# esq4/nind-denoise

Measured on AMD Instinct MI355X. Metric: megapixels/sec denoised, UtNet cs=256 on 24 MP frames, 1/2/4/8 MI355X, higher is better.
Workload: dtype f32; 1 GPU; configs[1]: one 6000x4000 (24.0 MP) fp32 frame per step, f32 storage in the conv stack (fp32 accumulate), UtNet(funit=64,PReLU) random-init (seed 123), cs=264 (nearest valid to the named size; the reference rejects 256 / 512) ucs=200 ol=64 -> 1276 tiles/frame, tiles per conv-stack launch 256, crop->infer->stitch device resident (frame and canvas in HBM); every tile's input is the whole cs x cs cro; tiles_per_frame=1276, parallelism=single GPU

## Files before the change

### include/nind_hip.h

```cpp
#ifndef NIND_HIP_H
#define NIND_HIP_H

#include <stddef.h>
#include <stdint.h>

#ifdef __cplusplus
extern "C" {
#endif

typedef enum nd_status {
    ND_OK = 0,
    ND_EINVAL = -1,
    ND_ENOMEM = -2,
    ND_EHIP = -3
} nd_status;

typedef enum nd_act {
    ND_ACT_NONE = 0,
    ND_ACT_PRELU = 1,
    ND_ACT_ELU = 2,
    ND_ACT_HARDSWISH = 3
} nd_act;

typedef enum nd_layer_kind {
    ND_CONV3 = 0,
    ND_CONVT3 = 1,
    ND_CONVT2S2 = 2,
    ND_CONV1 = 3,
    ND_CONV2S2 = 4
} nd_layer_kind;

typedef enum nd_dtype {
    ND_F32 = 0,
    ND_BF16 = 1,
    ND_F16 = 2
} nd_dtype;

typedef enum nd_flags {
    ND_FLAG_NO_SPLITK = 1,
    ND_FLAG_DIRECT_CONV = 2,
    ND_FLAG_W1D_REGS = 4,
    ND_FLAG_UNFUSED_POOL = 16,
    ND_FLAG_TILE_ENCODER = 32,
    ND_FLAG_TILE_LEVEL2 = 64,
    ND_FLAG_FIND_NOISE = 128,
    ND_FLAG_FULL_TILES = 8
} nd_flags;

int nd_version(void);
const char *nd_last_error(void);

int nd_tile_grid(int width, int height, int cs, int ucs, int ol, int *cols, int *rows, int *pad);
int nd_tile_geom(int i, int width, int height, int cs, int ucs, int ol,
                 int *x0, int *y0, int usefuldim[4], int usefulstart[2]);

int nd_tile_gather(const float *img_chw, int width, int height, int cs, int ucs, int ol,
                   int tile_begin, int tile_count, float *tiles_nchw, void *stream);
int nd_stitch_add(float *canvas_chw, int width, int height, int cs, int ucs, int ol,
                  const float *tiles_nchw, int tile_begin, int tile_count, void *stream);

int nd_utnet_num_tensors(void);
const char *nd_utnet_tensor_name(int idx);
size_t nd_utnet_packed_bytes(int funit, int dtype);
int nd_utnet_pack_weights(int funit, int dtype, const float *const *tensors, int n_tensors,
                          void *packed_host, size_t packed_bytes);

int nd_utnet_pack_weights_device(int funit, int dtype, const float *const *dev_tensors, int n_tensors, void *packed_dev,
                                 size_t packed_bytes, void *stream);

size_t nd_utnet_workspace_bytes_hw(int funit, int h, int w, int batch, int dtype);
int nd_utnet_workspace_init_hw(void *workspace, size_t workspace_bytes, int funit, int h, int w, int batch, int dtype,
                               void *stream);
int nd_utnet_forward_hw(int funit, int act, int dtype, int flags, const void *packed_dev,
                        const float *x_nchw, float *y_nchw, int batch, int h, int w,
                        void *workspace, size_t workspace_bytes, void *stream);

int nd_utnet_denoise_tiles(int funit, int act, int dtype, int flags, const void *packed_dev,
                           const float *img_chw, float *canvas_chw, int width, int height,
                           int cs, int ucs, int ol, int tile_begin, int tile_count, int batch,
                           void *workspace, size_t workspace_bytes, void *stream);

typedef void (*nd_progress_fn)(void *ctx, int n, int tile_begin, int tile_count);
size_t nd_utnet_frame_workspace_bytes(int funit, int dtype, int flags, int width, int height, int cs, int ucs, int ol, int batch);
int nd_utnet_denoise_frame(int funit, int act, int dtype, int flags, const void *packed_dev,
                           const float *img_chw, float *canvas_chw, int width, int height,
                           int cs, int ucs, int ol, int tile_begin, int tile_count, int batch,
                           void *workspace, size_t workspace_bytes, void *frame_ws, size_t frame_ws_bytes, void *stream,
                           nd_progress_fn progress, void *progress_ctx);
int nd_utnet_frame_plan(int funit, int dtype, int flags, int width, int height, int cs, int ucs, int ol, int *out);
int nd_utnet_frame_levels(int funit, int dtype, int flags, int width, int height, int cs, int ucs, int ol, int *levels);

typedef struct nd_step_profile {
    float ms;
    float ms_xform_in;
    float ms_gemm;
    float ms_xform_out;
    int form;
    int kind;
    double flops;
    double mfma_flops;
    double bytes;
    double xform_bytes_in;
    double xform_bytes_out;
} nd_step_profile;
int nd_utnet_profile_stack(int funit, int act, int dtype, int flags, const void *packed_dev, int batch, int cs, int crop,
                           void *workspace, size_t workspace_bytes, void *stream, nd_step_profile *steps, int max_steps);
const char *nd_utnet_step_name(int i);
int nd_utnet_useful_region(int funit, int cs, int crop, int step, int *rect);

int nd_unet_num_tensors(void);
const char *nd_unet_tensor_name(int idx);
size_t nd_unet_packed_bytes(int dtype);
int nd_unet_pack_weights(int dtype, const float *const *tensors, int n_tensors, void *packed_host, size_t packed_bytes);
size_t nd_unet_workspace_bytes(int h, int w, int batch, int dtype);
int nd_unet_workspace_init(void *workspace, size_t workspace_bytes, int h, int w, int batch, int dtype, void *stream);
int nd_unet_forward(int dtype, const void *packed_dev, const float *x_nchw, float *y_nchw, int batch, int h, int w,
                    void *workspace, size_t workspace_bytes, void *stream);

int nd_unet_pack_weights_device(int dtype, const float *const *dev_tensors, int n_tensors, void *packed_dev, size_t packed_bytes,
                                void *stream);

int nd_unet_num_steps(void);
const char *nd_unet_step_name(int i);
int nd_unet_useful_region(int cs, int crop, int step, int *rect);

int nd_unet_denoise_frame(int dtype, int flags, const void *packed_dev, const float *img_chw, float *canvas_chw, int width,
                          int height, int cs, int ucs, int ol, int tile_begin, int tile_count, int batch, void *workspace,
                          size_t workspace_bytes, void *stream, nd_progress_fn progress, void *progress_ctx);

double nd_utnet_flops(int funit, int cs);

size_t nd_layer_packed_bytes(int kind, int cin, int cout, int dtype);
int nd_layer_pack(int kind, int cin, int cout, int dtype, const float *weight, const float *bias,
                  void *packed_host, size_t packed_bytes);
size_t nd_layer_workspace_bytes(int kind, int batch, int cin, int cout, int h, int w, int dtype);
int nd_layer_forward(int kind, int act, float slope, int dtype, const void *packed_dev,
                     const float *x_nchw, int batch, int cin, int h, int w, int cout, float *y_nchw,
                     void *workspace, size_t workspace_bytes, int variant, int flags, void *stream);
int nd_maxpool2_forward(const float *x_nchw, int batch, int c, int h, int w, float *y_nchw,
                        void *workspace, size_t workspace_bytes, void *stream);

size_t nd_layer_wgrad_workspace_bytes(int kind, int batch, int cin, int cout, int h, int w);
int nd_layer_wgrad(int kind, const float *x_nchw, const float *dy_nchw, int batch, int cin, int h, int w, int cout,
// ... 53 lines not shown
```

### nind_denoise_amd/_lib.py

```python
import ctypes
import os
from ctypes import POINTER, c_char_p, c_double, c_float, c_int, c_size_t, c_void_p

_HERE = os.path.dirname(os.path.abspath(__file__))
LIB_PATH = os.path.join(_HERE, "libnind_hip.so")

ND_F32, ND_BF16, ND_F16 = 0, 1, 2
DTYPE = {"f32": 0, "fp32": 0, "float32": 0, "bf16": 1, "bfloat16": 1, "f16": 2, "fp16": 2, "float16": 2}
ACT = {"none": 0, "PReLU": 1, "ELU": 2, "Hardswish": 3}
KIND = {"conv3": 0, "convT3": 1, "convT2s2": 2, "conv1": 3, "conv2s2": 4}
FLAG_NO_SPLITK, FLAG_DIRECT_CONV, FLAG_W1D_REGS, FLAG_FULL_TILES, FLAG_UNFUSED_POOL, FLAG_TILE_ENCODER, FLAG_TILE_LEVEL2 = 1, 2, 4, 8, 16, 32, 64
FLAG_FIND_NOISE = 128
PROGRESS_FN = ctypes.CFUNCTYPE(None, c_void_p, c_int, c_int, c_int)


class StepProfile(ctypes.Structure):
    _fields_ = [("ms", c_float), ("ms_xform_in", c_float), ("ms_gemm", c_float), ("ms_xform_out", c_float),
                ("form", c_int), ("kind", c_int), ("flops", c_double), ("mfma_flops", c_double), ("bytes", c_double),
                ("xform_bytes_in", c_double), ("xform_bytes_out", c_double)]


FORM_NAMES = {-1: "pool", 0: "direct", 1: "w1d_f43", 2: "w1d_f23", 3: "wino3p_f6x6"}


class NindHipError(RuntimeError):
    pass


class NindHipMissing(ImportError):
    pass


_lib = None

_SIGNATURES = {
    "nd_version": (c_int, []),
    "nd_last_error": (c_char_p, []),
    "nd_tile_grid": (c_int, [c_int] * 5 + [POINTER(c_int)] * 3),
    "nd_tile_geom": (c_int, [c_int] * 6 + [POINTER(c_int)] * 4),
    "nd_tile_gather": (c_int, [c_void_p] + [c_int] * 7 + [c_void_p, c_void_p]),
    "nd_stitch_add": (c_int, [c_void_p] + [c_int] * 5 + [c_void_p, c_int, c_int, c_void_p]),
    "nd_utnet_num_tensors": (c_int, []),
    "nd_utnet_tensor_name": (c_char_p, [c_int]),
    "nd_utnet_packed_bytes": (c_size_t, [c_int, c_int]),
    "nd_utnet_pack_weights": (c_int, [c_int, c_int, POINTER(c_void_p), c_int, c_void_p, c_size_t]),
    "nd_utnet_pack_weights_device": (c_int, [c_int, c_int, POINTER(c_void_p), c_int, c_void_p, c_size_t, c_void_p]),
    "nd_utnet_workspace_bytes_hw": (c_size_t, [c_int] * 5),
    "nd_utnet_workspace_init_hw": (c_int, [c_void_p, c_size_t] + [c_int] * 5 + [c_void_p]),
    "nd_utnet_forward_hw": (c_int, [c_int] * 4 + [c_void_p] * 3 + [c_int, c_int, c_int, c_void_p, c_size_t, c_void_p]),
    "nd_utnet_denoise_tiles": (c_int, [c_int] * 4 + [c_void_p] * 3 + [c_int] * 8 + [c_void_p, c_size_t, c_void_p]),
    "nd_unet_num_tensors": (c_int, []),
    "nd_unet_tensor_name": (c_char_p, [c_int]),
    "nd_unet_packed_bytes": (c_size_t, [c_int]),
    "nd_unet_pack_weights": (c_int, [c_int, POINTER(c_void_p), c_int, c_void_p, c_size_t]),
    "nd_unet_workspace_bytes": (c_size_t, [c_int] * 4),
    "nd_unet_workspace_init": (c_int, [c_void_p, c_size_t] + [c_int] * 4 + [c_void_p]),
    "nd_unet_forward": (c_int, [c_int, c_void_p, c_void_p, c_void_p, c_int, c_int, c_int, c_void_p, c_size_t, c_void_p]),
    "nd_unet_pack_weights_device": (c_int, [c_int, POINTER(c_void_p), c_int, c_void_p, c_size_t, c_void_p]),
    "nd_unet_num_steps": (c_int, []),
    "nd_unet_step_name": (c_char_p, [c_int]),
    "nd_unet_useful_region": (c_int, [c_int, c_int, c_int, POINTER(c_int)]),
    "nd_unet_denoise_frame": (c_int, [c_int, c_int] + [c_void_p] * 3 + [c_int] * 8 + [c_void_p, c_size_t, c_void_p, PROGRESS_FN, c_void_p]),
    "nd_utnet_flops": (c_double, [c_int, c_int]),
    "nd_utnet_profile_stack": (c_int, [c_int] * 4 + [c_void_p, c_int, c_int, c_int, c_void_p, c_size_t, c_void_p, c_void_p, c_int]),
    "nd_utnet_step_name": (c_char_p, [c_int]),
    "nd_utnet_useful_region": (c_int, [c_int, c_int, c_int, c_int, POINTER(c_int)]),
    "nd_utnet_frame_workspace_bytes": (c_size_t, [c_int] * 9),
    "nd_utnet_frame_plan": (c_int, [c_int] * 8 + [POINTER(c_int)]),
    "nd_utnet_frame_levels": (c_int, [c_int] * 8 + [POINTER(c_int)]),
    "nd_utnet_denoise_frame": (c_int, [c_int] * 4 + [c_void_p] * 3 + [c_int] * 8 + [c_void_p, c_size_t, c_void_p, c_size_t, c_void_p,
                                                                                    PROGRESS_FN, c_void_p]),
    "nd_layer_packed_bytes": (c_size_t, [c_int] * 4),
    "nd_layer_pack": (c_int, [c_int] * 4 + [c_void_p, c_void_p, c_void_p, c_size_t]),
    "nd_layer_workspace_bytes": (c_size_t, [c_int] * 7),
    "nd_layer_forward": (c_int, [c_int, c_int, c_float, c_int, c_void_p, c_void_p] + [c_int] * 5
                         + [c_void_p, c_void_p, c_size_t, c_int, c_int, c_void_p]),
    "nd_winograd_packed_bytes": (c_size_t, [c_int] * 3),
    "nd_winograd_pack": (c_int, [c_int] * 4 + [c_void_p, c_void_p, c_void_p, c_size_t]),
    "nd_layer_winograd_workspace_bytes": (c_size_t, [c_int] * 7),
    "nd_layer_forward_winograd": (c_int, [c_int, c_int, c_int, c_float, c_void_p, c_void_p] + [c_int] * 5
                                  + [c_void_p, c_void_p, c_size_t, c_int, c_void_p]),
    "nd_maxpool2_forward": (c_int, [c_void_p] + [c_int] * 4 + [c_void_p, c_void_p, c_size_t, c_void_p]),
    "nd_layer_wgrad_workspace_bytes": (c_size_t, [c_int] * 6),
    "nd_layer_wgrad": (c_int, [c_int, c_void_p, c_void_p] + [c_int] * 5 + [c_void_p, c_void_p, c_void_p, c_size_t, c_void_p]),
    "nd_utnet_param_count": (c_size_t, [c_int]),
    "nd_utnet_param_range": (c_int, [c_int, c_int, POINTER(c_size_t), POINTER(c_size_t)]),
    "nd_utnet_train_blob_bytes": (c_size_t, [c_int]),
    "nd_utnet_grad_buckets": (c_int, [c_int, POINTER(c_size_t), POINTER(c_size_t), c_int]),
    "nd_utnet_train_workspace_bytes_hw": (c_size_t, [c_int] * 4),
    "nd_utnet_train_workspace_init_hw": (c_int, [c_void_p, c_size_t, c_int, c_int, c_int, c_int, c_void_p]),
    "nd_utnet_train_forward_hw": (c_int, [c_int, c_int, c_int, c_void_p, c_void_p, c_void_p, c_void_p, c_int, c_int, c_int, c_void_p,
                                          c_size_t, c_void_p]),
    "nd_utnet_train_backward_hw": (c_int, [c_int, c_int, c_int, c_void_p, c_void_p, c_void_p, c_void_p, c_void_p, c_int, c_int, c_int,
                                           c_void_p, c_size_t, c_void_p, POINTER(c_void_p), c_int]),
    "nd_utnet_train_step_hw": (c_int, [c_int, c_int, c_void_p, c_void_p, c_void_p, c_void_p, c_void_p, c_void_p, c_float, c_float,
                                       c_float, c_float, c_void_p, c_int, c_int, c_int, c_int, c_void_p, c_size_t, c_void_p,
                                       POINTER(c_void_p), c_int]),
    "nd_adam_step": (c_int, [c_void_p] * 5 + [c_size_t, c_float, c_float, c_float, c_float, c_int, c_int, c_void_p]),
    "nd_ssim_workspace_bytes": (c_size_t, [c_int] * 4),
    "nd_ssim": (c_int, [c_void_p, c_void_p] + [c_int] * 4 + [c_void_p, c_void_p, c_size_t, c_void_p]),
    "nd_ms_ssim": (c_int, [c_void_p, c_void_p] + [c_int] * 4 + [c_void_p, c_void_p, c_size_t, c_void_p]),
    "nd_ssim_loss_workspace_bytes": (c_size_t, [c_int] * 4),
    "nd_ssim_loss_grad": (c_int, [c_void_p, c_void_p] + [c_int] * 5 + [c_float, c_void_p, c_void_p, c_int, c_void_p, c_size_t,
                                  c_void_p]),
    "nd_mse": (c_int, [c_void_p, c_void_p, c_size_t, c_void_p, c_void_p, c_size_t, c_void_p]),
    "nd_conv_bench": (c_int, [c_int] * 9 + [c_void_p, c_size_t, c_void_p, POINTER(c_float)]),
    "nd_winograd_bench": (c_int, [c_int] * 8 + [c_void_p, c_size_t, c_void_p, POINTER(c_float)]),
    "nd_num_conv_variants": (c_int, []),
    "nd_conv_variant_name": (c_char_p, [c_int]),
}

EXPORTS = tuple(_SIGNATURES)


def load():
    global _lib
    if _lib is not None:
        return _lib
    if not os.path.isfile(LIB_PATH):
        raise NindHipMissing(
            f"{LIB_PATH} not found: build it with `make -C nind_denoise_amd/csrc` (or __graft_entry__.build()). "
            "nind_denoise_amd has no CPU fallback for the denoise hot path.")
# ... 46 lines not shown
```

### nind_denoise_amd/csrc/conv_f32.hip

```cpp
#include "conv_qp.inc"

extern const Variant g_variants_bf16[kGroup];
extern const Variant g_variants_f16[kGroup];
static const Variant g_f32_group[kGroup] = {ND_VARIANT_GROUP(ND_F32, "f32")};
static const Variant g_f32_extra[] = {
    ND_VARIANT(ND_F32, "f32", 2, 2, 2, 4, 9, 1, false, 3),
    ND_VARIANT(ND_F32, "f32", 2, 2, 1, 4, 9, 1, false, 3),
    ND_VARIANT(ND_F32, "f32", 2, 4, 4, 2, 1, 2, false, 3),
    ND_VARIANT(ND_F32, "f32", 2, 2, 2, 4, 1, 2, false, 3),
    ND_VARIANT(ND_F32, "f32", 2, 4, 4, 2, 1, 4, false, 2),
    ND_VARIANT(ND_F32, "f32", 2, 4, 2, 4, 1, 4, false, 2),
    ND_VARIANT(ND_F32, "f32", 2, 4, 4, 2, 1, 4, true, 2),
};
constexpr int kExtra = (int)(sizeof(g_f32_extra) / sizeof(g_f32_extra[0]));
static const int g_nvariants = 3 * kGroup + kExtra;
static const Variant &variant_at(int v) {
    if (v < kGroup) return g_f32_group[v];
    if (v < 2 * kGroup) return g_variants_bf16[v - kGroup];
    if (v < 3 * kGroup) return g_variants_f16[v - 2 * kGroup];
    return g_f32_extra[v - 3 * kGroup];
}


int nd_conv_variant_count() { return g_nvariants; }
// ... 157 lines not shown
        }
        const int order[] = {M <= 32 ? 3 : 0, 0, 1, 2};
        for (int v : order)
            if (variant_lds(variant_at(g0 + v), d.in, nullptr, nullptr, Hr, Wr, band2) <= kMaxLds) return g0 + v;
        return g0 + 2;
    }
    if (taps == 4) return g0 + (variant_lds(variant_at(g0 + 12), d.in, nullptr, nullptr, Hr, Wr) <= kMaxLds ? 12 : 13);
    if (KB % 2) return g0 + (up ? 7 : 5);
    if (up) {
        int cand[8], n = 0;
        if (dt == ND_F32 && M % 256 == 0 && KB % 4 == 0) cand[n++] = 3 * kGroup + 6;
        if (M >= 128) {
            if (KB % 4 == 0) cand[n++] = g0 + 10;
            if (KB % 2 == 0) cand[n++] = g0 + 8;
        }
        if (KB % 4 == 0) cand[n++] = g0 + 9;
        if (KB % 2 == 0) cand[n++] = g0 + 6;
        cand[n++] = g0 + 7;
        for (int i = 0; i < n; ++i)
            if (variant_lds(variant_at(cand[i]), d.in, nullptr, nullptr, Hr, Wr) <= kMaxLds) return cand[i];
        return cand[n - 1];
    }
    return g0 + 4;
}

bool nd_conv_pool_fits(const ConvDesc &d) {
    if (!d.pool || d.in.dt == ND_F32 || nd_taps(d.kind) != 9 || d.roi_rows > 0 || d.pre || d.nbatch > 1) return false;
    if (((d.in.Hb - 2) | (d.in.Wb - 2)) & 1) return false;
    if ((long)(d.in.Hb - 2) * (d.in.Wb - 2) < 100L * 100) return false;
    int dev, cus;
    if (nd_device(&dev, &cus) != ND_OK) return false;
    const int v = pick_variant(d, d.cout, cus);
    if (v < 0 || v >= g_nvariants) return false;
    return variant_lds(variant_at(v), d.in, nullptr, nullptr, 0, 0, true) <= kMaxLds;
}

bool nd_conv_roi_fits(const ConvDesc &d) {
    const bool up = d.kind == ND_CONVT2S2;
    int dev, cus;
    if (nd_device(&dev, &cus) != ND_OK) return false;
    const int v = pick_variant(d, up ? 4 * d.cout : d.cout, cus);
    if (v < 0 || v >= g_nvariants) return false;
    return variant_lds(variant_at(v), d.in, nullptr, nullptr, d.roi_rows > 0 ? d.roi_rows : 0, d.roi_rows > 0 ? d.roi_cols : 0) <= kMaxLds;
}

int nd_launch_conv(const ConvDesc &d, hipStream_t stream) {
    const int taps = nd_taps(d.kind);
    const bool up = d.kind == ND_CONVT2S2;
    const int dt = d.in.dt;
    if (dt < ND_F32 || dt > ND_F16 || d.out.dt != dt) ND_FAIL(ND_EINVAL, "conv: input / output storage types %d / %d", d.in.dt, d.out.dt);
    const int KB = nd_kblocks(d.cin, dt);
    const int M = up ? 4 * d.cout : d.cout;
    if (d.cout % nd_cpp(dt)) ND_FAIL(ND_EINVAL, "conv: cout=%d must be a multiple of %d", d.cout, nd_cpp(dt));
    ND_TRY(nd_check_in_planes("conv", d, KB));
    ND_TRY(nd_check_int32("conv", d.in));

    int dev = 0, ncus = 0;
    ND_TRY(nd_device(&dev, &ncus));
    int v = d.variant >= 0 ? d.variant : pick_variant(d, M, ncus);
    if (v < 0 || v >= g_nvariants) ND_FAIL(ND_EINVAL, "conv: unknown variant %d", v);
    const Variant &V = variant_at(v);
    if (V.taps != taps || V.up != up || V.dt != dt) ND_FAIL(ND_EINVAL, "conv: variant %s does not match layer kind %d / dtype %d", V.name, d.kind, dt);
    if (KB % V.kbc) ND_FAIL(ND_EINVAL, "conv: Cin/8=%d not a multiple of the variant's K chunk %d", KB, V.kbc);

    ConvParams p = nd_conv_params(d, KB, M);
    valid_grid(taps, d.in, &p.Hv, &p.Wv, &p.stride);
    const bool roi = d.roi_rows > 0;
    ND_TRY(nd_check_roi("conv", d, p.Hv, p.Wv, taps == 4 || d.nbatch > 1 || d.pre, "a stride-2, batched or training launch"));
    if (roi) {
        p.out += (long)((up ? 2 : 1) * d.roi_r0) * d.out.Wb + (up ? 2 : 1) * d.roi_c0;
        p.Hv = d.roi_rows;
        p.Wv = d.roi_cols;
    }
    p.PV = p.Hv * p.Wv;
    if (taps == 4 && ((d.in.Hb | d.in.Wb) & 1)) ND_FAIL(ND_EINVAL, "conv: the stride-2 layer reads even-sized buffers only");
    p.ioff = (taps == 9 ? 0 : d.in.pad * d.in.Wb + d.in.pad) + (roi ? d.roi_r0 * d.in.Wb + d.roi_c0 : 0);
    if (d.pre && (dt != ND_F32 || up)) ND_FAIL(ND_EINVAL, "conv: the pre-activation copy exists for fp32 non-upsampling layers only");
    ND_TRY(nd_check_out("conv", d, up ? 2 * p.Hv : p.Hv, up ? 2 * p.Wv : p.Wv, up || roi));

    if (d.pool) {
        if (dt == ND_F32 || taps != 9 || up || roi || d.pre || d.nbatch > 1 || (p.Hv & 1) || (p.Wv & 1))
            ND_FAIL(ND_EINVAL, "conv: a fused pool needs a whole 16-bit 3x3 layer with even output sizes (got %d x %d, dtype %d)", p.Hv, p.Wv, dt);
        ND_TRY(nd_conv_pool("conv", d, p.Hv, p.Wv, p));
        p.band2 = 1;
    }
    bool cross = true;
    const size_t lds = variant_lds(V, d.in, &cross, &p.G, roi ? p.Hv : 0, roi ? p.Wv : 0, p.band2 != 0);
    if (lds > kMaxLds) ND_FAIL(ND_EINVAL, "conv: %zu B of LDS needed (row width %d too large for variant %s)", lds, p.Wb, V.name);
    ND_TRY(nd_raise_lds(dev, (const void *)V.fn, lds));

    nd_conv_tiles(p, cross, V.nblk, V.mblk);
    p.linear = taps == 1 && !up && dt == ND_F32 && d.in.pad == 0 && d.out.pad == 0 && d.out.Hb == d.in.Hb && d.out.Wb == d.in.Wb && cross &&
               d.act == ND_ACT_NONE && d.nbatch > 1 && !d.pre && !roi;
    p.in_bs = d.in_bs;
    p.out_bs = d.out_bs;
    p.w_bs = (long)d.w_bs;
    if (d.nbatch > 1 && d.pre) ND_FAIL(ND_EINVAL, "conv: a batched launch keeps no pre-activation copy");
    nd_conv_fastdivs(p);
    if (dt != ND_F32) p.fd_upq = nd_fastdiv(p.cout / 8 > 0 ? p.cout / 8 : 1);
    const long ntiles = (long)p.tiles_per_problem * (d.nbatch > 1 ? d.nbatch : 1);
    const int per_cu = lds * 2 <= kMaxLds && V.threads <= 256 ? 2 : 1;
    const long slots = (long)ncus * per_cu;
    const long cap = d.part && !d.nosplit && !p.band2 ? (long)(d.part_bytes / ((size_t)V.mblk * V.nblk * 4)) : 0;
    const long grid = nd_conv_schedule(p, ntiles, KB / V.kbc, slots, cap);
    p.part = (f32x4 *)d.part;
#ifdef ND_QP_ABLATE
    static const int abl_env = getenv("ND_QP_ABL") ? atoi(getenv("ND_QP_ABL")) : 0;
    p.dbg = abl_env;
#endif
#ifdef ND_QP_STAMPS
    static const int dbg_env = getenv("ND_QP_DBG") ? atoi(getenv("ND_QP_DBG")) : 0;
    if (dbg_env & 128) {
        static int printed = 0;
        static const char *const names[5] = {"barrier", "issue DMA", "MFMA loop", "wait vmcnt", "epilogue+next"};
        char header[160];
        snprintf(header, sizeof header, "[qp stamps] %s cin %d M %d tiles %ld chunks %d G %d", V.name, d.cin, M, ntiles, KB / V.kbc, p.G);
        p.dbg = dbg_env;
        return nd_stamped_launch(V.fn, V.threads, lds, p, ntiles, KB / V.kbc, slots, stream, printed++ < 40, header, "   wave", names, 5,
// ... 9 lines not shown
```

### nind_denoise_amd/csrc/conv_qp.inc

```
#pragma once
#include <stdlib.h>

#include <initializer_list>
#include <type_traits>

#include "nd_common.h"

typedef float f32x4 __attribute__((ext_vector_type(4)));
typedef float f32x8 __attribute__((ext_vector_type(8)));
typedef float f32x16 __attribute__((ext_vector_type(16)));
typedef __bf16 bf16x8 __attribute__((ext_vector_type(8)));
typedef __bf16 bf16x4 __attribute__((ext_vector_type(4)));
typedef _Float16 f16x8 __attribute__((ext_vector_type(8)));
typedef _Float16 f16x4 __attribute__((ext_vector_type(4)));

template <int DT> struct FragOf { typedef f32x4 type; };
template <> struct FragOf<ND_BF16> { typedef bf16x8 type; };
template <> struct FragOf<ND_F16> { typedef f16x8 type; };

struct FastDiv {
    unsigned m;
    int sh;
};
static inline FastDiv nd_fastdiv(int d) {
    FastDiv f;
    int s = 0;
    while ((1L << s) < (long)d) ++s;
    f.m = (unsigned)((((unsigned long long)1 << (31 + s)) + (unsigned long long)d - 1) / (unsigned long long)d);
    f.sh = 31 + s;
    return f;
}
__device__ __forceinline__ unsigned fdiv(unsigned n, const FastDiv &f) { return (unsigned)(((unsigned long long)n * f.m) >> f.sh); }

struct ConvParams {
    const f32x4 *in;
    const float *wpk;
    const float *bias;
    f32x4 *out;
    long in_plane;
    long out_plane;
    int nimg;
    int P, Wb;
    int Hv, Wv, PV;
    int tpi;
    int G;
    int stride;
    int ioff;
    f32x4 *pre;
    long pre_plane;
    int KB;
    int M;
    int cout;
    int Po, Wo, opad;
    int out_plane0;
    int act;
    float slope;
    const float *slope_dev;
    int n_tiles_n;
    int n_tiles_m;
    int split_first, S, cps, nitems;
    f32x4 *part;
    int wpx;
    int tiles_per_problem;
    long in_bs, out_bs;
    long w_bs;
    int dbg;
    int linear;
    FastDiv fd_PV, fd_Wv, fd_ntm, fd_tpp, fd_upq, fd_tpi;
    f32x4 *pool;
    long pool_plane;
    int pool_P, pool_W, pool_pad;
    int band2;
    FastDiv fd_2Wv;
    const f32x4 *in2;
    long in2_plane;
    const int *origin2;
    int kb2, Wb2;
};

static inline void nd_conv_fastdivs(ConvParams &p) {
    p.fd_PV = nd_fastdiv(p.PV > 0 ? p.PV : 1);
    p.fd_Wv = nd_fastdiv(p.Wv > 0 ? p.Wv : 1);
    p.fd_2Wv = nd_fastdiv(p.Wv > 0 ? 2 * p.Wv : 1);
    p.fd_ntm = nd_fastdiv(p.n_tiles_m > 0 ? p.n_tiles_m : 1);
    p.fd_tpp = nd_fastdiv(p.tiles_per_problem > 0 ? p.tiles_per_problem : 1);
    p.fd_upq = nd_fastdiv(p.cout / 4 > 0 ? p.cout / 4 : 1);
    p.fd_tpi = nd_fastdiv(p.tpi > 0 ? p.tpi : 1);
}

ConvParams nd_conv_params(const ConvDesc &d, int KB, int M);
int nd_conv_pool(const char *who, const ConvDesc &d, int Hv, int Wv, ConvParams &p);
void nd_conv_tiles(ConvParams &p, bool cross, int nblk, int mblk);
long nd_conv_schedule(ConvParams &p, long ntiles, int nchunks, long slots, long cap);
double nd_conv_schedule_time(long ntiles, int nchunks, long slots, long cap);
int nd_launch_split_finish(const ConvParams &p, int n_split_tiles, int mblk, int nblk, int up, int dt, hipStream_t s);
#ifdef ND_QP_STAMPS
int nd_stamped_launch(void (*fn)(ConvParams), int threads, size_t lds, ConvParams p, long ntiles, int nchunks, long slots, hipStream_t s,
                      bool print, const char *header, const char *wave_prefix, const char *const *names, int nphases, std::initializer_list<int> waves);
#endif

__device__ __forceinline__ void glds16(const void *g, void *l) {
    __builtin_amdgcn_global_load_lds((const __attribute__((address_space(1))) void *)g,
                                     (__attribute__((address_space(3))) void *)l, 16, 0, 0);
}

__device__ __forceinline__ f32x8 sload8(const float *p) {
    const unsigned long long a = (unsigned long long)p;
    const unsigned lo = __builtin_amdgcn_readfirstlane((unsigned)a);
    const unsigned hi = __builtin_amdgcn_readfirstlane((unsigned)(a >> 32));
    const float *sp = (const float *)(((unsigned long long)hi << 32) | lo);
    f32x8 v;
    asm volatile("s_load_dwordx8 %0, %1, 0x0\n\ts_waitcnt lgkmcnt(0)" : "=s"(v) : "s"(sp) : "memory");
    return v;
}
__device__ __forceinline__ f32x4 sload_bias4(const float *p, int h) {
    const unsigned long long a = (unsigned long long)p;
    const unsigned lo = __builtin_amdgcn_readfirstlane((unsigned)a);
    const unsigned hi = __builtin_amdgcn_readfirstlane((unsigned)(a >> 32));
    const float *sp = (const float *)(((unsigned long long)hi << 32) | lo);
    f32x4 b0, b1;
    asm volatile("s_load_dwordx4 %0, %2, 0x0\n\ts_load_dwordx4 %1, %2, 0x10\n\ts_waitcnt lgkmcnt(0)" : "=&s"(b0), "=&s"(b1) : "s"(sp) : "memory");
    f32x4 r;
#pragma unroll
    for (int e = 0; e < 4; ++e) r[e] = h ? b1[e] : b0[e];
    return r;
}

#ifdef ND_QP_STAMPS
__device__ __forceinline__ unsigned long long qp_stamp() {
    unsigned long long t;
// ... 77 lines not shown
            const Item it = decode(vb + i * nwg);
            nsteps += it.c1 - it.c0;
        }
    if (nsteps == 0) return;

    auto pixel_of = [&](int nb, int l, int &img, int &r) -> bool {
        bool ok;
        if (p.tpi) {
            img = (int)fdiv((unsigned)nb, p.fd_tpi);
            r = (nb - img * p.tpi) * NBLK + l;
            ok = r < p.PV;
            r = ok ? r : p.PV - 1;
        } else {
            const unsigned g = (unsigned)nb * (unsigned)NBLK + (unsigned)l;
            const unsigned tot = (unsigned)p.nimg * (unsigned)p.PV;
            ok = g < tot;
            const unsigned gc = ok ? g : tot - 1;
            img = (int)fdiv(gc, p.fd_PV);
            r = (int)(gc - (unsigned)img * (unsigned)p.PV);
        }
        return ok;
    };
    auto yx_of = [&](int r, int &y, int &x) {
        if (p.band2) {
            const int band = (int)fdiv((unsigned)r, p.fd_2Wv), rem = r - band * 2 * p.Wv;
            y = 2 * band + (rem & 1);
            x = rem >> 1;
        } else {
            y = (int)fdiv((unsigned)r, p.fd_Wv);
            x = r - y * p.Wv;
        }
    };
    auto q_of = [&](int img, int r) -> long {
        int y, x;
        yx_of(r, y, x);
        return (long)img * p.P + (long)(y * p.stride) * p.Wb + x * p.stride + p.ioff;
    };
    auto tile_q0 = [&](int nb) -> long {
        if (TAPS == 1 && !UP && p.linear) return (long)nb * NBLK;
        int img, r;
        pixel_of(nb, 0, img, r);
        return q_of(img, r);
    };

    int f_id = vb, f_c = 0, f_end = 0, f_stage = 0, issued = 0;
    const float *f_w;
    const f32x4 *f_a;
    auto set_fill_tile = [&](int w) {
        const Item it = decode(w);
        f_c = it.c0;
        f_end = it.c1;
        const int z = (int)fdiv((unsigned)it.tile, p.fd_tpp), id = it.tile - z * p.tiles_per_problem;
        const int nb = (int)fdiv((unsigned)id, p.fd_ntm), mb = id - nb * p.n_tiles_m;
        f_w = p.wpk + z * p.w_bs + (size_t)mb * MTB * p.KB * TAPS * 256 + lane * 4;
        f_a = p.in + z * p.in_bs + tile_q0(nb) + lane;
    };
    set_fill_tile(f_id);
    constexpr bool SPREAD = DT != ND_F32 && TAPS == 9;
    constexpr int NFILL = SPREAD ? NW : (NW > 4 ? 4 : NW);
    constexpr int RW = KBC * TAPS;
    constexpr int NGROUPS = STEPS * (DT == ND_F32 ? 4 : 1);
#ifndef ND_QP_NUSE_NUM
#define ND_QP_NUSE_NUM 5
#endif
    constexpr int NUSE = NGROUPS * ND_QP_NUSE_NUM / 8 > 1 ? NGROUPS * ND_QP_NUSE_NUM / 8 : 1;
    constexpr int PSUB_ = (NUSE - MTB) / (2 * KBC);
    constexpr int PSUB = PSUB_ < 1 ? 1 : (PSUB_ > 4 ? 4 : PSUB_);
    constexpr int NSLICE = MTB + 2 * KBC * PSUB;
    constexpr int SPG = (NSLICE + NUSE - 1) / NUSE;
    char *fill_sb = smem;
    bool fill_on = false;
    auto fill_begin = [&]() {
        fill_on = issued < nsteps;
        fill_sb = smem + f_stage * stageB;
    };
    auto fill_slice = [&](int i) {
        if (!fill_on || wave >= NFILL) return;
#ifdef ND_QP_ABLATE
        if (p.dbg & (i < MTB ? 2 : 1)) return;
#endif
        if (i < MTB) {
            const float *src = f_w + ((size_t)i * p.KB + (size_t)f_c * KBC) * TAPS * 256;
            char *dst = fill_sb + i * RW * 1024;
            for (int q = wave; q < RW; q += NFILL) glds16(src + q * 256, dst + q * 1024);
        } else {
            const int pl = (i - MTB) / PSUB, part = (i - MTB) % PSUB;
            const f32x4 *src = f_a + (size_t)(f_c * 2 * KBC + pl) * p.in_plane;
            char *dst = fill_sb + WBYTES + pl * planeB;
            for (int g = wave + part * NFILL; g < G; g += NFILL * PSUB) glds16(src + g * 64, dst + g * 1024);
        }
    };
    auto fill_end = [&]() {
        if (!fill_on) return;
        ++issued;
        f_stage = (f_stage + 1 == NSTAGE) ? 0 : f_stage + 1;
        if (++f_c == f_end) {
            f_id += nwg;
            if (f_id < nitems) set_fill_tile(f_id);
        }
    };
    auto fill_group = [&](int gi) {
        if (!SPREAD || gi * SPG >= NSLICE) return;
        __builtin_amdgcn_sched_barrier(0);
#pragma unroll
        for (int k = 0; k < SPG; ++k)
            if (gi * SPG + k < NSLICE) {
                fill_slice(gi * SPG + k);
                if (gi * SPG + k == NSLICE - 1) fill_end();
            }
        __builtin_amdgcn_sched_barrier(0);
    };
    auto fill_next = [&]() {
        fill_begin();
#pragma unroll
        for (int i = 0; i < NSLICE; ++i) fill_slice(i);
        fill_end();
    };

    const int aOff = (wm * MR) * KBC * TAPS * 1024 + lane * 16;
    struct BOff { int v[NR]; };
    auto lane_offsets = [&](int w) -> BOff {
        BOff o;
        if (TAPS == 1 && !UP && p.linear) {
#pragma unroll
            for (int nr = 0; nr < NR; ++nr) o.v[nr] = WBYTES + h * planeB + ((wn * NR + nr) * 32 + j) * 16;
            return o;
        }
        const int tl_ = decode(w).tile;
        const int nb = (int)fdiv((unsigned)(tl_ - (int)fdiv((unsigned)tl_, p.fd_tpp) * p.tiles_per_problem), p.fd_ntm);
        const long q0 = tile_q0(nb);
#pragma unroll
        for (int nr = 0; nr < NR; ++nr) {
            int img, r;
            pixel_of(nb, (wn * NR + nr) * 32 + j, img, r);
            o.v[nr] = WBYTES + h * planeB + (int)(q_of(img, r) - q0) * 16;
// ... 349 lines not shown
```

### nind_denoise_amd/csrc/conv_w2d.hip

```cpp
#include "conv_qp.inc"

namespace {

typedef float f32x2 __attribute__((ext_vector_type(2)));

constexpr int kR = 8;
constexpr int kS = 16;
constexpr int kRI = kR + 2;
constexpr int kVPlane = kRI * kS * 16;
constexpr int kVPos = 2 * kVPlane;
constexpr int kVBytes = 6 * kVPos;
constexpr int kTaps = 18;
constexpr int kMTB = 2;
constexpr int kWBytes = kMTB * kTaps * 1024;
constexpr int kStage = kWBytes + kVBytes;
constexpr int kStages = 2;
constexpr int kScratch = 2048;
constexpr int kLds = kStages * kStage + 8 * kScratch;
constexpr int kDmaAt = 4;
constexpr int kXfAt = 12;
constexpr int kSlots = 4 * 32 * 4;

template <int OFF> __device__ __forceinline__ void glds16o(const void *g, void *l) {
    __builtin_amdgcn_global_load_lds((const __attribute__((address_space(1))) void *)g, (__attribute__((address_space(3))) void *)l, 16, OFF, 0);
}

__device__ __forceinline__ int vslot(int r, int s) { return r * kS + (s ^ ((r & 3) << 2)); }

__device__ __forceinline__ void w4_in(const f32x4 *d, f32x4 *v) {
    const f32x4 s34 = d[3] + d[4], d43 = d[4] - d[3], s12 = d[1] + d[2], d12 = d[1] - d[2], d42 = d[4] - d[2], d31 = d[3] - d[1];
    v[0] = 4.f * d[0] - 5.f * d[2] + d[4];
    v[1] = s34 - 4.f * s12;
    v[2] = d43 + 4.f * d12;
    v[3] = d42 + 2.f * d31;
    v[4] = d42 - 2.f * d31;
    v[5] = 4.f * d[1] - 5.f * d[3] + d[5];
}
__device__ __forceinline__ void w4_out(const float *m, float *y) {
    const float a = m[1] + m[2], b = m[1] - m[2], c = m[3] + m[4], e = m[3] - m[4];
    y[0] = m[0] + a + c;
    y[1] = b + 2.f * e;
    y[2] = a + 4.f * c;
    y[3] = b + 8.f * e + m[5];
}

__device__ __forceinline__ unsigned long long stamp() {
    unsigned long long t;
    __builtin_amdgcn_sched_barrier(0);
    asm volatile("s_memtime %0\n\ts_waitcnt lgkmcnt(0)" : "=s"(t)::"memory");
    __builtin_amdgcn_sched_barrier(0);
    return t;
}

struct Strip { int img, y0, x0; bool ok; };

template <int DBG, bool SRC2 = false>
__global__ __launch_bounds__(512) void conv_w2d(ConvParams p) {
    extern __shared__ __attribute__((aligned(16))) char smem[];
    const int lane = threadIdx.x & 63;
    const int wave = __builtin_amdgcn_readfirstlane(threadIdx.x >> 6);
    const int wm = wave >> 2, wn = wave & 3;
    const int j = lane & 31, h = lane >> 5;
    const int nwg = gridDim.x;
    const int bid = blockIdx.x;
    const int vb = (nwg % 8 == 0) ? (bid % 8) * (nwg / 8) + bid / 8 : bid;

    const int nchunks = p.KB;
    const int nitems = p.nitems;
    const int my_items = vb < nitems ? (nitems - vb + nwg - 1) / nwg : 0;
    struct Item { int tile, c0, c1, slice; };
    auto decode = [&](int w) -> Item {
        Item it;
        if (w < p.split_first) {
            it.tile = w; it.c0 = 0; it.c1 = nchunks; it.slice = -1;
        } else {
            const int u = w - p.split_first;
            const int t = u / p.S, ks = u - t * p.S;
            it.tile = p.split_first + t;
            it.c0 = ks * p.cps;
            it.c1 = it.c0 + p.cps < nchunks ? it.c0 + p.cps : nchunks;
            it.slice = u;
        }
        return it;
    };
    int nsteps = 0;
    if (p.split_first >= nitems)
        nsteps = my_items * nchunks;
    else
        for (int i = 0; i < my_items; ++i) {
            const Item it = decode(vb + i * nwg);
            nsteps += it.c1 - it.c0;
        }
    if (nsteps == 0) return;

    const unsigned tot = (unsigned)p.nimg * (unsigned)p.PV;
    auto strip_of = [&](int nb, int s) -> Strip {
        Strip r;
        const unsigned u = (unsigned)nb * kS + s;
        r.ok = u < tot;
        const unsigned uc = r.ok ? u : tot - 1;
        r.img = (int)fdiv(uc, p.fd_PV);
        const int rem = (int)(uc - (unsigned)r.img * p.PV);
        const int band = (int)fdiv((unsigned)rem, p.fd_Wv);
        r.y0 = band * kR;
        r.x0 = 4 * (rem - band * p.Wv);
        return r;
    };

    int f_id = vb, f_c = 0, f_end = 0, f_stage = 0, issued = 0;
    int f_nb = 0;
    const float *f_w;
    const unsigned lane16 = (unsigned)lane * 16u;
    const int kXfHalf = 1;
    const bool xfA = (wave >> 2) == kXfHalf, xfB = wave == 4 * (1 - kXfHalf);
    const int dw = wave - 4 * (1 - kXfHalf);
    int vwOff[2];
    int x_h[2], x_i[2], x_s[2];
#pragma unroll
    for (int ps = 0; ps < 2; ++ps) {
        const int xt = ps == 0 ? (wave & 3) * 64 + lane : 256 + lane;
        x_h[ps] = xt / (kS * kRI);
        x_i[ps] = (xt / kS) % kRI;
        x_s[ps] = xt % kS;
        vwOff[ps] = kWBytes + x_h[ps] * kVPlane + vslot(x_i[ps], x_s[ps]) * 16;
    }
    unsigned x_off[2] = {0, 0};
    int x_keep[2] = {6, 6};
    auto set_fill_tile = [&](int w) {
        const Item it = decode(w);
        f_c = it.c0;
        f_end = it.c1;
        const int nb = (int)fdiv((unsigned)it.tile, p.fd_ntm), mb = it.tile - nb * p.n_tiles_m;
        f_w = p.wpk + (size_t)mb * kMTB * p.KB * kTaps * 256;
        if constexpr (SRC2) f_nb = nb;
#pragma unroll
        for (int ps = 0; ps < 2; ++ps)
            if (ps == 0 ? xfA : xfB) {
                const Strip st = strip_of(nb, x_s[ps]);
                x_off[ps] = 16u * ((unsigned)x_h[ps] * (unsigned)p.in_plane + (unsigned)st.img * (unsigned)p.P + (unsigned)(st.y0 + x_i[ps]) * p.Wb + st.x0);
                const int left = p.wpx - st.x0;
                x_keep[ps] = left + 2 < 6 ? left + 2 : 6;
            }
    };
    auto set_fill_src2 = [&]() {
        const int nb = f_nb;
#pragma unroll
        for (int ps = 0; ps < 2; ++ps)
            if (ps == 0 ? xfA : xfB) {
                const Strip st = strip_of(nb, x_s[ps]);
                x_off[ps] = 16u * ((unsigned)x_h[ps] * (unsigned)p.in2_plane + (unsigned)p.origin2[st.img] + (unsigned)(st.y0 + x_i[ps]) * p.Wb2 + st.x0);
            }
    };
    set_fill_tile(f_id);
    if constexpr (SRC2) if (f_c >= p.kb2) set_fill_src2();
    f32x4 dn[2][6];
#pragma unroll
    for (int ps = 0; ps < 2; ++ps)
#pragma unroll
        for (int k = 0; k < 6; ++k) dn[ps][k] = f32x4{0.f, 0.f, 0.f, 0.f};
    auto fill_loads = [&]() {
        if (issued >= nsteps || (DBG & 8)) return;
        const bool s2 = SRC2 && f_c >= p.kb2;
        const char *kbase = s2 ? (const char *)(p.in2 + (size_t)(2 * (f_c - p.kb2)) * p.in2_plane)
                               : (const char *)(p.in + (size_t)(2 * f_c) * p.in_plane);
        if (xfA) {
#pragma unroll
            for (int k = 0; k < 6; ++k) dn[0][k] = *(const f32x4 *)(kbase + x_off[0] + 16 * k);
        }
        if (xfB) {
#pragma unroll
            for (int k = 0; k < 6; ++k) dn[1][k] = *(const f32x4 *)(kbase + x_off[1] + 16 * k);
        }
    };
    auto fill_xform = [&]() {
        if (issued >= nsteps || (DBG & 16)) return;
#pragma unroll
        for (int ps = 0; ps < 2; ++ps)
            if (ps == 0 ? xfA : xfB) {
                if (__builtin_amdgcn_ballot_w64(x_keep[ps] < 6)) {
                    const f32x4 zero = {0.f, 0.f, 0.f, 0.f};
#pragma unroll
                    for (int k = 3; k < 6; ++k)
                        if (k >= x_keep[ps]) dn[ps][k] = zero;
                }
                f32x4 v[6];
                w4_in(dn[ps], v);
                char *dst = smem + f_stage * kStage + vwOff[ps];
#pragma unroll
                for (int x = 0; x < 6; ++x) *(f32x4 *)(dst + x * kVPos) = v[x];
            }
    };
    auto fill_dma = [&]() {
        if (issued >= nsteps || (DBG & 4)) return;
        if (dw >= 0 && dw < 4) {
            const int mt = dw >> 1, pl0 = (dw & 1) * 9;
            const char *src = (const char *)(f_w + (((size_t)mt * p.KB + (size_t)f_c) * kTaps + pl0) * 256) + lane16;
            char *dst = smem + f_stage * kStage + (mt * kTaps + pl0) * 1024;
            glds16o<-4096>(src + 4096, dst + 4096);
            glds16o<-3072>(src + 4096, dst + 4096);
            glds16o<-2048>(src + 4096, dst + 4096);
            glds16o<-1024>(src + 4096, dst + 4096);
            glds16o<0>(src + 4096, dst + 4096);
            glds16o<1024>(src + 4096, dst + 4096);
            glds16o<2048>(src + 4096, dst + 4096);
            glds16o<3072>(src + 4096, dst + 4096);
            glds16o<0>(src + 8192, dst + 8192);
        }
    };
    auto fill_advance = [&]() {
        if (issued >= nsteps) return;
        ++issued;
        f_stage ^= 1;
        if (++f_c == f_end) {
            f_id += nwg;
            if (f_id < nitems) {
                set_fill_tile(f_id);
                if constexpr (SRC2) if (f_c >= p.kb2) set_fill_src2();
            }
        } else if constexpr (SRC2) {
            if (f_c == p.kb2) set_fill_src2();
        }
    };

    const int sl = 4 * wn + (j >> 3), rr = j & 7;
    const int aOff = (wm * kTaps) * 1024 + lane * 16;
    int bOffK[3];
#pragma unroll
    for (int ky = 0; ky < 3; ++ky) bOffK[ky] = kWBytes + h * kVPlane + vslot(rr + ky, sl) * 16;

    f32x16 acc[6];
#pragma unroll
    for (int x = 0; x < 6; ++x)
#pragma unroll
        for (int r = 0; r < 16; ++r) acc[x][r] = 0.f;

    const float slope = p.act == ND_ACT_NONE ? 1.f : (p.slope_dev ? *p.slope_dev : p.slope);
    const bool slope01 = p.act <= ND_ACT_PRELU && slope >= 0.f && slope <= 1.f;

    auto combine = [&](int g, f32x4 *y) {
#pragma unroll
        for (int e = 0; e < 4; ++e) {
            float m[6], o[4];
#pragma unroll
            for (int x = 0; x < 6; ++x) {
                m[x] = acc[x][4 * g + e];
                acc[x][4 * g + e] = 0.f;
            }
            w4_out(m, o);
#pragma unroll
            for (int i = 0; i < 4; ++i) y[i][e] = o[i];
        }
    };

    char *const scratch = smem + kStages * kStage + wave * kScratch;
    const int e_row = lane >> 4, e_px = lane & 15;
    f32x4 biasq[4];
    auto load_bias = [&](int id) {
        const int mb = id - (int)fdiv((unsigned)id, p.fd_ntm) * p.n_tiles_m;
#pragma unroll
        for (int g = 0; g < 4; ++g) biasq[g] = *(const f32x4 *)(p.bias + (mb * kMTB + wm) * 32 + 8 * g + 4 * h);
    };
    load_bias(decode(vb).tile);
    auto epilogue = [&](int id, auto fast) {
        const int nb = (int)fdiv((unsigned)id, p.fd_ntm), mb = id - nb * p.n_tiles_m;
        const Strip st = strip_of(nb, 4 * wn + (e_px >> 2));
        const int ex = st.x0 + (e_px & 3);
        const unsigned offA = (unsigned)((st.img * p.Po + (st.y0 + e_row + p.opad) * p.Wo + ex + p.opad) * 16);
        const unsigned offB = offA + (unsigned)(4 * p.Wo * 16);
        const bool okx = st.ok && ex < p.wpx;
        const bool okA = okx && st.y0 + e_row < p.Hv, okB = okx && st.y0 + e_row + 4 < p.Hv;
        const int q0 = (mb * kMTB + wm) * 8;
        const f32x2 slope2 = {slope, slope};
        const int pp_i = (e_px & ~3) + 2 * (e_px & 1);
        const int pxp = (st.x0 >> 1) + (e_px & 1), pyp = (st.y0 >> 1) + e_row;
        const bool okP = !SRC2 && p.pool && !(lane & 2) && st.ok && 2 * pxp + 1 < p.wpx && 2 * pyp + 1 < p.Hv;
        const unsigned offP = (unsigned)((st.img * p.pool_P + (pyp + p.pool_pad) * p.pool_W + pxp + p.pool_pad) * 16);
#pragma unroll
        for (int g = 0; g < 4; ++g) {
            f32x4 yy[4], ypre[4];
#pragma unroll
            for (int pr = 0; pr < 2; ++pr) {
                f32x2 m[6];
#pragma unroll
                for (int x = 0; x < 6; ++x) {
                    m[x] = f32x2{acc[x][4 * g + 2 * pr], acc[x][4 * g + 2 * pr + 1]};
                    acc[x][4 * g + 2 * pr] = 0.f;
                    acc[x][4 * g + 2 * pr + 1] = 0.f;
                }
                const f32x2 bq = {biasq[g][2 * pr], biasq[g][2 * pr + 1]};
                const f32x2 a = m[1] + m[2] + bq, b = m[1] - m[2] + bq, c = m[3] + m[4], e = m[3] - m[4];
                f32x2 y[4];
                y[0] = m[0] + a + c;
                y[1] = b + 2.f * e;
                y[2] = a + 4.f * c;
                y[3] = b + 8.f * e + m[5];
#pragma unroll
                for (int i = 0; i < 4; ++i) {
                    ypre[i][2 * pr] = y[i][0];
                    ypre[i][2 * pr + 1] = y[i][1];
                    if constexpr (decltype(fast)::value) {
                        const f32x2 t = y[i] * slope2;
                        y[i] = f32x2{fmaxf(y[i][0], t[0]), fmaxf(y[i][1], t[1])};
                    } else {
                        y[i] = f32x2{apply_act(y[i][0], p.act, slope), apply_act(y[i][1], p.act, slope)};
                    }
                    yy[i][2 * pr] = y[i][0];
                    yy[i][2 * pr + 1] = y[i][1];
                }
            }
            if (!SRC2 && p.pre) {
                const Strip so = strip_of(nb, sl);
                const int yo = so.y0 + rr, m4 = (q0 + 2 * g + h) * 4, left = p.wpx - so.x0;
                if (so.ok && yo < p.Hv && m4 < p.M) {
                    f32x4 *dst = p.pre + (long)(m4 >> 2) * p.pre_plane + ((long)so.img * p.Hv + yo) * p.wpx + so.x0;
#pragma unroll
                    for (int i = 0; i < 4; ++i)
                        if (i < left) dst[i] = ypre[i];
                }
            }
            if (DBG & 256) {
                const Strip so = strip_of(nb, sl);
                const int yo = so.y0 + rr, m4 = (q0 + 2 * g + h) * 4, left = p.wpx - so.x0;
                if (so.ok && yo < p.Hv && m4 < p.M) {
                    f32x4 *dst = p.out + (long)(p.out_plane0 + (m4 >> 2)) * p.out_plane + (long)so.img * p.Po + (long)(yo + p.opad) * p.Wo + so.x0 + p.opad;
#pragma unroll
                    for (int i = 0; i < 4; ++i)
                        if (i < left) dst[i] = yy[i];
                }
                continue;
            }
#pragma unroll
            for (int hq = 0; hq < 2; ++hq) {
                if (h == hq) {
                    f32x4 *w = (f32x4 *)scratch + rr * 16 + (j >> 3) * 4;
#pragma unroll
                    for (int i = 0; i < 4; ++i) w[i] = yy[i];
                }
                __builtin_amdgcn_fence(__ATOMIC_RELEASE, "wavefront");
                __builtin_amdgcn_wave_barrier();
                __builtin_amdgcn_fence(__ATOMIC_ACQUIRE, "wavefront");
                const f32x4 va = *((const f32x4 *)scratch + e_row * 16 + e_px);
                const f32x4 vb2 = *((const f32x4 *)scratch + (e_row + 4) * 16 + e_px);
                f32x4 vp = va;
                if (!SRC2 && p.pool) {
                    const f32x4 *blk = (const f32x4 *)scratch + (2 * e_row) * 16 + pp_i;
                    const f32x4 p00 = blk[0], p01 = blk[1], p10 = blk[16], p11 = blk[17];
#pragma unroll
                    for (int e = 0; e < 4; ++e) vp[e] = fmaxf(fmaxf(p00[e], p01[e]), fmaxf(p10[e], p11[e]));
                }
                __builtin_amdgcn_fence(__ATOMIC_RELEASE, "wavefront");
                __builtin_amdgcn_wave_barrier();
                __builtin_amdgcn_fence(__ATOMIC_ACQUIRE, "wavefront");
                const int quad = q0 + 2 * g + hq;
                if (quad * 4 < p.M && !(DBG & 1)) {
                    char *pb = (char *)(p.out + (size_t)(p.out_plane0 + quad) * p.out_plane);
                    if (okA) *(f32x4 *)(pb + offA) = va;
                    if (okB) *(f32x4 *)(pb + offB) = vb2;
                    if (okP) *(f32x4 *)((char *)(p.pool + (size_t)quad * p.pool_plane) + offP) = vp;
                }
            }
        }
    };
    auto epilogue_partial = [&](int slice) {
        f32x4 *dst = p.part + (size_t)slice * (kMTB * 8) * kSlots;
#pragma unroll
        for (int g = 0; g < 4; ++g) {
            f32x4 yy[4];
            combine(g, yy);
            f32x4 *d2 = dst + (size_t)(wm * 8 + 2 * g + h) * kSlots + 4 * (wn * 32 + j);
#pragma unroll
            for (int i = 0; i < 4; ++i) d2[i] = yy[i];
        }
    };

    fill_loads();
    fill_xform();
    fill_dma();
    fill_advance();
    asm volatile("s_waitcnt vmcnt(0) lgkmcnt(0)" ::: "memory");
    __builtin_amdgcn_s_barrier();

    int c_id = vb, c_stage = 0;
    Item c_it = decode(vb);
    int c_c = c_it.c0;
    unsigned long long tph[6] = {0, 0, 0, 0, 0, 0}, t0 = 0, t1 = 0;
    for (int s = 0; s < nsteps; ++s) {
        if (DBG & 128) t0 = stamp();
        fill_loads();
        __builtin_amdgcn_sched_barrier(0);
        if (DBG & 128) { t1 = stamp(); tph[0] += t1 - t0; t0 = t1; }
        const char *wa = smem + c_stage * kStage + aOff;
        const char *vq = smem + c_stage * kStage;
        f32x4 a[2], b[2];
        a[0] = *(const f32x4 *)wa;
        b[0] = *(const f32x4 *)(vq + bOffK[0]);
#pragma unroll
        for (int st = 0; st < kTaps; ++st) {
// ... 13 lines not shown
            }
            if (st + 1 == kDmaAt) {
                __builtin_amdgcn_sched_barrier(0);
                fill_dma();
                __builtin_amdgcn_sched_barrier(0);
            }
            if (st + 1 == kXfAt) {
                __builtin_amdgcn_sched_barrier(0);
                if (DBG & 128) { t1 = stamp(); tph[1] += t1 - t0; t0 = t1; }
                fill_xform();
                fill_advance();
                if (DBG & 128) { t1 = stamp(); tph[3] += t1 - t0; t0 = t1; }
                __builtin_amdgcn_sched_barrier(0);
            }
        }
        __builtin_amdgcn_sched_barrier(0);
        if (DBG & 128) { t1 = stamp(); tph[1] += t1 - t0; t0 = t1; }
        asm volatile("s_waitcnt vmcnt(0) lgkmcnt(0)" ::: "memory");
        if (DBG & 128) { t1 = stamp(); tph[2] += t1 - t0; t0 = t1; }
        c_stage ^= 1;
        if (++c_c == c_it.c1) {
            if (DBG & 2) {
            } else if (c_it.slice >= 0)
                epilogue_partial(c_it.slice);
            else if (slope01)
                epilogue(c_it.tile, std::true_type{});
            else
                epilogue(c_it.tile, std::false_type{});
            c_id += nwg;
            if (c_id < nitems) {
                c_it = decode(c_id);
                if (p.n_tiles_m > 1) load_bias(c_it.tile);
            }
            c_c = c_it.c0;
        }
        if (DBG & 128) { t1 = stamp(); tph[4] += t1 - t0; t0 = t1; }
        if (!(DBG & 64)) __builtin_amdgcn_s_barrier();
        if (DBG & 128) { t1 = stamp(); tph[5] += t1 - t0; }
    }
    if ((DBG & 128) && lane == 0 && p.part) {
        unsigned long long *o = (unsigned long long *)p.part + ((size_t)blockIdx.x * 8 + wave) * 8;
        for (int k = 0; k < 6; ++k) o[k] = tph[k];
        o[6] = (unsigned long long)nsteps;
    }
}

__global__ __launch_bounds__(256) void k_w2d_split_finish(ConvParams p) {
    const int t = blockIdx.x, quad = blockIdx.y;
    const int gid = p.split_first + t;
    const int nb = gid / p.n_tiles_m, mb = gid - nb * p.n_tiles_m;
    const int m4 = mb * (kMTB * 32) + quad * 4;
    if (m4 >= p.M) return;
    const float slope = p.act == ND_ACT_NONE ? 1.f : (p.slope_dev ? *p.slope_dev : p.slope);
    const f32x4 bv = *(const f32x4 *)(p.bias + m4);
    const unsigned tot = (unsigned)p.nimg * (unsigned)p.PV;
    for (int l = threadIdx.x; l < kSlots; l += 256) {
        const int i = l & 3, jj = l >> 2, wn = jj >> 5, j = jj & 31;
        const int s = 4 * wn + (j >> 3), rr = j & 7;
        const unsigned u = (unsigned)nb * kS + s;
        if (u >= tot) continue;
        const int img = (int)(u / (unsigned)p.PV);
        const int rem = (int)(u - (unsigned)img * p.PV);
        const int band = rem / p.Wv;
        const int y = band * kR + rr, x = 4 * (rem - band * p.Wv) + i;
        if (y >= p.Hv || x >= p.wpx) continue;
        f32x4 acc = {0.f, 0.f, 0.f, 0.f};
        for (int ks = 0; ks < p.S; ++ks) acc += p.part[((size_t)(t * p.S + ks) * (kMTB * 8) + quad) * kSlots + l];
        acc += bv;
        f32x4 v;
#pragma unroll
        for (int e = 0; e < 4; ++e) v[e] = p.act <= ND_ACT_PRELU ? (acc[e] > 0.f ? acc[e] : acc[e] * slope) : apply_act(acc[e], p.act, slope);
        p.out[(long)(p.out_plane0 + (m4 >> 2)) * p.out_plane + (long)img * p.Po + (long)(y + p.opad) * p.Wo + x + p.opad] = v;
    }
}

}

bool nd_w2d_ok(const QpBuf &in) { return in.dt == ND_F32 && in.Hb >= 3 && in.Wb >= 3; }
long nd_w2d_tiles(const QpBuf &in, int cout) {
    const long strips = (long)in.B * ((in.Hb - 2 + kR - 1) / kR) * ((in.Wb - 2 + 3) / 4);
    return ((strips + kS - 1) / kS) * ((cout + kMTB * 32 - 1) / (kMTB * 32));
}

int nd_launch_conv_w2d(const ConvDesc &d, hipStream_t stream) {
    if ((d.kind != ND_CONV3 && d.kind != ND_CONVT3) || d.in.dt != ND_F32 || d.out.dt != ND_F32) ND_FAIL(ND_EINVAL, "w2d: fp32 3x3 layers only");
    const int KB = nd_kblocks(d.cin);
    const int Hfull = d.in.Hb - 2, Wfull = d.in.Wb - 2;
    if (Hfull < 1 || Wfull < 1) ND_FAIL(ND_EINVAL, "w2d: input smaller than the kernel");
    ND_TRY(nd_check_roi("w2d", d, Hfull, Wfull, d.pool != nullptr, "a pooled layer"));
    const bool roi = d.roi_rows > 0;
    const int Hv = roi ? d.roi_rows : Hfull, Wpx = roi ? d.roi_cols : Wfull, Wg = (Wpx + 3) / 4, NB = (Hv + kR - 1) / kR;
    if (d.pre && (roi || d.pool)) ND_FAIL(ND_EINVAL, "w2d: a pre-activation copy goes with whole, unpooled layers only");
    if (d.cout % 4) ND_FAIL(ND_EINVAL, "w2d: cout must be a multiple of 4");
    ND_TRY(nd_check_in_planes("w2d", d, KB, true));
    const bool src2 = d.in2.base != nullptr;
    if (src2 && (d.pool || d.pre)) ND_FAIL(ND_EINVAL, "w2d: a layer with a second input source is neither pooled nor keeps a pre-activation copy");
    if (src2) ND_TRY(nd_check_in2("w2d", d, KB, (long)(d.roi_r0 + (NB - 1) * kR + kRI - 1) * d.in2.Wb + d.roi_c0 + 4 * (Wg - 1) + 6));
    ND_TRY(nd_check_out("w2d", d, Hfull, Wfull, false));
    ND_TRY(nd_check_int32("w2d", d.in));
    if (2 * d.in.np() * 16 + 65536 >= (1L << 32)) ND_FAIL(ND_EINVAL, "w2d: input too large for 32-bit byte offsets");

    int dev = 0, ncus = 0;
    ND_TRY(nd_device(&dev, &ncus));
    void (*fn)(ConvParams) = src2 ? conv_w2d<0, true> : conv_w2d<0>;
#ifdef ND_QP_STAMPS
    static const int dbg_all = getenv("ND_W2D_DBG") ? atoi(getenv("ND_W2D_DBG")) : 0;
    const int dbg_env = src2 ? 0 : dbg_all;
    switch (dbg_env) {
        case 1: fn = conv_w2d<1>; break;
        case 2: fn = conv_w2d<2>; break;
        case 4: fn = conv_w2d<4>; break;
        case 8: fn = conv_w2d<8>; break;
        case 16: fn = conv_w2d<16>; break;
        case 24: fn = conv_w2d<24>; break;
        case 28: fn = conv_w2d<28>; break;
        case 30: fn = conv_w2d<30>; break;
        case 32: fn = conv_w2d<32>; break;
        case 62: fn = conv_w2d<62>; break;
        case 128: fn = conv_w2d<128>; break;
        case 256: fn = conv_w2d<256>; break;
        default: break;
    }
#endif
    ND_TRY(nd_raise_lds(dev, (const void *)fn, kLds));

    ConvParams p = nd_conv_params(d, KB, d.cout);
    if (roi) {
        p.in += (long)d.roi_r0 * d.in.Wb + d.roi_c0;
        p.out += (long)d.roi_r0 * d.out.Wb + d.roi_c0;
    }
    if (src2) {
        p.in2 = (const f32x4 *)d.in2.base + (long)d.in2_plane0 * d.in2.np() + (roi ? (long)d.roi_r0 * d.in2.Wb + d.roi_c0 : 0);
        p.in2_plane = d.in2.np();
        p.origin2 = d.in2_origin;
        p.kb2 = d.in2_from / 2;
        p.Wb2 = d.in2.Wb;
    }
    p.Hv = Hv;
    p.Wv = Wg;
    p.PV = NB * Wg;
    p.wpx = Wpx;
    if (d.pool) {
        ND_TRY(nd_conv_pool("w2d", d, Hv, Wpx, p));
        if (d.pool->used() * 16 >= (1L << 32)) ND_FAIL(ND_EINVAL, "w2d: pooled destination too large for 32-bit byte offsets");
    }
    nd_conv_tiles(p, true, kS, kMTB * 32);
    nd_conv_fastdivs(p);
    const long ntiles = p.tiles_per_problem;
    const long cap = d.part && !d.nosplit && !d.pool && !d.pre ? (long)(d.part_bytes / ((size_t)kMTB * 32 * kSlots * 4)) : 0;
    const long grid = nd_conv_schedule(p, ntiles, KB, ncus, cap);
    p.part = (f32x4 *)d.part;
#ifdef ND_QP_STAMPS
    if (dbg_env == 128) {
        static int printed = 0;
        static const char *const names[6] = {"issue loads + DMA", "MFMA loop", "wait vmcnt", "transform+publish (inside the loop)", "epilogue", "barrier"};
        return nd_stamped_launch(fn, 512, kLds, p, ntiles, KB, ncus, stream, printed++ < 2, nullptr, "[w2d stamps] wave", names, 6, {0, 1, 4});
    }
#endif
    hipLaunchKernelGGL(fn, dim3((unsigned)grid), dim3(512), kLds, stream, p);
    if (p.split_first < ntiles) hipLaunchKernelGGL(k_w2d_split_finish, dim3((unsigned)(ntiles - p.split_first), kMTB * 8), dim3(256), 0, stream, p);
    ND_HIP(hipGetLastError());
    return ND_OK;
}

bool nd_f43_w2d(const QpBuf &in, int cout, bool pre, int flags) {
    return !(flags & ND_FLAG_W1D_REGS) && nd_w2d_ok(in) && (!pre || nd_w2d_tiles(in, cout) >= 512);
}
int nd_launch_conv_f43(const ConvDesc &d, int flags, hipStream_t stream) {
    return nd_f43_w2d(d.in, d.cout, d.pre != nullptr, flags) ? nd_launch_conv_w2d(d, stream) : nd_launch_conv_w1d(4, d, stream);
}
```

### nind_denoise_amd/csrc/launch.hip

```cpp
#include <atomic>
#include <mutex>
#include <unordered_map>
#include <vector>

#include "conv_qp.inc"

namespace {
constexpr int kMaxDevices = 16;
std::atomic<int> g_cus[kMaxDevices];
std::mutex g_mu;
std::unordered_map<const void *, int> g_state[kMaxDevices];
}

int nd_device(int *dev, int *ncus) {
    ND_HIP(hipGetDevice(dev));
    if (*dev < 0 || *dev >= kMaxDevices) ND_FAIL(ND_EINVAL, "device index %d outside [0, %d)", *dev, kMaxDevices);
    if (!ncus) return ND_OK;
    int n = g_cus[*dev].load(std::memory_order_relaxed);
    if (!n) {
        hipDeviceProp_t prop;
        ND_HIP(hipGetDeviceProperties(&prop, *dev));
        n = prop.multiProcessorCount > 0 ? prop.multiProcessorCount : 256;
        g_cus[*dev].store(n, std::memory_order_relaxed);
    }
    *ncus = n;
    return ND_OK;
}

int nd_raise_lds(int dev, const void *fn, size_t bytes) {
    std::lock_guard<std::mutex> lock(g_mu);
    int &limit = g_state[dev][fn];
    if ((int)bytes <= limit) return ND_OK;
    ND_HIP(hipFuncSetAttribute(fn, hipFuncAttributeMaxDynamicSharedMemorySize, (int)bytes));
    limit = (int)bytes;
    return ND_OK;
}

int nd_once_per_device(int dev, int (*init)()) {
    std::lock_guard<std::mutex> lock(g_mu);
    int &done = g_state[dev][(const void *)init];
    if (done) return ND_OK;
    ND_TRY(init());
    done = 1;
    return ND_OK;
}

int nd_check_in_planes(const char *who, const ConvDesc &d, int KB, bool takes_in2) {
    if (d.in.planes < d.in_plane0 + 2 * KB) ND_FAIL(ND_EINVAL, "%s: input buffer has %d planes, needs %d", who, d.in.planes, d.in_plane0 + 2 * KB);
    if (d.in2.base && !takes_in2) ND_FAIL(ND_EINVAL, "%s: this kernel form has no second input source", who);
    return ND_OK;
}

int nd_check_in2(const char *who, const ConvDesc &d, int KB, long reach) {
    const QpBuf &q = d.in2;
    const int n2 = 2 * KB - d.in2_from;
    if (q.dt != ND_F32 || d.in.dt != ND_F32 || !d.in2_origin || d.in2_from <= 0 || (d.in2_from & 1) || n2 <= 0 || d.in2_plane0 < 0 ||
        d.in2_plane0 + n2 > q.planes || d.in2_origin_max < 0 || reach <= 0)
        ND_FAIL(ND_EINVAL, "%s: second input source: planes [%d,+%d) of %d from input plane %d of %d", who, d.in2_plane0, n2, q.planes,
                d.in2_from, 2 * KB);
    const long last = d.in2_origin_max + reach, room = (long)(q.planes - d.in2_plane0 - n2 + 1) * q.np() + (long)nd_buf_slack(q.Wb);
    if (last > room) ND_FAIL(ND_EINVAL, "%s: second input source: a launch reaches element %ld of a plane, the buffer ends at %ld", who, last, room);
    if ((2 * q.np() + last) * 16 + 65536 >= (1L << 32)) ND_FAIL(ND_EINVAL, "%s: second input source too large for 32-bit byte offsets", who);
    return ND_OK;
}

int nd_check_out(const char *who, const ConvDesc &d, int oh, int ow, bool at_least) {
    const int Hb = oh + 2 * d.out.pad, Wb = ow + 2 * d.out.pad;
    const bool fits = at_least ? (d.out.Hb >= Hb && d.out.Wb >= Wb) : (d.out.Hb == Hb && d.out.Wb == Wb);
    if (!fits || d.out.B != d.in.B)
        ND_FAIL(ND_EINVAL, "%s: destination %dx%dx%d(pad %d) does not fit result %dx%dx%d", who, d.out.B, d.out.Hb, d.out.Wb, d.out.pad,
                d.in.B, oh, ow);
    if (d.out_plane0 + d.cout / nd_cpp(d.out.dt) > d.out.planes) ND_FAIL(ND_EINVAL, "%s: destination planes overflow", who);
    return ND_OK;
}

int nd_check_int32(const char *who, const QpBuf &in) {
    if (in.used() >= (1L << 31)) ND_FAIL(ND_EINVAL, "%s: %ld linear pixels exceed the int32 index range", who, in.used());
    return ND_OK;
}

int nd_check_roi(const char *who, const ConvDesc &d, int Hv, int Wv, bool refused, const char *why) {
    if (d.roi_rows <= 0) return ND_OK;
    if (refused || d.roi_r0 < 0 || d.roi_c0 < 0 || d.roi_cols < 1 || d.roi_r0 + d.roi_rows > Hv || d.roi_c0 + d.roi_cols > Wv)
        ND_FAIL(ND_EINVAL, "%s: region [%d,+%d) x [%d,+%d) outside the %d x %d grid (or %s)", who, d.roi_r0, d.roi_rows, d.roi_c0,
                d.roi_cols, Hv, Wv, why);
    return ND_OK;
}

ConvParams nd_conv_params(const ConvDesc &d, int KB, int M) {
    ConvParams p = {};
    p.in = (const f32x4 *)d.in.base + (long)d.in_plane0 * d.in.np();
    p.wpk = d.wpk;
    p.bias = d.bias;
    p.out = (f32x4 *)d.out.base;
    p.in_plane = d.in.np();
    p.out_plane = d.out.np();
    p.nimg = d.in.B;
    p.P = d.in.Hb * d.in.Wb;
    p.Wb = d.in.Wb;
    p.pre = (f32x4 *)d.pre;
    p.pre_plane = d.pre_plane;
    p.KB = KB;
    p.M = M;
    p.cout = d.cout;
    p.Po = d.out.Hb * d.out.Wb;
    p.Wo = d.out.Wb;
    p.opad = d.out.pad;
    p.out_plane0 = d.out_plane0;
    p.act = d.act;
    p.slope = d.slope;
    p.slope_dev = d.slope_dev;
    return p;
}

int nd_conv_pool(const char *who, const ConvDesc &d, int Hv, int Wv, ConvParams &p) {
    const QpBuf &q = *d.pool;
    if (q.dt != d.in.dt || q.B != d.in.B || q.Hb - 2 * q.pad != Hv / 2 || q.Wb - 2 * q.pad != Wv / 2 || q.planes < d.cout / nd_cpp(d.in.dt))
        ND_FAIL(ND_EINVAL, "%s: pooled destination does not fit %d x %d x %d", who, d.cout, Hv / 2, Wv / 2);
    p.pool = (f32x4 *)q.base;
    p.pool_plane = q.np();
    p.pool_P = q.Hb * q.Wb;
    p.pool_W = q.Wb;
    p.pool_pad = q.pad;
    return ND_OK;
}

void nd_conv_tiles(ConvParams &p, bool cross, int nblk, int mblk) {
    if (cross) {
        p.tpi = 0;
        p.n_tiles_n = (int)(((long)p.nimg * p.PV + nblk - 1) / nblk);
    } else {
        p.tpi = (p.PV + nblk - 1) / nblk;
        p.n_tiles_n = p.tpi * p.nimg;
    }
    p.n_tiles_m = (p.M + mblk - 1) / mblk;
    p.tiles_per_problem = p.n_tiles_n * p.n_tiles_m;
}

namespace {
constexpr double kSplitOver = 3.0;
struct SplitPlan { int first, S, cps; double time; };
SplitPlan plan_split(long ntiles, int nchunks, long slots, long max_items) {
    SplitPlan b;
    const long full = ntiles / slots * slots, R = ntiles - full;
    b.first = (int)ntiles;
    b.S = 1;
    b.cps = nchunks;
    b.time = (double)((ntiles + slots - 1) / slots) * (nchunks + kSplitOver);
    if (R == 0 || max_items <= 0) return b;
    const double base = (double)(full / slots) * (nchunks + kSplitOver);
    for (int S = 2; S <= nchunks && S <= 64; ++S) {
        const int cps = (nchunks + S - 1) / S, Se = (nchunks + cps - 1) / cps;
        if (R * Se > max_items) break;
        const double t = base + (double)((R * Se + slots - 1) / slots) * (cps + 1.5 * kSplitOver);
        if (t < 0.93 * b.time) {
// ... 62 lines not shown
```

### nind_denoise_amd/csrc/nd_common.h

```cpp
#pragma once
#include <hip/hip_runtime.h>

#include <stdarg.h>
#include <stdint.h>
#include <stdio.h>

#include "nind_hip.h"

void nd_set_error(const char *fmt, ...);
#define ND_FAIL(code, ...)        \
    do {                          \
        nd_set_error(__VA_ARGS__); \
        return (code);            \
    } while (0)
#define ND_HIP(call)                                                                         \
    do {                                                                                     \
        hipError_t e_ = (call);                                                              \
        if (e_ != hipSuccess) ND_FAIL(ND_EHIP, "%s failed: %s", #call, hipGetErrorString(e_)); \
    } while (0)
#define ND_TRY(call)        \
    do {                    \
        int r_ = (call);    \
        if (r_ != 0) return r_; \
    } while (0)

static inline int nd_cpp(int dt) { return dt == ND_F32 ? 4 : 8; }
struct QpBuf {
    float *base;
    int planes;
    int B, Hb, Wb;
    int pad;
    long pstride;
    int dt = ND_F32;
    long np() const { return pstride; }
    long used() const { return (long)B * Hb * Wb; }
};

struct ConvDesc {
    int kind = ND_CONV3;
    int act = ND_ACT_NONE;
    float slope = 1.f;
    const float *slope_dev = nullptr;
    const float *wpk = nullptr;
    const float *bias = nullptr;
    int cin = 0, cout = 0;
    QpBuf in = {};
    QpBuf out = {};
    int out_plane0 = 0;
    int variant = -1;
    int in_plane0 = 0;
    float *pre = nullptr;
    long pre_plane = 0;
    float *part = nullptr;
    size_t part_bytes = 0;
    bool nosplit = false;
    int nbatch = 1;
    long in_bs = 0, out_bs = 0;
    size_t w_bs = 0;
    const QpBuf *pool = nullptr;
    int roi_r0 = 0, roi_c0 = 0, roi_rows = 0, roi_cols = 0;
    QpBuf in2 = {};
    int in2_plane0 = 0, in2_from = 0;
    const int *in2_origin = nullptr;
    long in2_origin_max = 0;
};
int nd_check_in2(const char *who, const ConvDesc &d, int KB, long reach);
static const size_t kSplitScratchBytes = (size_t)512 * 64 * 1024 * 4;
int nd_launch_conv(const ConvDesc &d, hipStream_t stream);
bool nd_conv_pool_fits(const ConvDesc &d);
bool nd_conv_roi_fits(const ConvDesc &d);
int nd_conv_variant_count();
int nd_conv_variant_gemm(int cin, int cout);
size_t nd_wino_packed_floats(int T, int cin, int cout);
int nd_wino_pack(int T, int kind, int cin, int cout, const float *w, const float *bias, float *packed);
size_t nd_wino_scratch_bytes(int T, const QpBuf &in, int cin, int cout);
int nd_launch_conv_wino(int T, const ConvDesc &d, void *scratch, size_t scratch_bytes, hipStream_t s, hipEvent_t *ev2 = nullptr);
void nd_wino_xform_bytes(int T, const QpBuf &in, int cin, int cout, double *bytes_in, double *bytes_out);
size_t nd_w1d_packed_floats(int T, int cin, int cout);
int nd_w1d_pack(int T, int kind, int cin, int cout, const float *w, const float *bias, float *packed);
bool nd_w1d_fits(int T, const QpBuf &in);
int nd_launch_conv_w1d(int T, const ConvDesc &d, hipStream_t stream);
bool nd_w2d_ok(const QpBuf &in);
long nd_w2d_tiles(const QpBuf &in, int cout);
int nd_launch_conv_w2d(const ConvDesc &d, hipStream_t stream);
bool nd_f43_w2d(const QpBuf &in, int cout, bool pre, int flags);
int nd_launch_conv_f43(const ConvDesc &d, int flags, hipStream_t stream);
static inline size_t nd_buf_slack(int Wb) { return (size_t)10 * Wb + 8 + 2048; }
int nd_device(int *dev, int *ncus = nullptr);
int nd_raise_lds(int dev, const void *fn, size_t bytes);
int nd_once_per_device(int dev, int (*init)());
int nd_check_in_planes(const char *who, const ConvDesc &d, int KB, bool takes_in2 = false);
int nd_check_out(const char *who, const ConvDesc &d, int oh, int ow, bool at_least);
int nd_check_int32(const char *who, const QpBuf &in);
int nd_check_roi(const char *who, const ConvDesc &d, int Hv, int Wv, bool refused, const char *why);
static inline int nd_check_flags(int flags, bool frame_loop = false, bool unet_frame = false) {
    const int known = ND_FLAG_NO_SPLITK | ND_FLAG_DIRECT_CONV | ND_FLAG_W1D_REGS | ND_FLAG_FULL_TILES | ND_FLAG_UNFUSED_POOL |
                      ND_FLAG_TILE_ENCODER | (frame_loop ? ND_FLAG_TILE_LEVEL2 : 0) | (unet_frame ? ND_FLAG_FIND_NOISE : 0);
    if (flags & ~known) ND_FAIL(ND_EINVAL, "unknown flag bits 0x%x", flags);
    return ND_OK;
}
const char *nd_conv_variant_label(int v);

static inline int nd_mtiles(int kind, int cout) {
    return kind == ND_CONVT2S2 ? (4 * cout + 255) / 256 * 8 : (cout + 127) / 128 * 4;
}
struct NdUpRow { int a, b, co; };
__host__ __device__ static inline NdUpRow nd_up_row(int m, int cout, int dt) {
    NdUpRow r;
    const int cpp = dt == ND_F32 ? 4 : 8, q = cout / cpp;
    const int G = m / (2 * cpp), e = m % cpp;
    r.b = (m / cpp) & 1;
    r.a = G / q;
    r.co = cpp * (G % q) + e;
    return r;
}
static inline int nd_taps(int kind) { return (kind == ND_CONV3 || kind == ND_CONVT3) ? 9 : (kind == ND_CONV2S2 ? 4 : 1); }
static inline int nd_kblocks(int cin, int dt = ND_F32) { return (cin + 2 * nd_cpp(dt) - 1) / (2 * nd_cpp(dt)); }
static inline size_t nd_bias_offset(int kind, int cin, int cout, int dt = ND_F32, int w1d_T = 0) {
    return (size_t)nd_mtiles(kind, cout) * nd_kblocks(cin, dt) * (w1d_T ? 3 * (w1d_T + 2) : nd_taps(kind)) * 256;
}
static inline size_t nd_packed_floats(int kind, int cin, int cout, int dt = ND_F32) {
    return nd_bias_offset(kind, cin, cout, dt) + (size_t)nd_mtiles(kind, cout) * 32;
}
void nd_pack_layer(int kind, int cin, int cout, int dt, const float *w, const float *bias, float *packed);

int nd_pack_layer_device(int kind, int cin, int cout, int dt, const float *w, const float *bias, float *packed, hipStream_t s,
                         const float *scale = nullptr);
int nd_launch_bn_fold(int cout, const float *b, const float *g, const float *be, const float *rm, const float *rv, float *scale,
                      float *fbias, hipStream_t s);
int nd_pack_w1d_device(int T, int kind, int cin, int cout, const float *w, const float *bias, float *packed, hipStream_t s);
int nd_pack_wino_device(int T, int kind, int cin, int cout, const float *w, const float *bias, float *packed, hipStream_t s);

int nd_launch_nchw_to_qp(const float *x, int C, const QpBuf &dst, int plane0, hipStream_t s);
int nd_launch_qp_to_nchw(const QpBuf &src, int plane0, float *y, int C, hipStream_t s);
int nd_launch_reflect_pack(const float *x_nchw, int B, int H, int W, const QpBuf &dst, hipStream_t s);
int nd_launch_maxpool2(const QpBuf &src, int src_plane0, int planes, const QpBuf &dst, hipStream_t s);
int nd_launch_final1x1(const QpBuf &src, int cin, const float *w, const float *bias, int crop, float *y_nchw, int H,
                       int W, hipStream_t s, int sigmoid = 0);
int nd_launch_final1x1_stitch(const QpBuf &src, int cin, const float *w, const float *bias, int crop, float *canvas,
                              int width, int height, int cs, int ucs, int ol, int tile_begin, int tile_count,
                              hipStream_t s, int sigmoid = 0, const float *noise_img = nullptr);
int nd_launch_gather_pack(const float *img, int width, int height, int cs, int ucs, int ol, int tile_begin,
                          int tile_count, const QpBuf &dst, hipStream_t s, int border = 2, bool reflect = true);
int nd_launch_gather_band(const float *img, int width, int height, int cs, int ucs, int ol, int band_row0, const QpBuf &dst,
                          hipStream_t s);
enum nd_edge_set { ND_EDGE_ROWS = 0, ND_EDGE_COLS = 1, ND_EDGE_CORNERS = 2 };
int nd_launch_gather_edges(const float *img, int width, int height, int cs, int ucs, int ol, int set, int first, int count,
                           const QpBuf &dst, hipStream_t s);
int nd_launch_skip_origins(const QpBuf &src, int dst_pad, int tile_begin, int tile_count, int cols, int band_rows, int step, long slot_elems,
                           int *table, long *origin_max, hipStream_t s);
// ... 7 lines not shown
```

### nind_denoise_amd/csrc/pack.hip

```cpp
#include <string.h>

#include "nd_common.h"

static thread_local char g_err[512] = "";

void nd_set_error(const char *fmt, ...) {
    va_list ap;
    va_start(ap, fmt);
    vsnprintf(g_err, sizeof(g_err), fmt, ap);
    va_end(ap);
}

extern "C" const char *nd_last_error(void) { return g_err; }
extern "C" int nd_version(void) { return 109; }

static inline uint16_t f32_to_bf16_rne(float f) {
    uint32_t u;
    memcpy(&u, &f, 4);
    if ((u & 0x7fffffffu) > 0x7f800000u) return (uint16_t)((u >> 16) | 0x40);
    return (uint16_t)((u + 0x7fffu + ((u >> 16) & 1u)) >> 16);
}
static inline uint16_t f32_to_f16_rne(float f) {
    const _Float16 h = (_Float16)f;
    uint16_t u;
    memcpy(&u, &h, 2);
    return u;
}

void nd_pack_layer(int kind, int cin, int cout, int dt, const float *w, const float *bias, float *packed) {
    const int taps = nd_taps(kind);
    const int KB = nd_kblocks(cin, dt);
    const int MT = nd_mtiles(kind, cout);
    const int M = kind == ND_CONVT2S2 ? 4 * cout : cout;
    const int cpp = nd_cpp(dt);
    float *bp = packed + nd_bias_offset(kind, cin, cout, dt);
    auto weff = [&](int m, int ci, int t) -> float {
        if (m >= M || ci >= cin) return 0.f;
        switch (kind) {
            case ND_CONV3: return w[((size_t)m * cin + ci) * 9 + t];
            case ND_CONVT3: return w[((size_t)ci * cout + m) * 9 + (8 - t)];
            case ND_CONVT2S2: {
                const NdUpRow r = nd_up_row(m, cout, dt);
                return w[((size_t)ci * cout + r.co) * 4 + 2 * r.a + r.b];
            }
            case ND_CONV2S2: return w[((size_t)m * cin + ci) * 4 + t];
            default: return w[(size_t)m * cin + ci];
        }
    };
    for (int mt = 0; mt < MT; ++mt)
        for (int kb = 0; kb < KB; ++kb)
            for (int t = 0; t < taps; ++t) {
                float *dst = packed + (((size_t)mt * KB + kb) * taps + t) * 256;
                uint16_t *dst16 = (uint16_t *)dst;
                for (int lane = 0; lane < 64; ++lane) {
                    const int i = lane & 31, h = lane >> 5;
                    const int m = 32 * mt + i;
                    for (int s = 0; s < cpp; ++s) {
                        const float v = weff(m, 2 * cpp * kb + cpp * h + s, t);
                        if (dt == ND_F32)
                            dst[lane * 4 + s] = v;
                        else
                            dst16[lane * 8 + s] = dt == ND_BF16 ? f32_to_bf16_rne(v) : f32_to_f16_rne(v);
                    }
                }
            }
    for (int m = 0; m < MT * 32; ++m) {
        float v = 0.f;
// ... 21 lines not shown
```

### nind_denoise_amd/csrc/utnet.hip

```cpp
#include <string.h>

#include <string>
#include <vector>

#include "nd_common.h"

#include "utnet_net.h"

extern "C" int nd_utnet_num_tensors(void) { return (int)tensor_names().size(); }
extern "C" const char *nd_utnet_tensor_name(int idx) {
    const auto &n = tensor_names();
    return (idx >= 0 && idx < (int)n.size()) ? n[idx].c_str() : nullptr;
}

extern "C" size_t nd_utnet_packed_bytes(int funit, int dtype) {
    if (check_funit(funit, dtype) != ND_OK) return 0;
    return blob_layout(funit, dtype).total * sizeof(float);
}

extern "C" int nd_utnet_pack_weights(int funit, int dtype, const float *const *tensors, int n_tensors, void *packed_host,
                                     size_t packed_bytes) {
    ND_TRY(check_funit(funit, dtype));
    if (n_tensors != nd_utnet_num_tensors()) ND_FAIL(ND_EINVAL, "nd_utnet_pack_weights: expected %d tensors, got %d", nd_utnet_num_tensors(), n_tensors);
    const BlobLayout bl = blob_layout(funit, dtype);
// ... 108 lines not shown
    ND_TRY(nd_launch_final1x1(pl.buf[T4B], funit, fw, fw + 3 * funit, 2, y, h, w, s));
    return ND_OK;
}

extern "C" int nd_utnet_denoise_tiles(int funit, int act, int dtype, int flags, const void *packed, const float *img,
                                      float *canvas, int width, int height, int cs, int ucs, int ol, int tile_begin,
                                      int tile_count, int batch, void *ws, size_t ws_bytes, void *stream) {
    ND_TRY(nd_check_flags(flags));
    Plan pl;
    ND_TRY(forward_common(funit, act, dtype, packed, batch, tile_count, cs, cs, ws, ws_bytes, &pl));
    if (!img || !canvas) ND_FAIL(ND_EINVAL, "UtNet: null image");
    hipStream_t s = (hipStream_t)stream;
    const float *blob = (const float *)packed;
    ND_TRY(nd_launch_gather_pack(img, width, height, cs, ucs, ol, tile_begin, tile_count, pl.buf[X0], s));
    const BlobLayout bl = blob_layout(funit, dtype);
    Roi rois[kNumSteps];
    StackOpts o;
    o.flags = flags;
    const int crop = (cs - ucs) / 2;
    if (!(flags & ND_FLAG_FULL_TILES) && plan_rois(pl, crop, crop, rois) && rois_supported(funit, dtype, flags, pl, bl, rois)) o.rois = rois;
    ND_TRY(run_stack(funit, act, dtype, blob, pl, s, o));
    const float *fw = blob + bl.off[kNumLayers - 1];
    ND_TRY(nd_launch_final1x1_stitch(pl.buf[T4B], funit, fw, fw + 3 * funit, 2, canvas, width, height, cs, ucs, ol,
                                     tile_begin, tile_count, s));
    return ND_OK;
}

extern "C" size_t nd_utnet_frame_workspace_bytes(int funit, int dtype, int flags, int width, int height, int cs, int ucs, int ol,
                                                 int batch) {
    FramePlan fp;
    if (nd_check_flags(flags, true) != ND_OK || frame_plan(funit, dtype, flags, width, height, cs, ucs, ol, batch, &fp) != ND_OK) return 0;
    return fp.bytes;
}

extern "C" int nd_utnet_frame_plan(int funit, int dtype, int flags, int width, int height, int cs, int ucs, int ol, int *out) {
    ND_TRY(nd_check_flags(flags, true));
    if (!out) ND_FAIL(ND_EINVAL, "nd_utnet_frame_plan: null output");
    FramePlan fp;
    ND_TRY(frame_plan(funit, dtype, flags, width, height, cs, ucs, ol, 1, &fp));
    const int v[8] = {fp.D, fp.aligned, fp.R, fp.nbands, fp.S, fp.cols, fp.rows, fp.hx};
    memcpy(out, v, sizeof(v));
    return ND_OK;
}

extern "C" int nd_utnet_frame_levels(int funit, int dtype, int flags, int width, int height, int cs, int ucs, int ol, int *levels) {
    ND_TRY(nd_check_flags(flags, true));
    if (!levels) ND_FAIL(ND_EINVAL, "nd_utnet_frame_levels: null output");
    FramePlan fp;
    ND_TRY(frame_plan(funit, dtype, flags, width, height, cs, ucs, ol, 1, &fp));
    *levels = fp.levels;
    return ND_OK;
}

extern "C" int nd_utnet_denoise_frame(int funit, int act, int dtype, int flags, const void *packed, const float *img, float *canvas,
                                      int width, int height, int cs, int ucs, int ol, int tile_begin, int tile_count, int batch,
                                      void *ws, size_t ws_bytes, void *fws, size_t fws_bytes, void *stream, nd_progress_fn progress,
                                      void *progress_ctx) {
    ND_TRY(nd_check_flags(flags, true));
    FramePlan fp;
    ND_TRY(frame_plan(funit, dtype, flags, width, height, cs, ucs, ol, batch, &fp));
    if (tile_begin < 0 || tile_count < 0 || tile_begin + tile_count > fp.cols * fp.rows)
        ND_FAIL(ND_EINVAL, "nd_utnet_denoise_frame: tiles [%d,+%d) outside the grid of %d", tile_begin, tile_count, fp.cols * fp.rows);
    const int end = tile_begin + tile_count;
    Plan pl;
    ND_TRY(forward_common(funit, act, dtype, packed, batch, batch, cs, cs, ws, ws_bytes, &pl));
    const BlobLayout bl = blob_layout(funit, dtype);
    Roi rois[kNumSteps];
    const int crop = (cs - ucs) / 2;
    if (fp.D && !(plan_rois(pl, crop, crop, rois) && rois_supported(funit, dtype, flags, pl, bl, rois))) fp.D = 0;
    if (fp.D == 0) {
        int n = 0;
        for (int t0 = tile_begin; t0 < end; t0 += batch, ++n) {
            const int cnt = end - t0 < batch ? end - t0 : batch;
            if (progress) progress(progress_ctx, n, t0, cnt);
            ND_TRY(nd_utnet_denoise_tiles(funit, act, dtype, flags & ~ND_FLAG_TILE_LEVEL2, packed, img, canvas, width, height, cs, ucs, ol, t0, cnt, batch, ws,
                                          ws_bytes, stream));
        }
        return ND_OK;
    }
    if (!img || !canvas) ND_FAIL(ND_EINVAL, "UtNet: null image");
    if (!fws || fws_bytes < fp.bytes || ((uintptr_t)fws & 255))
        ND_FAIL(ND_ENOMEM, "nd_utnet_denoise_frame: frame workspace %zu B given, %zu B needed (256-byte aligned)", fws_bytes, fp.bytes);
    hipStream_t s = (hipStream_t)stream;
    const float *blob = (const float *)packed;
    const float *fw = blob + bl.off[kNumLayers - 1];
    char *const band_base = (char *)fws, *const rows_base = band_base + fp.band_bytes, *const cols_base = rows_base + fp.row_edge_bytes;
    char *const corner_base = cols_base + fp.col_edge_bytes;
    int *const origins = (int *)(corner_base + fp.corner_bytes);
    const bool l2 = fp.levels == 3;
    char *const l2_band_base = (char *)origins + 3 * fp.origin_bytes, *const l2_rows_base = l2_band_base + fp.l2_band_bytes;
    char *const l2_cols_base = l2_rows_base + fp.l2_row_bytes, *const l2_corner_base = l2_cols_base + fp.l2_col_bytes;
    char *const l2_wino = l2_corner_base + fp.l2_corner_bytes;
    const int f4 = funit / 4, cols = fp.cols, S = fp.S;
    const int n2 = enc_extent(cs + 4, P2), n3 = l2_extent(n2, P3);
    StackOpts enc, enc2, dec;
    enc.flags = enc2.flags = dec.flags = flags;
    enc.step_end = enc2.step_begin = kSharedSteps;
    enc2.step_end = kLevel2End;
    dec.step_begin = l2 ? kLevel2End : kSharedSteps;
    dec.rois = rois;
    auto l2_scratch = [&](Plan p) {
        p.split = pl.split;
        p.wino = l2_wino;
        p.wino_bytes = fp.l2_wino_bytes;
        return p;
    };
    struct Skip { Buf cat; int planes, step, tstep; const int *win; int *table; bool in_place; } skips[3] = {
        {CAT4, f4, -1, S, fp.win4, origins, false}, {CAT3, 2 * f4, -1, S / 2, fp.win3, origins + fp.origin_bytes / sizeof(int), false},
        {CAT2, 4 * f4, -1, S / 4, fp.win2, origins + 2 * fp.origin_bytes / sizeof(int), false}};
    const int nskips = l2 ? 3 : 2;
    for (Skip &k : skips)
        for (int i = kSharedSteps; i < kNumSteps; ++i)
            if (kSteps[i].layer >= 0 && kSteps[i].src == k.cat) {
                k.step = i;
                k.in_place = form_takes_src2(kSteps[i], step_form(kSteps[i], funit, dtype, flags, pl, bl), funit, flags, pl);
            }
    StepSrc2 src2[3];
    dec.src2 = src2;
    const int per_band = fp.R * cols;
    const Plan bf = make_enc_plan(funit, fp.hx, fp.wx, 1, fp.hx, fp.wx, 1, band_base, dtype, fp.slots);
    const Plan bf2 = l2 ? l2_band_plan(fp, funit, dtype, fp.R, cs, l2_band_base) : Plan();
    int band_done = tile_begin / per_band - 1;
    for (int t0 = tile_begin, n = 0; t0 < end; ++n) {
        const int b0 = t0 / per_band;
        int cnt = end - t0 < batch ? end - t0 : batch;
        if (t0 + cnt > (b0 + 2) * per_band) cnt = (b0 + 2) * per_band - t0;
        for (int b = band_done + 1; b <= (t0 + cnt - 1) / per_band; ++b) {
            const int row0 = b * fp.R, nrows = fp.rows - row0 < fp.R ? fp.rows - row0 : fp.R;
            Plan bp = band_slot(make_enc_plan(funit, band_hx(fp, nrows, cs), fp.wx, 1, fp.hx, fp.wx, 1, band_base, dtype, fp.slots), b & 1, fp.slots);
            bp.split = pl.split;
            ND_TRY(nd_launch_gather_band(img, width, height, cs, ucs, ol, row0, bp.buf[X0], s));
            ND_TRY(run_stack(funit, act, dtype, blob, bp, s, enc));
            Plan re = band_slot(row_edge_plan(fp, funit, dtype, nrows, rows_base), b & 1, fp.slots, P2);
            Plan ce = band_slot(col_edge_plan(fp, funit, dtype, nrows, cs, cols_base), b & 1, fp.slots, P2);
            re.split = ce.split = pl.split;
            ND_TRY(nd_launch_gather_edges(img, width, height, cs, ucs, ol, ND_EDGE_ROWS, row0, nrows, re.buf[X0], s));
            ND_TRY(nd_launch_gather_edges(img, width, height, cs, ucs, ol, ND_EDGE_COLS, row0, nrows, ce.buf[X0], s));
            ND_TRY(run_stack(funit, act, dtype, blob, re, s, enc));
            ND_TRY(run_stack(funit, act, dtype, blob, ce, s, enc));
            if (l2) {
                Plan b2 = l2_scratch(l2_slot(l2_band_plan(fp, funit, dtype, nrows, cs, l2_band_base), b & 1, fp.slots));
                b2.buf[P2] = bp.buf[P2];
                ND_TRY(run_stack(funit, act, dtype, blob, b2, s, enc2));
                const Plan r2 = l2_scratch(l2_slot(l2_row_plan(fp, funit, dtype, nrows, l2_rows_base), b & 1, fp.slots, P3));
                const Plan c2 = l2_scratch(l2_slot(l2_col_plan(fp, funit, dtype, nrows, cs, l2_cols_base), b & 1, fp.slots, P3));
                const int h2 = bp.buf[P2].Hb, w2 = bp.buf[P2].Wb;
                for (int side = 0; side < 2; ++side) {
                    const int at = side * (kStrip2 - 1), in0 = 1 - side, in1 = kStrip2 - side;
                    SpliceMap br, lr, bc, lc;
                    br.step_y = bc.step_x = S / 4;
                    br.oy = bc.ox = side * (n2 - kStrip2);
                    lr.img_y = lc.img_x = 2;
                    lr.img_add = lc.img_add = side;
                    lr.oy = lc.ox = -at;
                    ND_TRY(nd_launch_splice(bp.buf[P2], 0, r2.buf[P2], 0, 2 * f4, 0, nrows, 1, 0, br, in0, in1, 0, w2, s, 0, 0, side * nrows));
                    ND_TRY(nd_launch_splice(re.buf[P2], 0, r2.buf[P2], 0, 2 * f4, 0, nrows, 1, 0, lr, at, at + 1, 0, w2, s, 0, 0, side * nrows));
                    ND_TRY(nd_launch_splice(bp.buf[P2], 0, c2.buf[P2], 0, 2 * f4, 0, cols, cols, 0, bc, 0, h2, in0, in1, s, 0, 0, side * cols));
                    ND_TRY(nd_launch_splice(ce.buf[P2], 0, c2.buf[P2], 0, 2 * f4, 0, cols, cols, 0, lc, 0, h2, at, at + 1, s, 0, 0, side * cols));
                }
                ND_TRY(run_stack(funit, act, dtype, blob, r2, s, enc2));
                ND_TRY(run_stack(funit, act, dtype, blob, c2, s, enc2));
            }
            band_done = b;
        }
        if (progress) progress(progress_ctx, n, t0, cnt);
        Plan cp = corner_plan(funit, dtype, cnt, batch, corner_base);
        cp.split = pl.split;
        ND_TRY(nd_launch_gather_edges(img, width, height, cs, ucs, ol, ND_EDGE_CORNERS, t0, cnt, cp.buf[X0], s));
        ND_TRY(run_stack(funit, act, dtype, blob, cp, s, enc));
        const Plan tp = make_plan(funit, cs, cs, batch, cnt, (char *)ws, dtype);
        dec.nsrc2 = 0;
        for (int ki = 0; ki < nskips; ++ki) {
            const Skip &k = skips[ki];
            const QpBuf &src = k.cat == CAT2 ? bf2.buf[k.cat] : bf.buf[k.cat];
            if (!k.in_place) {
                SpliceMap m;
                m.step_y = m.step_x = k.tstep;
                ND_TRY(nd_launch_splice(src, k.planes, tp.buf[k.cat], k.planes, k.planes, t0, cnt, cols, 0, m, k.win[0], k.win[1], k.win[0],
                                        k.win[1], s, fp.R, slot_elems(src, fp.slots)));
                continue;
            }
            StepSrc2 &q = src2[dec.nsrc2++];
            q.step = k.step;
            q.buf = src;
            q.plane0 = q.from = k.planes;
            q.origin = k.table;
            ND_TRY(nd_launch_skip_origins(src, tp.buf[k.cat].pad, t0, cnt, cols, fp.R, k.tstep, slot_elems(src, fp.slots), k.table,
                                          &q.origin_max, s));
        }
        SpliceMap whole;
        whole.step_y = whole.step_x = S / 4;
        ND_TRY(nd_launch_splice(bf.buf[P2], 0, tp.buf[P2], 0, 2 * f4, t0, cnt, cols, 0, whole, 0, n2, 0, n2, s, fp.R,
                                slot_elems(bf.buf[P2], fp.slots)));
        for (int b = b0; b <= (t0 + cnt - 1) / per_band; ++b) {
            const int lo = t0 > b * per_band ? t0 : b * per_band, hi = t0 + cnt < (b + 1) * per_band ? t0 + cnt : (b + 1) * per_band;
            const int row0 = b * fp.R, nrows = fp.rows - row0 < fp.R ? fp.rows - row0 : fp.R;
            const QpBuf rl = band_slot(row_edge_plan(fp, funit, dtype, nrows, rows_base), b & 1, fp.slots, P2).buf[P2];
            const QpBuf cl = band_slot(col_edge_plan(fp, funit, dtype, nrows, cs, cols_base), b & 1, fp.slots, P2).buf[P2];
            for (int side = 0; side < 2; ++side) {
                const int at = side * (n2 - 1);
                SpliceMap mr, mc;
                mr.step_x = mc.step_y = S / 4;
                mr.img_y = mc.img_x = 2;
                mr.img_add = mc.img_add = side;
                mr.oy = mc.ox = -at;
                ND_TRY(nd_launch_splice(rl, 0, tp.buf[P2], 0, 2 * f4, lo, hi - lo, cols, row0, mr, at, at + 1, 0, n2, s, 0, 0, lo - t0));
                ND_TRY(nd_launch_splice(cl, 0, tp.buf[P2], 0, 2 * f4, lo, hi - lo, cols, row0, mc, 0, n2, at, at + 1, s, 0, 0, lo - t0));
            }
        }
        for (int k = 0; k < 4; ++k) {
            const int r = (k >> 1) * (n2 - 1), c = (k & 1) * (n2 - 1);
            SpliceMap m;
            m.img_t = 4;
            m.img_add = k;
            m.oy = -r;
            m.ox = -c;
            ND_TRY(nd_launch_splice(cp.buf[P2], 0, tp.buf[P2], 0, 2 * f4, t0, cnt, cols, 0, m, r, r + 1, c, c + 1, s));
        }
        if (l2) {
            const Plan k2 = l2_scratch(l2_corner_plan(funit, dtype, cnt, batch, l2_corner_base));
            for (int k = 0; k < 4; ++k) {
                SpliceMap m;
                m.img_t = 1;
                m.oy = (k >> 1) * (n2 - kStrip2);
                m.ox = (k & 1) * (n2 - kStrip2);
                ND_TRY(nd_launch_splice(tp.buf[P2], 0, k2.buf[P2], 0, 2 * f4, 0, cnt, cnt, 0, m, 0, kStrip2, 0, kStrip2, s, 0, 0, k * cnt));
            }
            ND_TRY(run_stack(funit, act, dtype, blob, k2, s, enc2));
            SpliceMap whole3;
            whole3.step_y = whole3.step_x = S / 8;
            ND_TRY(nd_launch_splice(bf2.buf[P3], 0, tp.buf[P3], 0, 4 * f4, t0, cnt, cols, 0, whole3, 0, n3, 0, n3, s, fp.R,
                                    slot_elems(bf2.buf[P3], fp.slots)));
            for (int b = b0; b <= (t0 + cnt - 1) / per_band; ++b) {
                const int lo = t0 > b * per_band ? t0 : b * per_band, hi = t0 + cnt < (b + 1) * per_band ? t0 + cnt : (b + 1) * per_band;
                const int row0 = b * fp.R, nrows = fp.rows - row0 < fp.R ? fp.rows - row0 : fp.R;
                const QpBuf rl = l2_slot(l2_row_plan(fp, funit, dtype, nrows, l2_rows_base), b & 1, fp.slots, P3).buf[P3];
                const QpBuf cl = l2_slot(l2_col_plan(fp, funit, dtype, nrows, cs, l2_cols_base), b & 1, fp.slots, P3).buf[P3];
                for (int side = 0; side < 2; ++side) {
// ... 443 lines not shown
```

### nind_denoise_amd/csrc/utnet_net.h

```cpp
#pragma once
#include <string.h>

#include <string>
#include <vector>

#include "nd_common.h"

namespace {

struct LayerSpec {
    const char *key;
    int kind;
    int cin_mul, cout_mul;
    int prelu;
};

const LayerSpec kLayers[] = {
    {"convs1.0", ND_CONV3, 0, 1, 0},    {"convs1.2", ND_CONV3, 1, 1, 1},    {"convs2.0", ND_CONV3, 1, 2, 2},
    {"convs2.2", ND_CONV3, 2, 2, 3},    {"convs3.0", ND_CONV3, 2, 4, 4},    {"convs3.2", ND_CONV3, 4, 4, 5},
    {"convs4.0", ND_CONV3, 4, 8, 6},    {"convs4.2", ND_CONV3, 8, 8, 7},    {"bottom.0", ND_CONV3, 8, 16, 8},
    {"bottom.2", ND_CONVT3, 16, 16, 9}, {"up1", ND_CONVT2S2, 16, 8, -1},    {"tconvs1.0", ND_CONVT3, 16, 8, 10},
    {"tconvs1.2", ND_CONVT3, 8, 8, 11}, {"up2", ND_CONVT2S2, 8, 4, -1},     {"tconvs2.0", ND_CONVT3, 8, 4, 12},
    {"tconvs2.2", ND_CONVT3, 4, 4, 13}, {"up3", ND_CONVT2S2, 4, 2, -1},     {"tconvs3.0", ND_CONVT3, 4, 2, 14},
    {"tconvs3.2", ND_CONVT3, 2, 2, 15}, {"up4", ND_CONVT2S2, 2, 1, -1},     {"tconvs4.0", ND_CONVT3, 2, 1, 16},
// ... 259 lines not shown
        const Buf b = kind == ND_CONVT3 ? st.dst : st.src;
        const QpBuf &q = pl.buf[b];
        const int H = q.Hb - 2 * q.pad, W = q.Wb - 2 * q.pad;
        int r0 = 0, r1 = H, c0 = 0, c1 = W;
        if (kind == ND_CONVT3) {
            if (hi[0][b] >= 0) { r0 = lo[0][b]; r1 = hi[0][b]; }
            if (hi[1][b] >= 0) { c0 = lo[1][b]; c1 = hi[1][b]; }
        } else {
            if (hi[0][st.dst] >= 0) { r0 = lo[0][st.dst] >> 1; r1 = (hi[0][st.dst] + 1) >> 1; }
            if (hi[1][st.dst] >= 0) { c0 = lo[1][st.dst] >> 1; c1 = (hi[1][st.dst] + 1) >> 1; }
        }
        r0 = r0 < 0 ? 0 : r0; c0 = c0 < 0 ? 0 : c0;
        r1 = r1 > H ? H : r1; c1 = c1 > W ? W : c1;
        if (r0 == 0 && c0 == 0 && r1 == H && c1 == W) continue;
        if (r1 <= r0 || c1 <= c0) continue;
        roi[i] = Roi{r0, c0, r1 - r0, c1 - c0};
        any = true;
    }
    return any;
}

inline bool rois_supported(int f, int dt, int flags, const Plan &pl, const BlobLayout &bl, const Roi *rois) {
    for (int i = 0; i < kNumSteps; ++i) {
        if (rois[i].rows <= 0) continue;
        const Form form = step_form(kSteps[i], f, dt, flags, pl, bl);
        if (form == FORM_DIRECT) {
            const LayerSpec &l = kLayers[kSteps[i].layer];
            ConvDesc d;
            d.kind = l.kind;
            d.cin = lcin(l, f);
            d.cout = lcout(l, f);
            d.in = pl.buf[kSteps[i].src];
            d.out = pl.buf[kSteps[i].dst];
            d.roi_r0 = rois[i].r0;
            d.roi_c0 = rois[i].c0;
            d.roi_rows = rois[i].rows;
            d.roi_cols = rois[i].cols;
            if (!nd_conv_roi_fits(d)) return false;
            continue;
        }
        if (form == FORM_WINO3P) continue;
        if (form == FORM_W1D4 && !(flags & ND_FLAG_W1D_REGS)) continue;
        return false;
    }
    return true;
}

struct StepSrc2 {
    int step = -1;
    QpBuf buf = {};
    int plane0 = 0, from = 0;
    const int *origin = nullptr;
    long origin_max = 0;
};
inline bool form_takes_src2(const Step &st, Form form, int f, int flags, const Plan &pl) {
    if (form == FORM_WINO3P) return kWinoTile == 6;
    return form == FORM_W1D4 && nd_f43_w2d(pl.buf[st.src], lcout(kLayers[st.layer], f), false, flags);
}

struct StackOpts {
    int flags = 0;
    const Roi *rois = nullptr;
    int step_begin = 0, step_end = kNumSteps;
    const StepSrc2 *src2 = nullptr;
    int nsrc2 = 0;
    hipEvent_t *ev = nullptr;
    hipEvent_t *ev_x = nullptr;
    const QpBuf *pre = nullptr;
    const unsigned char *train_w1 = nullptr;
};
int run_stack(int f, int act, int dt, const float *blob, const Plan &pl, hipStream_t s, const StackOpts &o) {
    const QpBuf *const pre = o.pre;
    const int flags = o.flags, step_begin = o.step_begin, step_end = o.step_end;
    const BlobLayout bl = blob_layout(f, dt, pre != nullptr);
    const int cpp = nd_cpp(dt);
    int si = step_begin;
    bool pool_done = false;
    QpBuf pool_view;
    for (int k = step_begin; k < step_end; ++k) {
        const Step &st = kSteps[k];
        if (o.ev) ND_HIP(hipEventRecord(o.ev[si], s));
        const int this_step = si++;
        if (st.layer < 0) {
            if (pool_done) {
                pool_done = false;
                continue;
            }
            ND_TRY(nd_launch_maxpool2(pl.buf[st.src], st.dst_plane0_mul * f / cpp, st.dst_plane0_mul * f / cpp, pl.buf[st.dst], s));
            continue;
        }
        const LayerSpec &l = kLayers[st.layer];
        ConvDesc d;
        d.kind = l.kind;
        d.act = l.prelu >= 0 ? act : ND_ACT_NONE;
        d.slope = 0.25f;
        d.slope_dev = (l.prelu >= 0 && act == ND_ACT_PRELU) ? blob + l.prelu : nullptr;
        if (pre && l.prelu >= 0) {
            d.pre = pre[l.prelu].base;
            d.pre_plane = pre[l.prelu].np();
        }
        d.cin = lcin(l, f);
        d.cout = lcout(l, f);
        d.wpk = blob + bl.off[st.layer];
        d.bias = d.wpk + nd_bias_offset(l.kind, d.cin, d.cout, dt);
        d.in = pl.buf[st.src];
        d.out = pl.buf[st.dst];
        d.out_plane0 = st.dst_plane0_mul * f / cpp;
        d.part = pl.split;
        d.part_bytes = kSplitScratchBytes;
        d.nosplit = (flags & ND_FLAG_NO_SPLITK) != 0;
        const Form form = step_form(st, f, dt, flags, pl, bl, o.train_w1);
        if (o.rois && o.rois[this_step].rows > 0) {
            d.roi_r0 = o.rois[this_step].r0;
            d.roi_c0 = o.rois[this_step].c0;
            d.roi_rows = o.rois[this_step].rows;
            d.roi_cols = o.rois[this_step].cols;
        }
        for (int i = 0; i < o.nsrc2; ++i)
            if (o.src2[i].step == k) {
                d.in2 = o.src2[i].buf;
                d.in2_plane0 = o.src2[i].plane0;
                d.in2_from = o.src2[i].from;
                d.in2_origin = o.src2[i].origin;
                d.in2_origin_max = o.src2[i].origin_max;
            }
        const bool next_is_pool = this_step + 1 < step_end && kSteps[this_step + 1].layer < 0;
        const bool w2d = form == FORM_W1D4 && nd_f43_w2d(d.in, d.cout, pre != nullptr, flags);
        if (next_is_pool && !pre && !(flags & ND_FLAG_UNFUSED_POOL)) {
            pool_view = pl.buf[kSteps[this_step + 1].dst];
            d.pool = &pool_view;
            pool_done = w2d || form == FORM_WINO3P || (form == FORM_DIRECT && dt != ND_F32 && nd_conv_pool_fits(d));
            if (!pool_done) d.pool = nullptr;
        }
        if (form == FORM_W1D4 || form == FORM_W1D2) {
            const int T = form == FORM_W1D4 ? kW1dTile : 2;
            if (!pre) d.wpk = blob + (T == kW1dTile ? bl.w1off[st.layer] : bl.w1off2[st.layer]);
            d.bias = d.wpk + nd_bias_offset(d.kind, d.cin, d.cout, ND_F32, T);
            ND_TRY(form == FORM_W1D4 ? nd_launch_conv_f43(d, flags, s) : nd_launch_conv_w1d(T, d, s));
            continue;
        }
        if (form == FORM_WINO3P) {
            d.wpk = blob + bl.woff[st.layer];
            d.bias = nullptr;
            const int nimg = d.in.B;
            for (int b0 = 0; b0 < nimg; b0 += kWinoChunk) {
                ConvDesc c = d;
                c.in.B = c.out.B = nimg - b0 < kWinoChunk ? nimg - b0 : kWinoChunk;
                c.in.base = d.in.base + (size_t)b0 * d.in.Hb * d.in.Wb * 4;
                c.out.base = d.out.base + (size_t)b0 * d.out.Hb * d.out.Wb * 4;
                QpBuf pv;
                if (d.pool) {
                    pv = *d.pool;
                    pv.B = c.in.B;
                    pv.base = d.pool->base + (size_t)b0 * pv.Hb * pv.Wb * 4;
                    c.pool = &pv;
                }
                if (d.in2_origin) c.in2_origin = d.in2_origin + b0;
                ND_TRY(nd_launch_conv_wino(kWinoTile, c, pl.wino, pl.wino_bytes, s, (o.ev_x && nimg <= kWinoChunk) ? o.ev_x + 2 * this_step : nullptr));
            }
            continue;
        }
        ND_TRY(nd_launch_conv(d, s));
    }
    if (o.ev) ND_HIP(hipEventRecord(o.ev[si], s));
    return ND_OK;
}

constexpr int kSharedSteps = 6;
constexpr int kStrip = 16;
constexpr double kBandBytes = 8.0 * (1 << 30);

inline int enc_extent(int x, int b) {
    const int p1 = (x - 4) / 2;
    switch (b) {
        case X0: return x;
        case A1: return x - 2;
        case CAT4: return x - 4;
        case P1: return p1;
        case A2: return p1 - 2;
        case CAT3: return p1 - 4;
        default: return (p1 - 4) / 2;
    }
}
Plan make_enc_plan(int f, int hx, int wx, int B, int hcap, int wcap, int cap, char *base, int dt, int slots = 1, Buf slotted = CAT4) {
    Plan p = {};
    size_t off = 0;
    auto add = [&](Buf id, int ch, int pad) {
        QpBuf &q = p.buf[id];
        q.planes = id == X0 ? 2 : (ch + nd_cpp(dt) - 1) / nd_cpp(dt);
        q.dt = dt;
        q.B = B;
        q.Hb = enc_extent(hx, id) + 2 * pad;
        q.Wb = enc_extent(wx, id) + 2 * pad;
        q.pad = pad;
        q.pstride = (long)cap * (enc_extent(hcap, id) + 2 * pad) * (enc_extent(wcap, id) + 2 * pad);
        if ((id == CAT4 || id == CAT3 || id == P2) && id >= slotted) q.pstride *= slots;
        q.base = (float *)(base + off);
        off += ((size_t)q.planes * q.pstride + nd_buf_slack(enc_extent(wcap, id) + 2 * pad)) * 16;
        off = (off + 255) & ~(size_t)255;
    };
    add(X0, 8, 0);
    add(A1, f, 0);
    add(CAT4, 2 * f, 2);
    add(P1, f, 0);
    add(A2, 2 * f, 0);
    add(CAT3, 4 * f, 2);
    add(P2, 2 * f, 0);
    p.split = nullptr;
    p.wino = nullptr;
    p.bytes = off;
    return p;
}

inline long slot_elems(const QpBuf &q, int slots) { return q.pstride / slots; }
inline Plan band_slot(Plan p, int slot, int slots, Buf slotted = CAT4) {
    for (Buf id : {CAT4, CAT3, P2})
        if (id >= slotted) p.buf[id].base += (size_t)slot * slot_elems(p.buf[id], slots) * 4;
    return p;
}

struct FramePlan {
    int D = 0;
    int aligned = 0;
    int S = 0, cols = 0, rows = 0, pad = 0;
    int R = 0, nbands = 0;
    int slots = 1;
    int hx = 0, wx = 0;
    int win4[2] = {0, 0}, win3[2] = {0, 0};
    size_t band_bytes = 0, row_edge_bytes = 0, col_edge_bytes = 0, corner_bytes = 0, origin_bytes = 0, bytes = 0;
    int levels = 0;
    int h2 = 0, w2 = 0;
    int win2[2] = {0, 0};
    size_t l2_band_bytes = 0, l2_row_bytes = 0, l2_col_bytes = 0, l2_corner_bytes = 0, l2_wino_bytes = 0;
};
inline int band_hx(const FramePlan &fp, int nrows, int cs) { return (nrows - 1) * fp.S + cs + 4; }
inline Plan row_edge_plan(const FramePlan &fp, int f, int dt, int nrows, char *base) {
    return make_enc_plan(f, kStrip, fp.wx, 2 * nrows, kStrip, fp.wx, 2 * fp.R, base, dt, fp.slots, P2);
}
inline Plan col_edge_plan(const FramePlan &fp, int f, int dt, int nrows, int cs, char *base) {
    return make_enc_plan(f, band_hx(fp, nrows, cs), kStrip, 2 * fp.cols, fp.hx, kStrip, 2 * fp.cols, base, dt, fp.slots, P2);
}
inline Plan corner_plan(int f, int dt, int ntiles, int cap, char *base) {
    return make_enc_plan(f, kStrip, kStrip, 4 * ntiles, kStrip, kStrip, 4 * cap, base, dt);
}

constexpr int kLevel2End = 9;
constexpr int kStrip2 = 6;

inline int l2_extent(int x, int b) {
    switch (b) {
        case P2: return x;
        case A3: return x - 2;
        case CAT2: return x - 4;
        default: return (x - 4) / 2;
    }
}
Plan make_l2_plan(int f, int h2, int w2, int B, int hcap, int wcap, int cap, char *base, int dt, int slots = 1, Buf slotted = CAT2,
                  bool own_p2 = true) {
    Plan p = {};
    size_t off = 0;
    auto add = [&](Buf id, int ch, int pad) {
        QpBuf &q = p.buf[id];
        q.planes = (ch + nd_cpp(dt) - 1) / nd_cpp(dt);
        q.dt = dt;
        q.B = B;
        q.Hb = l2_extent(h2, id) + 2 * pad;
        q.Wb = l2_extent(w2, id) + 2 * pad;
        q.pad = pad;
        q.pstride = (long)cap * (l2_extent(hcap, id) + 2 * pad) * (l2_extent(wcap, id) + 2 * pad);
        if ((id == CAT2 || id == P3) && id >= slotted) q.pstride *= slots;
        q.base = (float *)(base + off);
        off += ((size_t)q.planes * q.pstride + nd_buf_slack(l2_extent(wcap, id) + 2 * pad)) * 16;
        off = (off + 255) & ~(size_t)255;
    };
    if (own_p2) add(P2, 2 * f, 0);
    add(A3, 4 * f, 0);
    add(CAT2, 8 * f, 2);
    add(P3, 4 * f, 0);
    p.split = nullptr;
    p.wino = nullptr;
    p.bytes = off;
    return p;
}
inline Plan l2_slot(Plan p, int slot, int slots, Buf slotted = CAT2) {
    for (Buf id : {CAT2, P3})
        if (id >= slotted) p.buf[id].base += (size_t)slot * slot_elems(p.buf[id], slots) * 4;
// ... 12 lines not shown
inline Plan l2_col_plan(const FramePlan &fp, int f, int dt, int nrows, int cs, char *base) {
    return make_l2_plan(f, band_h2(fp, nrows, cs), kStrip2, 2 * fp.cols, fp.h2, kStrip2, 2 * fp.cols, base, dt, fp.slots, P3);
}
inline Plan l2_corner_plan(int f, int dt, int ntiles, int cap, char *base) {
    return make_l2_plan(f, kStrip2, kStrip2, 4 * ntiles, kStrip2, kStrip2, 4 * cap, base, dt);
}

inline void frame_plan_level2(int f, int dt, int flags, int cs, int batch, const BlobLayout &bl, const Roi *rois, FramePlan *fp) {
    fp->levels = fp->D;
    if ((flags & ND_FLAG_TILE_LEVEL2) || fp->S % 8) return;
    const int n2 = enc_extent(cs + 4, P2), n = l2_extent(n2, CAT2);
    if (n2 < kStrip2 + 2 || l2_extent(n2, P3) < 3) return;
    bool reads_cat2 = false;
    for (int i = kLevel2End; i < kNumSteps; ++i) {
        const Step &st = kSteps[i];
        if (st.layer < 0 || st.src != CAT2 || kLayers[st.layer].kind != ND_CONVT3) continue;
        if (rois[i].rows <= 0 || rois[i].r0 != rois[i].c0 || rois[i].rows != rois[i].cols) return;
        fp->win2[0] = rois[i].r0 - 2 < 0 ? 0 : rois[i].r0 - 2;
        fp->win2[1] = rois[i].r0 + rois[i].rows > n ? n : rois[i].r0 + rois[i].rows;
        if (fp->win2[0] < 1 || fp->win2[1] > n - 1 || fp->win2[1] <= fp->win2[0]) return;
        reads_cat2 = true;
    }
    if (!reads_cat2) return;
    fp->h2 = enc_extent(fp->hx, P2);
    fp->w2 = enc_extent(fp->wx, P2);
    Plan plans[4] = {l2_band_plan(*fp, f, dt, fp->R, cs, nullptr), l2_row_plan(*fp, f, dt, fp->R, nullptr),
                     l2_col_plan(*fp, f, dt, fp->R, cs, nullptr), l2_corner_plan(f, dt, batch, batch, nullptr)};
    plans[0].buf[P2] = make_enc_plan(f, fp->hx, fp->wx, 1, fp->hx, fp->wx, 1, nullptr, dt).buf[P2];
    size_t wino = 0;
    for (const Plan &pp : plans)
        for (int i = kSharedSteps; i < kLevel2End; ++i) {
            const Step &st = kSteps[i];
            if (st.layer < 0) continue;
            const LayerSpec &l = kLayers[st.layer];
            const Form form = step_form(st, f, dt, flags, pp, bl);
            if (form == FORM_WINO3P) {
                QpBuf v = pp.buf[st.src];
                v.B = v.B < kWinoChunk ? v.B : kWinoChunk;
                const size_t need = nd_wino_scratch_bytes(kWinoTile, v, lcin(l, f), lcout(l, f));
                wino = need > wino ? need : wino;
            } else if (form != FORM_W1D4 || !nd_f43_w2d(pp.buf[st.src], lcout(l, f), false, flags)) {
                return;
            }
        }
    fp->l2_band_bytes = plans[0].bytes;
    fp->l2_row_bytes = plans[1].bytes;
    fp->l2_col_bytes = plans[2].bytes;
    fp->l2_corner_bytes = plans[3].bytes;
    fp->l2_wino_bytes = (wino + 255) & ~(size_t)255;
    fp->bytes += fp->origin_bytes + fp->l2_band_bytes + fp->l2_row_bytes + fp->l2_col_bytes + fp->l2_corner_bytes + fp->l2_wino_bytes;
    fp->levels = 3;
}

int frame_plan(int f, int dt, int flags, int W, int H, int cs, int ucs, int ol, int batch, FramePlan *fp) {
    *fp = FramePlan();
    ND_TRY(check_funit(f, dt));
    if (!valid_cs(cs)) ND_FAIL(ND_EINVAL, "frame plan: tile size %d", cs);
    ND_TRY(nd_tile_grid(W, H, cs, ucs, ol, &fp->cols, &fp->rows, &fp->pad));
    fp->S = ucs - ol;
    fp->aligned = 1;
    while (fp->aligned < 4 && fp->S % (1 << fp->aligned) == 0) ++fp->aligned;
    if (dt != ND_F32 || (flags & (ND_FLAG_FULL_TILES | ND_FLAG_TILE_ENCODER | ND_FLAG_DIRECT_CONV | ND_FLAG_W1D_REGS)) ||
        fp->S % 4 || W < cs || H < cs || batch <= 0)
        return ND_OK;
    const Plan tp = make_plan(f, cs, cs, 1, 1, nullptr, dt);
    const BlobLayout bl = blob_layout(f, dt);
    Roi rois[kNumSteps];
    const int crop = (cs - ucs) / 2;
    if (!plan_rois(tp, crop, crop, rois)) return ND_OK;
    for (int i = 0; i < kNumSteps; ++i) {
        const Step &st = kSteps[i];
        if (st.layer < 0 || (st.src != CAT4 && st.src != CAT3) || kLayers[st.layer].kind != ND_CONVT3) continue;
        const int n = enc_extent(cs + 4, st.src), edge = st.src == CAT4 ? 2 : 1;
        if (rois[i].rows <= 0 || rois[i].r0 != rois[i].c0 || rois[i].rows != rois[i].cols) return ND_OK;
        int *w = st.src == CAT4 ? fp->win4 : fp->win3;
        w[0] = rois[i].r0 - 2 < 0 ? 0 : rois[i].r0 - 2;
        w[1] = rois[i].r0 + rois[i].rows > n ? n : rois[i].r0 + rois[i].rows;
        if (w[0] < edge || w[1] > n - edge) return ND_OK;
    }
    if (fp->win4[1] <= fp->win4[0] || fp->win3[1] <= fp->win3[0]) return ND_OK;
    fp->wx = (fp->cols - 1) * fp->S + cs + 4;
    for (int R = fp->rows; R >= 1; --R) {
        const int hx = band_hx(*fp, R, cs);
        const size_t b = make_enc_plan(f, hx, fp->wx, 1, hx, fp->wx, 1, nullptr, dt).bytes;
        if (b <= kBandBytes || R == 1) {
            fp->R = R;
            fp->hx = hx;
            fp->band_bytes = b;
            break;
        }
    }
    fp->nbands = (fp->rows + fp->R - 1) / fp->R;
    fp->R = (fp->rows + fp->nbands - 1) / fp->nbands;
    fp->hx = band_hx(*fp, fp->R, cs);
    fp->slots = fp->nbands > 1 ? 2 : 1;
    fp->band_bytes = make_enc_plan(f, fp->hx, fp->wx, 1, fp->hx, fp->wx, 1, nullptr, dt, fp->slots).bytes;
    if ((long)fp->hx * fp->wx >= (1L << 26)) return ND_OK;
    const Plan plans[4] = {make_enc_plan(f, fp->hx, fp->wx, 1, fp->hx, fp->wx, 1, nullptr, dt), row_edge_plan(*fp, f, dt, fp->R, nullptr),
                           col_edge_plan(*fp, f, dt, fp->R, cs, nullptr), corner_plan(f, dt, batch, batch, nullptr)};
    for (const Plan &pp : plans)
        for (int i = 0; i < kSharedSteps; ++i) {
            const Step &st = kSteps[i];
            if (st.layer < 0) continue;
            if (step_form(st, f, dt, flags, pp, bl) != FORM_W1D4 || !nd_f43_w2d(pp.buf[st.src], lcout(kLayers[st.layer], f), false, flags))
                return ND_OK;
        }
    fp->row_edge_bytes = plans[1].bytes;
    fp->col_edge_bytes = plans[2].bytes;
    fp->corner_bytes = plans[3].bytes;
    fp->origin_bytes = ((size_t)batch * sizeof(int) + 255) & ~(size_t)255;
    fp->bytes = fp->band_bytes + fp->row_edge_bytes + fp->col_edge_bytes + fp->corner_bytes + 2 * fp->origin_bytes;
    fp->D = 2;
    frame_plan_level2(f, dt, flags, cs, batch, bl, rois, fp);
    return ND_OK;
}

}
```

### nind_denoise_amd/csrc/winograd.hip

```cpp
#include <stdlib.h>

#include <algorithm>
#include <atomic>
#include <thread>
#include <vector>

#include "nd_common.h"

typedef float f32x4 __attribute__((ext_vector_type(4)));

namespace {

__device__ __forceinline__ void tile_pos(long t, int TX, int TY, int &tx, int &ty, int &b) {
    const unsigned u = (unsigned)t, row = u / (unsigned)TX;
    tx = (int)(u - row * (unsigned)TX);
    b = (int)(row / (unsigned)TY);
    ty = (int)(row - (unsigned)b * (unsigned)TY);
}

template <int T> struct Wino;
template <> struct Wino<2> {
    static constexpr int A = 4;
    template <typename V> __host__ __device__ static void bt(const V *d, V *o) {
        o[0] = d[0] - d[2];
// ... 188 lines not shown
        tile_pos(tt, TX, TY, tx, ty, b);
        const int x = T * tx + j;
        if (x >= Wv) continue;
#pragma unroll
        for (int i = 0; i < T; ++i)
            if (T * ty + i < Hv) dst[((long)b * Ho + T * ty + i + opad) * Wo + x + opad] = sm[i][p];
    }
}

template <int T, int NTL>
__global__ __launch_bounds__(NTL * (T + 2)) void k_wino_in2(const f32x4 *__restrict__ x, long xnp, int Hb, int Wb, long img_stride, int row_stride, int B,
                                                            int TY, int TX, f32x4 *__restrict__ v, long vnp, long vbs, const f32x4 *__restrict__ x2,
                                                            long x2np, int row_stride2, const int *__restrict__ origin2, int q2) {
    constexpr int A = Wino<T>::A, RS = A * A + 1;
    __shared__ f32x4 sm[NTL * RS];
    const long tiles = (long)B * TY * TX;
    const long t0 = (long)blockIdx.x * NTL;
    const int q = blockIdx.y;
    const f32x4 zero = {0.f, 0.f, 0.f, 0.f};
    {
        const int tl = threadIdx.x / A, j = threadIdx.x % A;
        const long t = t0 + tl;
        if (t < tiles) {
            int tx, ty, b;
    tile_pos(t, TX, TY, tx, ty, b);
            const bool s2 = q >= q2;
            const long rs = s2 ? row_stride2 : row_stride;
            const f32x4 *src = (s2 ? x2 + (long)(q - q2) * x2np + origin2[b] : x + (long)q * xnp + (long)b * img_stride) + (long)(T * ty) * rs + T * tx + j;
            f32x4 d[A], o[A];
            const bool okj = T * tx + j < Wb;
#pragma unroll
            for (int i = 0; i < A; ++i) d[i] = (okj && T * ty + i < Hb) ? src[(long)i * rs] : zero;
            Wino<T>::bt(d, o);
#pragma unroll
            for (int i = 0; i < A; ++i) sm[tl * RS + i * A + j] = o[i];
        }
    }
    __syncthreads();
    {
        const int i = threadIdx.x / NTL, tl = threadIdx.x % NTL;
        const long t = t0 + tl;
        if (t < tiles) {
            f32x4 r[A], o[A];
#pragma unroll
            for (int j = 0; j < A; ++j) r[j] = sm[tl * RS + i * A + j];
            Wino<T>::bt(r, o);
            f32x4 *dst = v + (long)q * vnp + t;
#pragma unroll
            for (int j = 0; j < A; ++j) dst[(long)(i * A + j) * vbs] = o[j];
        }
    }
}

template <int T, int NTL>
__global__ __launch_bounds__(NTL * (T + 2)) void k_wino_out2(const f32x4 *__restrict__ m, long mnp, long mbs, int B, int TY, int TX, int Hv,
                                                             int Wv, const float *__restrict__ bias, int act, float slope_imm,
                                                             const float *__restrict__ slope_dev, f32x4 *__restrict__ out, long onp,
                                                             int out_plane0, long out_img_stride, int Wo, int opad, f32x4 *__restrict__ pool, long pnp,
                                                             int Hp, int Wp, int ppad) {
    constexpr int A = Wino<T>::A, RS = T * A + 1, NTH = NTL * A;
    __shared__ f32x4 sr[NTL * RS];
    __shared__ f32x4 so[T][NTL * T];
    const long tiles = (long)B * TY * TX;
    const long t0 = (long)blockIdx.x * NTL;
    const int q = blockIdx.y;
    const f32x4 bv = *(const f32x4 *)(bias + 4 * q);
    const float slope = act == ND_ACT_NONE ? 1.f : (slope_dev ? *slope_dev : slope_imm);
    {
        const int j = threadIdx.x / NTL, tl = threadIdx.x % NTL;
        const long t = t0 + tl;
        if (t < tiles) {
            const f32x4 *src = m + (long)q * mnp + t;
            f32x4 c[A], o[T];
#pragma unroll
            for (int i = 0; i < A; ++i) c[i] = src[(long)(i * A + j) * mbs];
            Wino<T>::at(c, o);
#pragma unroll
            for (int i = 0; i < T; ++i) sr[tl * RS + i * A + j] = o[i];
        }
    }
    __syncthreads();
    if (threadIdx.x < NTL * T) {
        const int i = threadIdx.x / NTL, tl = threadIdx.x % NTL;
        if (t0 + tl < tiles) {
            f32x4 r[A], o[T];
#pragma unroll
            for (int j = 0; j < A; ++j) r[j] = sr[tl * RS + i * A + j];
            Wino<T>::at(r, o);
#pragma unroll
            for (int j = 0; j < T; ++j) {
                f32x4 y = o[j] + bv;
#pragma unroll
                for (int e = 0; e < 4; ++e) {
                    const float u = y[e];
                    switch (act) {
                        case ND_ACT_ELU: y[e] = u > 0.f ? u : expm1f(u); break;
                        case ND_ACT_HARDSWISH: y[e] = u * fminf(fmaxf(u + 3.f, 0.f), 6.f) / 6.f; break;
                        default: y[e] = u > 0.f ? u : u * slope; break;
                    }
                }
                so[i][tl * T + j] = y;
            }
        }
    }
    __syncthreads();
    f32x4 *dst = out + (long)(out_plane0 + q) * onp;
    for (int idx = threadIdx.x; idx < T * NTL * T; idx += NTH) {
        const int i = idx / (NTL * T), pp = idx - i * (NTL * T);
        const long tt = t0 + pp / T;
        if (tt >= tiles) continue;
        int tx, ty, b;
        tile_pos(tt, TX, TY, tx, ty, b);
        const int xx = T * tx + pp % T, yy = T * ty + i;
        if (xx < Wv && yy < Hv) dst[(long)b * out_img_stride + (long)(yy + opad) * Wo + xx + opad] = so[i][pp];
    }
    if (pool) {
        f32x4 *pd = pool + (long)q * pnp;
        for (int idx = threadIdx.x; idx < (T / 2) * NTL * (T / 2); idx += NTH) {
            const int a = idx / (NTL * (T / 2)), pp = idx - a * (NTL * (T / 2));
            const int tl = pp / (T / 2), c = pp % (T / 2);
            const long tt = t0 + tl;
            if (tt >= tiles) continue;
            int tx, ty, b;
        tile_pos(tt, TX, TY, tx, ty, b);
            const int px = tx * (T / 2) + c, py = ty * (T / 2) + a;
            if (2 * px + 1 < Wv && 2 * py + 1 < Hv) {
                const f32x4 p00 = so[2 * a][tl * T + 2 * c], p01 = so[2 * a][tl * T + 2 * c + 1];
                const f32x4 p10 = so[2 * a + 1][tl * T + 2 * c], p11 = so[2 * a + 1][tl * T + 2 * c + 1];
                f32x4 v;
#pragma unroll
                for (int e = 0; e < 4; ++e) v[e] = fmaxf(fmaxf(p00[e], p01[e]), fmaxf(p10[e], p11[e]));
                pd[((long)b * Hp + py + ppad) * Wp + px + ppad] = v;
            }
        }
    }
}

constexpr int kOutNtl = 32;
int positions(int T) { return (T + 2) * (T + 2); }
size_t gemm_floats(int cin, int cout) { return nd_packed_floats(ND_CONV1, cin, cout, ND_F32); }

struct WinoGeo {
    int TY, TX, Hv, Wv;
    long tiles;
    long vnp, mnp;
    long vbs, mbs;
    size_t v_bytes, m_bytes;
};
WinoGeo wino_geo(int T, const QpBuf &in, int cin, int cout, int roi_rows = 0, int roi_cols = 0) {
    WinoGeo g;
    g.Hv = roi_rows > 0 ? roi_rows : in.Hb - 2;
    g.Wv = roi_rows > 0 ? roi_cols : in.Wb - 2;
    g.TY = (g.Hv + T - 1) / T;
    g.TX = (g.Wv + T - 1) / T;
    g.tiles = (long)in.B * g.TY * g.TX;
    g.vnp = g.mnp = g.tiles;
    const long slack = 4096;
    g.vbs = (long)(2 * nd_kblocks(cin)) * g.vnp + slack;
    g.mbs = (long)((cout + 3) / 4) * g.mnp + slack;
    g.v_bytes = (size_t)positions(T) * g.vbs * 16;
    g.m_bytes = (size_t)positions(T) * g.mbs * 16;
    return g;
}
}

size_t nd_wino_packed_floats(int T, int cin, int cout) {
    return (size_t)positions(T) * gemm_floats(cin, cout) + (size_t)(cout + 3) / 4 * 4;
}

// ... 8 lines not shown
        std::vector<std::thread> th;
        for (int t = 0; t < nt; ++t)
            th.emplace_back([&] {
                for (int i = next.fetch_add(1); i < n; i = next.fetch_add(1)) fn(i);
            });
        for (auto &x : th) x.join();
    };
    parallel_for(cout, [&](int co) {
        for (int ci = 0; ci < cin; ++ci) {
            double g[3][3], tmp[8][3], U[8][8];
            for (int ky = 0; ky < 3; ++ky)
                for (int kx = 0; kx < 3; ++kx)
                    g[ky][kx] = kind == ND_CONV3 ? w[(((size_t)co * cin + ci) * 3 + ky) * 3 + kx]
                                                 : w[(((size_t)ci * cout + co) * 3 + (2 - ky)) * 3 + (2 - kx)];
            for (int kx = 0; kx < 3; ++kx) {
                double c[3] = {g[0][kx], g[1][kx], g[2][kx]}, o[8];
                if (T == 2) Wino<2>::g(c, o); else if (T == 4) Wino<4>::g(c, o); else Wino<6>::g(c, o);
                for (int i = 0; i < A; ++i) tmp[i][kx] = o[i];
            }
            for (int i = 0; i < A; ++i) {
                double o[8];
                if (T == 2) Wino<2>::g(tmp[i], o); else if (T == 4) Wino<4>::g(tmp[i], o); else Wino<6>::g(tmp[i], o);
                for (int j = 0; j < A; ++j) U[i][j] = o[j];
            }
            for (int i = 0; i < A; ++i)
                for (int j = 0; j < A; ++j) u[((size_t)(i * A + j) * cout + co) * cin + ci] = (float)U[i][j];
        }
    });
    const size_t gf = gemm_floats(cin, cout);
    parallel_for(P, [&](int p) { nd_pack_layer(ND_CONV1, cin, cout, ND_F32, u.data() + (size_t)p * cout * cin, nullptr, packed + p * gf); });
    float *b = packed + (size_t)P * gf;
    for (int co = 0; co < (cout + 3) / 4 * 4; ++co) b[co] = (bias && co < cout) ? bias[co] : 0.f;
    return ND_OK;
}

size_t nd_wino_scratch_bytes(int T, const QpBuf &in, int cin, int cout) {
    const WinoGeo g = wino_geo(T, in, cin, cout);
    return ((g.v_bytes + 255) & ~(size_t)255) + ((g.m_bytes + 255) & ~(size_t)255);
}

void nd_wino_xform_bytes(int T, const QpBuf &in, int cin, int cout, double *bytes_in, double *bytes_out) {
    const WinoGeo g = wino_geo(T, in, cin, cout);
    const double P = positions(T), px_in = (double)in.B * in.Hb * in.Wb, px_out = (double)in.B * g.Hv * g.Wv;
    *bytes_in = 4.0 * cin * px_in + 4.0 * cin * P * (double)g.tiles;
    *bytes_out = 4.0 * cout * P * (double)g.tiles + 4.0 * cout * px_out;
}

int nd_launch_conv_wino(int T, const ConvDesc &d, void *scratch, size_t scratch_bytes, hipStream_t s, hipEvent_t *ev2) {
    if (T != 2 && T != 4 && T != 6) ND_FAIL(ND_EINVAL, "winograd: tile must be 2, 4 or 6");
    if ((d.kind != ND_CONV3 && d.kind != ND_CONVT3) || d.in.dt != ND_F32 || d.out.dt != ND_F32)
        ND_FAIL(ND_EINVAL, "winograd: fp32 3x3 layers only");
    if (d.cin % 16 || d.cout % 4) ND_FAIL(ND_EINVAL, "winograd: Cin must be a multiple of 16, Cout of 4 (got %d, %d)", d.cin, d.cout);
    if (d.pre) ND_FAIL(ND_EINVAL, "winograd: inference only (no pre-activation copy)");
    ND_TRY(nd_check_roi("winograd", d, d.in.Hb - 2, d.in.Wb - 2, T != 6 || d.pool, "a layer other than an unpooled F(6x6) one"));
    const bool roi = d.roi_rows > 0;
    const WinoGeo g = wino_geo(T, d.in, d.cin, d.cout, d.roi_rows, d.roi_cols);
    const bool src2 = d.in2.base != nullptr;
    if (src2) {
        if (T != 6) ND_FAIL(ND_EINVAL, "winograd: only the F(6x6) form has a second input source");
        ND_TRY(nd_check_in2("winograd", d, nd_kblocks(d.cin), (long)(d.roi_r0 + g.Hv + 1) * d.in2.Wb + d.roi_c0 + g.Wv + 2));
    }
    ND_TRY(nd_check_out("winograd", d, d.in.Hb - 2, d.in.Wb - 2, false));
    const long roi_in = roi ? (long)d.roi_r0 * d.in.Wb + d.roi_c0 : 0, roi_out = roi ? (long)d.roi_r0 * d.out.Wb + d.roi_c0 : 0;
    const int vHb = g.Hv + 2, vWb = g.Wv + 2;
    const size_t need = nd_wino_scratch_bytes(T, d.in, d.cin, d.cout);
    if (!scratch || scratch_bytes < need) ND_FAIL(ND_ENOMEM, "winograd: scratch %zu B given, %zu B needed", scratch_bytes, need);
    if (g.tiles >= (1L << 31)) ND_FAIL(ND_EINVAL, "winograd: %ld tiles exceed the 32-bit tile index", g.tiles);
    const int P = positions(T);
    f32x4 *v = (f32x4 *)scratch;
    f32x4 *m = (f32x4 *)((char *)scratch + ((g.v_bytes + 255) & ~(size_t)255));
    const int in_planes = 2 * nd_kblocks(d.cin), out_planes = d.cout / 4;
    const f32x4 *x = (const f32x4 *)d.in.base + (long)d.in_plane0 * d.in.np() + roi_in;
    dim3 gi((unsigned)((g.tiles + 255) / 256), in_planes);
    constexpr int kNtl = 16;
    dim3 gi2((unsigned)((g.tiles + kNtl - 1) / kNtl), in_planes);
    if (T == 2)
        hipLaunchKernelGGL(k_wino_input<2>, gi, dim3(256), 0, s, x, d.in.np(), d.in.Hb, d.in.Wb, d.in.B, g.TY, g.TX, v, g.vnp, g.vbs);
    else if (T == 6)
        hipLaunchKernelGGL((k_wino_in2<6, kNtl>), gi2, dim3(kNtl * 8), 0, s, x, d.in.np(), vHb, vWb, (long)d.in.Hb * d.in.Wb, d.in.Wb, d.in.B, g.TY, g.TX, v, g.vnp, g.vbs,
                           src2 ? (const f32x4 *)d.in2.base + (long)d.in2_plane0 * d.in2.np() + (roi ? (long)d.roi_r0 * d.in2.Wb + d.roi_c0 : 0) : nullptr,
                           d.in2.np(), d.in2.Wb, d.in2_origin, src2 ? d.in2_from : in_planes);
    else
        hipLaunchKernelGGL(k_wino_input<4>, gi, dim3(256), 0, s, x, d.in.np(), d.in.Hb, d.in.Wb, d.in.B, g.TY, g.TX, v, g.vnp, g.vbs);
    ND_HIP(hipGetLastError());
    if (ev2) ND_HIP(hipEventRecord(ev2[0], s));

    ConvDesc e;
    e.kind = ND_CONV1;
    e.cin = d.cin;
    e.cout = d.cout;
    e.wpk = d.wpk;
    e.bias = d.wpk + nd_bias_offset(ND_CONV1, d.cin, d.cout);
    e.in = {(float *)v, in_planes, d.in.B, g.TY, g.TX, 0, g.vnp, ND_F32};
    e.out = {(float *)m, out_planes, d.in.B, g.TY, g.TX, 0, g.mnp, ND_F32};
    e.variant = nd_conv_variant_gemm(d.cin, d.cout);
    e.part = d.part;
    e.part_bytes = d.part_bytes;
    e.nosplit = d.nosplit;
    e.nbatch = P;
    e.in_bs = g.vbs;
    e.out_bs = g.mbs;
    e.w_bs = gemm_floats(d.cin, d.cout);
    ND_TRY(nd_launch_conv(e, s));
    if (ev2) ND_HIP(hipEventRecord(ev2[1], s));

    const float *bias = d.wpk + (size_t)P * gemm_floats(d.cin, d.cout);
    dim3 go((unsigned)((g.tiles + 127) / 128), out_planes);
    f32x4 *out = (f32x4 *)d.out.base + roi_out;
    f32x4 *pool = nullptr;
    long pnp = 0;
    int Hp = 0, Wp = 0, ppad = 0;
    if (d.pool) {
        const QpBuf &q = *d.pool;
        if (q.dt != ND_F32 || q.B != d.in.B || q.Hb - 2 * q.pad != g.Hv / 2 || q.Wb - 2 * q.pad != g.Wv / 2 || q.planes < out_planes)
            ND_FAIL(ND_EINVAL, "winograd: pooled destination does not fit %dx%dx%d", d.cout, g.Hv / 2, g.Wv / 2);
        pool = (f32x4 *)q.base;
        pnp = q.np();
        Hp = q.Hb;
        Wp = q.Wb;
        ppad = q.pad;
    }
    if (T == 6 && kOutNtl == 16) {
        dim3 go2((unsigned)((g.tiles + 15) / 16), out_planes);
        hipLaunchKernelGGL((k_wino_out2<6, 16>), go2, dim3(128), 0, s, (const f32x4 *)m, g.mnp, g.mbs, d.in.B, g.TY, g.TX, g.Hv, g.Wv, bias,
                           d.act, d.slope, d.slope_dev, out, d.out.np(), d.out_plane0, (long)d.out.Hb * d.out.Wb, d.out.Wb, d.out.pad, pool, pnp, Hp, Wp, ppad);
    } else if (T == 6) {
        dim3 go2((unsigned)((g.tiles + 31) / 32), out_planes);
        hipLaunchKernelGGL((k_wino_out2<6, 32>), go2, dim3(256), 0, s, (const f32x4 *)m, g.mnp, g.mbs, d.in.B, g.TY, g.TX, g.Hv, g.Wv, bias,
                           d.act, d.slope, d.slope_dev, out, d.out.np(), d.out_plane0, (long)d.out.Hb * d.out.Wb, d.out.Wb, d.out.pad, pool, pnp, Hp, Wp, ppad);
    }
    else if (T == 2)
        hipLaunchKernelGGL(k_wino_output<2>, go, dim3(128), 0, s, (const f32x4 *)m, g.mnp, g.mbs, d.in.B, g.TY, g.TX, g.Hv, g.Wv, bias,
                           d.act, d.slope, d.slope_dev, out, d.out.np(), d.out_plane0, d.out.Hb, d.out.Wb, d.out.pad, pool, pnp, Hp, Wp, ppad);
    else
        hipLaunchKernelGGL(k_wino_output<4>, go, dim3(128), 0, s, (const f32x4 *)m, g.mnp, g.mbs, d.in.B, g.TY, g.TX, g.Hv, g.Wv, bias,
                           d.act, d.slope, d.slope_dev, out, d.out.np(), d.out_plane0, d.out.Hb, d.out.Wb, d.out.pad, pool, pnp, Hp, Wp, ppad);
    ND_HIP(hipGetLastError());
    return ND_OK;
}
```

### nind_denoise_amd/networks/UtNet.py

```python
import ctypes

import torch
from torch import nn

from .. import _lib
from ..synth import utnet_layer_table, utnet_prelu_keys

_ACTIVATIONS = {"PReLU": nn.PReLU, "ELU": nn.ELU, "Hardswish": nn.Hardswish}
_SHORT_DTYPE = {_lib.ND_F32: "f32", _lib.ND_BF16: "bf16", _lib.ND_F16: "f16"}


def canonical_compute_dtype(name):
    if name not in _lib.DTYPE:
        raise ValueError(f"unknown compute dtype {name!r}; choose one of {', '.join(_lib.DTYPE)}")
    return _SHORT_DTYPE[_lib.DTYPE[name]]


def valid_cs(cs):
    return cs >= 104 and (cs - 56) % 16 == 0


def nearest_valid_cs(cs):
    k = (cs - 56 + 8) // 16
    return max(104, 16 * k + 56)
# ... 36 lines not shown

    @staticmethod
    def forward(ctx, model, names, x, *params):
        st = model._train_state(x.device)
        with torch.no_grad():
            for n, p in zip(names, params):
                off, cnt = st.ranges[n]
                st.flat[off:off + cnt].copy_(p.detach().reshape(-1))
        batch, h, w = x.size(0), x.size(2), x.size(3)
        y = torch.empty_like(x)
        with torch.cuda.device(x.device):
            ws = st.workspace(model, h, w, batch)
            _lib.check(_lib.load().nd_utnet_train_forward_hw(model.funit, _lib.ACT[model.activation], model.flags,
                                                             st.flat.data_ptr(), st.blobs.data_ptr(), x.data_ptr(), y.data_ptr(),
                                                             batch, h, w, ws.data_ptr(), ws.numel(), _lib.stream_ptr(x.device)),
                       "nd_utnet_train_forward_hw")
        st.generation += 1
        ctx.model, ctx.names, ctx.geom, ctx.generation = model, names, (batch, h, w), st.generation
        ctx.shapes = [p.shape for p in params]
        return y

    @staticmethod
    def backward(ctx, gy):
        model = ctx.model
        st = model._train_state(gy.device)
        if st.generation != ctx.generation:
            raise RuntimeError("UtNet backward: another forward of this module ran under autograd since this graph was built; its "
                               "activations are gone (one forward/backward in flight per module -- as the reference's training loop runs)")
        batch, h, w = ctx.geom
        want_dx, want_p = ctx.needs_input_grad[2], ctx.needs_input_grad[3:]
        gy = gy.to(torch.float32).contiguous()
        dx = torch.empty(batch, 3, h, w, dtype=torch.float32, device=gy.device) if want_dx else None
        with torch.cuda.device(gy.device):
            _lib.check(_lib.load().nd_utnet_train_backward_hw(model.funit, _lib.ACT[model.activation], model.flags,
                                                              st.flat.data_ptr(), st.grads.data_ptr() if any(want_p) else None,
                                                              st.blobs.data_ptr(), gy.data_ptr(), dx.data_ptr() if want_dx else None,
                                                              batch, h, w, st.ws.data_ptr(), st.ws.numel(), _lib.stream_ptr(gy.device),
                                                              None, 0), "nd_utnet_train_backward_hw")
        grads = []
        for n, shape, want in zip(ctx.names, ctx.shapes, want_p):
            off, cnt = st.ranges[n]
            grads.append(st.grads[off:off + cnt].view(shape).clone() if want else None)
        return (None, None, dx) + tuple(grads)


class UtNet(nn.Module):
    split_k = True
    winograd = True
    w1d_regs = False
    useful_only = True
    fused_pool = True
    share_encoder = True
    share_level2 = True

    def __init__(self, funit=64, activation='PReLU', compute_dtype='f32'):
        super().__init__()
        funit = int(funit)
        compute_dtype = canonical_compute_dtype(compute_dtype)
        if activation not in _ACTIVATIONS:
            exit(f'UtNet: unknown activation function: {activation}')
        self.funit, self.activation = funit, activation
        groups = {}
        for key, kind, cin, cout, k in utnet_layer_table(funit):
            if kind == "conv":
                layer = nn.Conv2d(cin, cout, k)
            elif kind == "convT":
                layer = nn.ConvTranspose2d(cin, cout, k)
            else:
                layer = nn.ConvTranspose2d(cin, cout, k, stride=2)
            if "." in key:
                seq, idx = key.split(".")
                groups.setdefault(seq, {})[int(idx)] = layer
            else:
                groups[key] = layer
        for key in utnet_prelu_keys():
            seq, idx = key.split(".")
            groups[seq][int(idx)] = _ACTIVATIONS[activation]()
        order = ["convs1", "convs2", "convs3", "convs4", "bottom"]
        for n in range(1, 5):
            order += [f"up{n}", f"tconvs{n}"]
        for name in order:
            g = groups[name]
            self.add_module(name, nn.Sequential(*[g[i] for i in sorted(g)]) if isinstance(g, dict) else g)
        self._packed = {}
        self.pack_on_device = True
        self._workspaces = {}
        self.max_cached_workspaces = 2
        self.compute_dtype = compute_dtype
        self.weights_generation = 0

    def set_compute_dtype(self, name):
        self.compute_dtype = canonical_compute_dtype(name)
        return self

    @property
    def _dt(self):
        return _lib.DTYPE[self.compute_dtype]

    @property
    def flags(self):
        return ((0 if self.split_k else _lib.FLAG_NO_SPLITK) | (0 if self.winograd else _lib.FLAG_DIRECT_CONV) |
                (_lib.FLAG_W1D_REGS if self.w1d_regs else 0) | (0 if self.useful_only else _lib.FLAG_FULL_TILES) |
                (0 if self.fused_pool else _lib.FLAG_UNFUSED_POOL) | (0 if self.share_encoder else _lib.FLAG_TILE_ENCODER))

    @property
    def frame_flags(self):
        return self.flags | (0 if self.share_level2 else _lib.FLAG_TILE_LEVEL2)

    def _weights_key(self, device):
        return (str(device), self.weights_generation) + tuple((p.data_ptr(), p._version) for p in self.parameters())

    def packed_weights(self, device):
        key = self._weights_key(device)
        hit = self._packed.get(self.compute_dtype)
        if hit is not None and hit[0] == key:
            return hit[1]
        lib = _lib.load()
        sd = self.state_dict()
        names = _lib.utnet_tensor_names()
        nbytes = lib.nd_utnet_packed_bytes(self.funit, self._dt)
        if nbytes == 0:
            raise ValueError(f"UtNet: funit={self.funit} is not supported by the HIP path for {self.compute_dtype} "
                             "(multiple of 8 for f32, of 16 for bf16 / f16)")
        on_device = self.pack_on_device
        where = device if on_device else "cpu"
        keep = []
        ptrs = (ctypes.c_void_p * len(names))()
        for i, n in enumerate(names):
            if n in sd:
                t = sd[n].detach().to(device=where, dtype=torch.float32).contiguous()
                keep.append(t)
                ptrs[i] = t.data_ptr()
            else:
                ptrs[i] = None
        if on_device:
            dev_blob = torch.empty(nbytes // 4, dtype=torch.float32, device=device)
            with torch.cuda.device(device):
                _lib.check(lib.nd_utnet_pack_weights_device(self.funit, self._dt, ptrs, len(names), dev_blob.data_ptr(), nbytes,
                                                            _lib.stream_ptr(device)), "nd_utnet_pack_weights_device")
                torch.cuda.current_stream(device).synchronize()
        else:
            blob = torch.empty(nbytes // 4, dtype=torch.float32)
            _lib.check(lib.nd_utnet_pack_weights(self.funit, self._dt, ptrs, len(names), blob.data_ptr(), nbytes),
                       "nd_utnet_pack_weights")
            dev_blob = blob.to(device)
        self._packed[self.compute_dtype] = (key, dev_blob)
        return dev_blob

    def workspace(self, cs, batch, device, width=None):
        h, w = int(cs), int(cs if width is None else width)
        key = (str(device), h, w, int(batch), self.compute_dtype)
        ws = self._workspaces.get(key)
        if ws is None:
            lib = _lib.load()
            nbytes = lib.nd_utnet_workspace_bytes_hw(self.funit, h, w, batch, self._dt)
            if nbytes == 0:
                _lib.check(lib.nd_utnet_workspace_init_hw(None, 0, self.funit, h, w, batch, self._dt, None), "UtNet")
            while len(self._workspaces) >= self.max_cached_workspaces:
                self._workspaces.pop(next(iter(self._workspaces)))
            ws = torch.empty(nbytes, dtype=torch.uint8, device=device)
# ... 57 lines not shown
```

Baseline: 84.14 MP/s.

## Fold skip-connection convolution halves into frame-shared addend sources

Adds an addend-source path to the w2d, split-K reduce and Winograd output kernels, plus a K-block sub-range into the packed weights. The decoder convolutions over concatenated skip inputs can then be split. The skip half is computed once per frame on shared buffers and added in, instead of being recomputed per tile. Bias and activation are deferred to the epilogue after the addend is added. It is enabled by default through fold_skips, and costs extra addend buffers, more validation and new kernel variants.

```diff
diff --git a/include/nind_hip.h b/include/nind_hip.h
--- a/include/nind_hip.h
+++ b/include/nind_hip.h
@@ -44,6 +44,7 @@
     ND_FLAG_TILE_ENCODER = 32,
     ND_FLAG_TILE_LEVEL2 = 64,
     ND_FLAG_FIND_NOISE = 128,
+    ND_FLAG_TILE_SKIPS = 256,
     ND_FLAG_FULL_TILES = 8
 } nd_flags;
 
@@ -89,6 +90,7 @@
                            nd_progress_fn progress, void *progress_ctx);
 int nd_utnet_frame_plan(int funit, int dtype, int flags, int width, int height, int cs, int ucs, int ol, int *out);
 int nd_utnet_frame_levels(int funit, int dtype, int flags, int width, int height, int cs, int ucs, int ol, int *levels);
+int nd_utnet_frame_folds(int funit, int dtype, int flags, int width, int height, int cs, int ucs, int ol, int *mask);
 
 typedef struct nd_step_profile {
     float ms;
diff --git a/nind_denoise_amd/_lib.py b/nind_denoise_amd/_lib.py
--- a/nind_denoise_amd/_lib.py
+++ b/nind_denoise_amd/_lib.py
@@ -11,6 +11,7 @@
 KIND = {"conv3": 0, "convT3": 1, "convT2s2": 2, "conv1": 3, "conv2s2": 4}
 FLAG_NO_SPLITK, FLAG_DIRECT_CONV, FLAG_W1D_REGS, FLAG_FULL_TILES, FLAG_UNFUSED_POOL, FLAG_TILE_ENCODER, FLAG_TILE_LEVEL2 = 1, 2, 4, 8, 16, 32, 64
 FLAG_FIND_NOISE = 128
+FLAG_TILE_SKIPS = 256
 PROGRESS_FN = ctypes.CFUNCTYPE(None, c_void_p, c_int, c_int, c_int)
 
 
@@ -68,6 +69,7 @@
     "nd_utnet_frame_workspace_bytes": (c_size_t, [c_int] * 9),
     "nd_utnet_frame_plan": (c_int, [c_int] * 8 + [POINTER(c_int)]),
     "nd_utnet_frame_levels": (c_int, [c_int] * 8 + [POINTER(c_int)]),
+    "nd_utnet_frame_folds": (c_int, [c_int] * 8 + [POINTER(c_int)]),
     "nd_utnet_denoise_frame": (c_int, [c_int] * 4 + [c_void_p] * 3 + [c_int] * 8 + [c_void_p, c_size_t, c_void_p, c_size_t, c_void_p,
                                                                                     PROGRESS_FN, c_void_p]),
     "nd_layer_packed_bytes": (c_size_t, [c_int] * 4),
diff --git a/nind_denoise_amd/csrc/conv_f32.hip b/nind_denoise_amd/csrc/conv_f32.hip
--- a/nind_denoise_amd/csrc/conv_f32.hip
+++ b/nind_denoise_amd/csrc/conv_f32.hip
@@ -233,7 +233,8 @@
     const int KB = nd_kblocks(d.cin, dt);
     const int M = up ? 4 * d.cout : d.cout;
     if (d.cout % nd_cpp(dt)) ND_FAIL(ND_EINVAL, "conv: cout=%d must be a multiple of %d", d.cout, nd_cpp(dt));
-    ND_TRY(nd_check_in_planes("conv", d, KB));
+    ND_TRY(nd_check_in_planes("conv", d, KB, false, true));
+    if (d.add.base) ND_FAIL(ND_EINVAL, "conv: this kernel form takes no addend source");
     ND_TRY(nd_check_int32("conv", d.in));
 
     int dev = 0, ncus = 0;
@@ -245,6 +246,10 @@
     if (KB % V.kbc) ND_FAIL(ND_EINVAL, "conv: Cin/8=%d not a multiple of the variant's K chunk %d", KB, V.kbc);
 
     ConvParams p = nd_conv_params(d, KB, M);
+    if (d.w_kb) {
+        p.KBw = d.w_kb;
+        p.wpk += (size_t)d.w_kb0 * taps * 256;
+    }
     valid_grid(taps, d.in, &p.Hv, &p.Wv, &p.stride);
     const bool roi = d.roi_rows > 0;
     ND_TRY(nd_check_roi("conv", d, p.Hv, p.Wv, taps == 4 || d.nbatch > 1 || d.pre, "a stride-2, batched or training launch"));
diff --git a/nind_denoise_amd/csrc/conv_qp.inc b/nind_denoise_amd/csrc/conv_qp.inc
--- a/nind_denoise_amd/csrc/conv_qp.inc
+++ b/nind_denoise_amd/csrc/conv_qp.inc
@@ -76,6 +76,11 @@
     long in2_plane;
     const int *origin2;
     int kb2, Wb2;
+    int KBw;
+    const f32x4 *add;
+    long add_plane;
+    const int *origin_add;
+    int W_add;
 };
 
 static inline void nd_conv_fastdivs(ConvParams &p) {
@@ -259,7 +264,7 @@
         f_end = it.c1;
         const int z = (int)fdiv((unsigned)it.tile, p.fd_tpp), id = it.tile - z * p.tiles_per_problem;
         const int nb = (int)fdiv((unsigned)id, p.fd_ntm), mb = id - nb * p.n_tiles_m;
-        f_w = p.wpk + z * p.w_bs + (size_t)mb * MTB * p.KB * TAPS * 256 + lane * 4;
+        f_w = p.wpk + z * p.w_bs + (size_t)mb * MTB * p.KBw * TAPS * 256 + lane * 4;
         f_a = p.in + z * p.in_bs + tile_q0(nb) + lane;
     };
     set_fill_tile(f_id);
@@ -287,7 +292,7 @@
         if (p.dbg & (i < MTB ? 2 : 1)) return;
 #endif
         if (i < MTB) {
-            const float *src = f_w + ((size_t)i * p.KB + (size_t)f_c * KBC) * TAPS * 256;
+            const float *src = f_w + ((size_t)i * p.KBw + (size_t)f_c * KBC) * TAPS * 256;
             char *dst = fill_sb + i * RW * 1024;
             for (int q = wave; q < RW; q += NFILL) glds16(src + q * 256, dst + q * 1024);
         } else {
diff --git a/nind_denoise_amd/csrc/conv_w2d.hip b/nind_denoise_amd/csrc/conv_w2d.hip
--- a/nind_denoise_amd/csrc/conv_w2d.hip
+++ b/nind_denoise_amd/csrc/conv_w2d.hip
@@ -54,7 +54,7 @@
 
 struct Strip { int img, y0, x0; bool ok; };
 
-template <int DBG, bool SRC2 = false>
+template <int DBG, bool SRC2 = false, bool ADD = false>
 __global__ __launch_bounds__(512) void conv_w2d(ConvParams p) {
     extern __shared__ __attribute__((aligned(16))) char smem[];
     const int lane = threadIdx.x & 63;
@@ -131,7 +131,7 @@
         f_c = it.c0;
         f_end = it.c1;
         const int nb = (int)fdiv((unsigned)it.tile, p.fd_ntm), mb = it.tile - nb * p.n_tiles_m;
-        f_w = p.wpk + (size_t)mb * kMTB * p.KB * kTaps * 256;
+        f_w = p.wpk + (size_t)mb * kMTB * p.KBw * kTaps * 256;
         if constexpr (SRC2) f_nb = nb;
 #pragma unroll
         for (int ps = 0; ps < 2; ++ps)
@@ -194,7 +194,7 @@
         if (issued >= nsteps || (DBG & 4)) return;
         if (dw >= 0 && dw < 4) {
             const int mt = dw >> 1, pl0 = (dw & 1) * 9;
-            const char *src = (const char *)(f_w + (((size_t)mt * p.KB + (size_t)f_c) * kTaps + pl0) * 256) + lane16;
+            const char *src = (const char *)(f_w + (((size_t)mt * p.KBw + (size_t)f_c) * kTaps + pl0) * 256) + lane16;
             char *dst = smem + f_stage * kStage + (mt * kTaps + pl0) * 1024;
             glds16o<-4096>(src + 4096, dst + 4096);
             glds16o<-3072>(src + 4096, dst + 4096);
@@ -256,6 +256,7 @@
     const int e_row = lane >> 4, e_px = lane & 15;
     f32x4 biasq[4];
     auto load_bias = [&](int id) {
+        if constexpr (ADD) return;
         const int mb = id - (int)fdiv((unsigned)id, p.fd_ntm) * p.n_tiles_m;
 #pragma unroll
         for (int g = 0; g < 4; ++g) biasq[g] = *(const f32x4 *)(p.bias + (mb * kMTB + wm) * 32 + 8 * g + 4 * h);
@@ -273,7 +274,23 @@
         const f32x2 slope2 = {slope, slope};
         const int pp_i = (e_px & ~3) + 2 * (e_px & 1);
         const int pxp = (st.x0 >> 1) + (e_px & 1), pyp = (st.y0 >> 1) + e_row;
-        const bool okP = !SRC2 && p.pool && !(lane & 2) && st.ok && 2 * pxp + 1 < p.wpx && 2 * pyp + 1 < p.Hv;
+        unsigned offQA = 0, offQB = 0;
+        f32x4 qa[8], qb[8];
+        auto add_loads = [&](int k) {
+            const int qq = (q0 + k) * 4 < p.M ? q0 + k : 0;
+            const char *pq = (const char *)(p.add + (size_t)qq * p.add_plane);
+            qa[k] = *(const f32x4 *)(pq + offQA);
+            qb[k] = *(const f32x4 *)(pq + offQB);
+        };
+        if constexpr (ADD) {
+            const unsigned oq = 16u * ((unsigned)p.origin_add[st.img] + (unsigned)(st.y0 + e_row) * (unsigned)p.W_add + (unsigned)ex);
+            offQA = okA ? oq : 0u;
+            offQB = okB ? oq + 64u * (unsigned)p.W_add : 0u;
+            add_loads(0);
+            add_loads(1);
+            __builtin_amdgcn_sched_barrier(0);
+        }
+        const bool okP = !SRC2 && !ADD && p.pool && !(lane & 2) && st.ok && 2 * pxp + 1 < p.wpx && 2 * pyp + 1 < p.Hv;
         const unsigned offP = (unsigned)((st.img * p.pool_P + (pyp + p.pool_pad) * p.pool_W + pxp + p.pool_pad) * 16);
 #pragma unroll
         for (int g = 0; g < 4; ++g) {
@@ -287,8 +304,13 @@
                     acc[x][4 * g + 2 * pr] = 0.f;
                     acc[x][4 * g + 2 * pr + 1] = 0.f;
                 }
-                const f32x2 bq = {biasq[g][2 * pr], biasq[g][2 * pr + 1]};
-                const f32x2 a = m[1] + m[2] + bq, b = m[1] - m[2] + bq, c = m[3] + m[4], e = m[3] - m[4];
+                f32x2 a = m[1] + m[2], b = m[1] - m[2];
+                const f32x2 c = m[3] + m[4], e = m[3] - m[4];
+                if constexpr (!ADD) {
+                    const f32x2 bq = {biasq[g][2 * pr], biasq[g][2 * pr + 1]};
+                    a += bq;
+                    b += bq;
+                }
                 f32x2 y[4];
                 y[0] = m[0] + a + c;
                 y[1] = b + 2.f * e;
@@ -298,7 +320,8 @@
                 for (int i = 0; i < 4; ++i) {
                     ypre[i][2 * pr] = y[i][0];
                     ypre[i][2 * pr + 1] = y[i][1];
-                    if constexpr (decltype(fast)::value) {
+                    if constexpr (ADD) {
+                    } else if constexpr (decltype(fast)::value) {
                         const f32x2 t = y[i] * slope2;
                         y[i] = f32x2{fmaxf(y[i][0], t[0]), fmaxf(y[i][1], t[1])};
                     } else {
@@ -308,7 +331,7 @@
                     yy[i][2 * pr + 1] = y[i][1];
                 }
             }
-            if (!SRC2 && p.pre) {
+            if (!SRC2 && !ADD && p.pre) {
                 const Strip so = strip_of(nb, sl);
                 const int yo = so.y0 + rr, m4 = (q0 + 2 * g + h) * 4, left = p.wpx - so.x0;
                 if (so.ok && yo < p.Hv && m4 < p.M) {
@@ -339,10 +362,29 @@
                 __builtin_amdgcn_fence(__ATOMIC_RELEASE, "wavefront");
                 __builtin_amdgcn_wave_barrier();
                 __builtin_amdgcn_fence(__ATOMIC_ACQUIRE, "wavefront");
-                const f32x4 va = *((const f32x4 *)scratch + e_row * 16 + e_px);
-                const f32x4 vb2 = *((const f32x4 *)scratch + (e_row + 4) * 16 + e_px);
+                f32x4 va = *((const f32x4 *)scratch + e_row * 16 + e_px);
+                f32x4 vb2 = *((const f32x4 *)scratch + (e_row + 4) * 16 + e_px);
+                if constexpr (ADD) {
+                    const int k = 2 * g + hq;
+                    va += qa[k];
+                    vb2 += qb[k];
+                    if (k + 2 < 8) {
+                        add_loads(k + 2);
+                        __builtin_amdgcn_sched_barrier(0);
+                    }
+#pragma unroll
+                    for (int e = 0; e < 4; ++e) {
+                        if constexpr (decltype(fast)::value) {
+                            va[e] = fmaxf(va[e], va[e] * slope);
+                            vb2[e] = fmaxf(vb2[e], vb2[e] * slope);
+                        } else {
+                            va[e] = apply_act(va[e], p.act, slope);
+                            vb2[e] = apply_act(vb2[e], p.act, slope);
+                        }
+                    }
+                }
                 f32x4 vp = va;
-                if (!SRC2 && p.pool) {
+                if (!SRC2 && !ADD && p.pool) {
                     const f32x4 *blk = (const f32x4 *)scratch + (2 * e_row) * 16 + pp_i;
                     const f32x4 p00 = blk[0], p01 = blk[1], p10 = blk[16], p11 = blk[17];
 #pragma unroll
@@ -462,7 +504,7 @@
     const int m4 = mb * (kMTB * 32) + quad * 4;
     if (m4 >= p.M) return;
     const float slope = p.act == ND_ACT_NONE ? 1.f : (p.slope_dev ? *p.slope_dev : p.slope);
-    const f32x4 bv = *(const f32x4 *)(p.bias + m4);
+    const f32x4 bv = p.add ? f32x4{0.f, 0.f, 0.f, 0.f} : *(const f32x4 *)(p.bias + m4);
     const unsigned tot = (unsigned)p.nimg * (unsigned)p.PV;
     for (int l = threadIdx.x; l < kSlots; l += 256) {
         const int i = l & 3, jj = l >> 2, wn = jj >> 5, j = jj & 31;
@@ -476,7 +518,10 @@
         if (y >= p.Hv || x >= p.wpx) continue;
         f32x4 acc = {0.f, 0.f, 0.f, 0.f};
         for (int ks = 0; ks < p.S; ++ks) acc += p.part[((size_t)(t * p.S + ks) * (kMTB * 8) + quad) * kSlots + l];
-        acc += bv;
+        if (p.add)
+            acc += p.add[(long)(m4 >> 2) * p.add_plane + (long)p.origin_add[img] + (long)y * p.W_add + x];
+        else
+            acc += bv;
         f32x4 v;
 #pragma unroll
         for (int e = 0; e < 4; ++e) v[e] = p.act <= ND_ACT_PRELU ? (acc[e] > 0.f ? acc[e] : acc[e] * slope) : apply_act(acc[e], p.act, slope);
@@ -502,8 +547,11 @@
     const int Hv = roi ? d.roi_rows : Hfull, Wpx = roi ? d.roi_cols : Wfull, Wg = (Wpx + 3) / 4, NB = (Hv + kR - 1) / kR;
     if (d.pre && (roi || d.pool)) ND_FAIL(ND_EINVAL, "w2d: a pre-activation copy goes with whole, unpooled layers only");
     if (d.cout % 4) ND_FAIL(ND_EINVAL, "w2d: cout must be a multiple of 4");
-    ND_TRY(nd_check_in_planes("w2d", d, KB, true));
-    const bool src2 = d.in2.base != nullptr;
+    ND_TRY(nd_check_in_planes("w2d", d, KB, true, true));
+    const bool src2 = d.in2.base != nullptr, add = d.add.base != nullptr;
+    if (add && (d.pool || d.pre || src2))
+        ND_FAIL(ND_EINVAL, "w2d: a layer with an addend source is neither pooled nor keeps a pre-activation copy nor has a second input source");
+    if (add) ND_TRY(nd_check_add("w2d", d, (long)(d.roi_r0 + Hv - 1 + d.add.pad) * d.add.Wb + d.roi_c0 + Wpx - 1 + d.add.pad + 1));
     if (src2 && (d.pool || d.pre)) ND_FAIL(ND_EINVAL, "w2d: a layer with a second input source is neither pooled nor keeps a pre-activation copy");
     if (src2) ND_TRY(nd_check_in2("w2d", d, KB, (long)(d.roi_r0 + (NB - 1) * kR + kRI - 1) * d.in2.Wb + d.roi_c0 + 4 * (Wg - 1) + 6));
     ND_TRY(nd_check_out("w2d", d, Hfull, Wfull, false));
@@ -512,10 +560,10 @@
 
     int dev = 0, ncus = 0;
     ND_TRY(nd_device(&dev, &ncus));
-    void (*fn)(ConvParams) = src2 ? conv_w2d<0, true> : conv_w2d<0>;
+    void (*fn)(ConvParams) = add ? conv_w2d<0, false, true> : src2 ? conv_w2d<0, true> : conv_w2d<0>;
 #ifdef ND_QP_STAMPS
     static const int dbg_all = getenv("ND_W2D_DBG") ? atoi(getenv("ND_W2D_DBG")) : 0;
-    const int dbg_env = src2 ? 0 : dbg_all;
+    const int dbg_env = src2 || add ? 0 : dbg_all;
     switch (dbg_env) {
         case 1: fn = conv_w2d<1>; break;
         case 2: fn = conv_w2d<2>; break;
@@ -546,6 +594,17 @@
         p.kb2 = d.in2_from / 2;
         p.Wb2 = d.in2.Wb;
     }
+    if (d.w_kb) {
+        p.KBw = d.w_kb;
+        p.wpk += (size_t)d.w_kb0 * kTaps * 256;
+    }
+    if (add) {
+        p.add = (const f32x4 *)d.add.base + (long)d.add_plane0 * d.add.np() + (long)((roi ? d.roi_r0 : 0) + d.add.pad) * d.add.Wb +
+                (roi ? d.roi_c0 : 0) + d.add.pad;
+        p.add_plane = d.add.np();
+        p.origin_add = d.add_origin;
+        p.W_add = d.add.Wb;
+    }
     p.Hv = Hv;
     p.Wv = Wg;
     p.PV = NB * Wg;
diff --git a/nind_denoise_amd/csrc/launch.hip b/nind_denoise_amd/csrc/launch.hip
--- a/nind_denoise_amd/csrc/launch.hip
+++ b/nind_denoise_amd/csrc/launch.hip
@@ -45,9 +45,24 @@
     return ND_OK;
 }
 
-int nd_check_in_planes(const char *who, const ConvDesc &d, int KB, bool takes_in2) {
+int nd_check_in_planes(const char *who, const ConvDesc &d, int KB, bool takes_in2, bool takes_add) {
     if (d.in.planes < d.in_plane0 + 2 * KB) ND_FAIL(ND_EINVAL, "%s: input buffer has %d planes, needs %d", who, d.in.planes, d.in_plane0 + 2 * KB);
     if (d.in2.base && !takes_in2) ND_FAIL(ND_EINVAL, "%s: this kernel form has no second input source", who);
+    if ((d.add.base || d.w_kb) && !takes_add) ND_FAIL(ND_EINVAL, "%s: this kernel form takes no addend source and no K-block sub-range", who);
+    if (d.w_kb && (d.w_kb0 < 0 || d.w_kb0 + KB > d.w_kb))
+        ND_FAIL(ND_EINVAL, "%s: K blocks [%d,+%d) outside the %d of the packed weights", who, d.w_kb0, KB, d.w_kb);
+    return ND_OK;
+}
+
+int nd_check_add(const char *who, const ConvDesc &d, long reach) {
+    const QpBuf &q = d.add;
+    const int n = d.cout / 4;
+    if (q.dt != ND_F32 || d.out.dt != ND_F32 || !d.add_origin || d.add_plane0 < 0 || d.add_plane0 + n > q.planes || d.add_origin_max < 0 ||
+        reach <= 0)
+        ND_FAIL(ND_EINVAL, "%s: addend source: planes [%d,+%d) of %d", who, d.add_plane0, n, q.planes);
+    const long last = d.add_origin_max + reach, room = (long)(q.planes - d.add_plane0 - n + 1) * q.np() + (long)nd_buf_slack(q.Wb);
+    if (last > room) ND_FAIL(ND_EINVAL, "%s: addend source: a launch reaches element %ld of a plane, the buffer ends at %ld", who, last, room);
+    if (last * 16 >= (1L << 32)) ND_FAIL(ND_EINVAL, "%s: addend source too large for 32-bit byte offsets", who);
     return ND_OK;
 }
 
@@ -101,6 +116,7 @@
     p.pre = (f32x4 *)d.pre;
     p.pre_plane = d.pre_plane;
     p.KB = KB;
+    p.KBw = KB;
     p.M = M;
     p.cout = d.cout;
     p.Po = d.out.Hb * d.out.Wb;
diff --git a/nind_denoise_amd/csrc/nd_common.h b/nind_denoise_amd/csrc/nd_common.h
--- a/nind_denoise_amd/csrc/nd_common.h
+++ b/nind_denoise_amd/csrc/nd_common.h
@@ -63,8 +63,14 @@
     int in2_plane0 = 0, in2_from = 0;
     const int *in2_origin = nullptr;
     long in2_origin_max = 0;
+    int w_kb = 0, w_kb0 = 0;
+    QpBuf add = {};
+    int add_plane0 = 0;
+    const int *add_origin = nullptr;
+    long add_origin_max = 0;
 };
 int nd_check_in2(const char *who, const ConvDesc &d, int KB, long reach);
+int nd_check_add(const char *who, const ConvDesc &d, long reach);
 static const size_t kSplitScratchBytes = (size_t)512 * 64 * 1024 * 4;
 int nd_launch_conv(const ConvDesc &d, hipStream_t stream);
 bool nd_conv_pool_fits(const ConvDesc &d);
@@ -89,13 +95,13 @@
 int nd_device(int *dev, int *ncus = nullptr);
 int nd_raise_lds(int dev, const void *fn, size_t bytes);
 int nd_once_per_device(int dev, int (*init)());
-int nd_check_in_planes(const char *who, const ConvDesc &d, int KB, bool takes_in2 = false);
+int nd_check_in_planes(const char *who, const ConvDesc &d, int KB, bool takes_in2 = false, bool takes_add = false);
 int nd_check_out(const char *who, const ConvDesc &d, int oh, int ow, bool at_least);
 int nd_check_int32(const char *who, const QpBuf &in);
 int nd_check_roi(const char *who, const ConvDesc &d, int Hv, int Wv, bool refused, const char *why);
 static inline int nd_check_flags(int flags, bool frame_loop = false, bool unet_frame = false) {
     const int known = ND_FLAG_NO_SPLITK | ND_FLAG_DIRECT_CONV | ND_FLAG_W1D_REGS | ND_FLAG_FULL_TILES | ND_FLAG_UNFUSED_POOL |
-                      ND_FLAG_TILE_ENCODER | (frame_loop ? ND_FLAG_TILE_LEVEL2 : 0) | (unet_frame ? ND_FLAG_FIND_NOISE : 0);
+                      ND_FLAG_TILE_ENCODER | (frame_loop ? ND_FLAG_TILE_LEVEL2 | ND_FLAG_TILE_SKIPS : 0) | (unet_frame ? ND_FLAG_FIND_NOISE : 0);
     if (flags & ~known) ND_FAIL(ND_EINVAL, "unknown flag bits 0x%x", flags);
     return ND_OK;
 }
diff --git a/nind_denoise_amd/csrc/pack.hip b/nind_denoise_amd/csrc/pack.hip
--- a/nind_denoise_amd/csrc/pack.hip
+++ b/nind_denoise_amd/csrc/pack.hip
@@ -12,7 +12,7 @@
 }
 
 extern "C" const char *nd_last_error(void) { return g_err; }
-extern "C" int nd_version(void) { return 109; }
+extern "C" int nd_version(void) { return 110; }
 
 static inline uint16_t f32_to_bf16_rne(float f) {
     uint32_t u;
diff --git a/nind_denoise_amd/csrc/utnet.hip b/nind_denoise_amd/csrc/utnet.hip
--- a/nind_denoise_amd/csrc/utnet.hip
+++ b/nind_denoise_amd/csrc/utnet.hip
@@ -184,6 +184,15 @@
     return ND_OK;
 }
 
+extern "C" int nd_utnet_frame_folds(int funit, int dtype, int flags, int width, int height, int cs, int ucs, int ol, int *mask) {
+    ND_TRY(nd_check_flags(flags, true));
+    if (!mask) ND_FAIL(ND_EINVAL, "nd_utnet_frame_folds: null output");
+    FramePlan fp;
+    ND_TRY(frame_plan(funit, dtype, flags, width, height, cs, ucs, ol, 1, &fp));
+    *mask = fp.folds;
+    return ND_OK;
+}
+
 extern "C" int nd_utnet_denoise_frame(int funit, int act, int dtype, int flags, const void *packed, const float *img, float *canvas,
                                       int width, int height, int cs, int ucs, int ol, int tile_begin, int tile_count, int batch,
                                       void *ws, size_t ws_bytes, void *fws, size_t fws_bytes, void *stream, nd_progress_fn progress,
@@ -205,7 +214,7 @@
         for (int t0 = tile_begin; t0 < end; t0 += batch, ++n) {
             const int cnt = end - t0 < batch ? end - t0 : batch;
             if (progress) progress(progress_ctx, n, t0, cnt);
-            ND_TRY(nd_utnet_denoise_tiles(funit, act, dtype, flags & ~ND_FLAG_TILE_LEVEL2, packed, img, canvas, width, height, cs, ucs, ol, t0, cnt, batch, ws,
+            ND_TRY(nd_utnet_denoise_tiles(funit, act, dtype, flags & ~(ND_FLAG_TILE_LEVEL2 | ND_FLAG_TILE_SKIPS), packed, img, canvas, width, height, cs, ucs, ol, t0, cnt, batch, ws,
                                           ws_bytes, stream));
         }
         return ND_OK;
@@ -237,16 +246,23 @@
         p.wino_bytes = fp.l2_wino_bytes;
         return p;
     };
-    struct Skip { Buf cat; int planes, step, tstep; const int *win; int *table; bool in_place; } skips[3] = {
-        {CAT4, f4, -1, S, fp.win4, origins, false}, {CAT3, 2 * f4, -1, S / 2, fp.win3, origins + fp.origin_bytes / sizeof(int), false},
-        {CAT2, 4 * f4, -1, S / 4, fp.win2, origins + 2 * fp.origin_bytes / sizeof(int), false}};
+    struct Skip { Buf cat; int planes, step, tstep; const int *win; int *table; bool in_place, fold; Form form; } skips[3] = {
+        {CAT4, f4, -1, S, fp.win4, origins, false, false, FORM_DIRECT},
+        {CAT3, 2 * f4, -1, S / 2, fp.win3, origins + fp.origin_bytes / sizeof(int), false, false, FORM_DIRECT},
+        {CAT2, 4 * f4, -1, S / 4, fp.win2, origins + 2 * fp.origin_bytes / sizeof(int), false, false, FORM_DIRECT}};
+    char *const fold_wino = (char *)fws + fp.bytes - fp.fold_wino_bytes;
     const int nskips = l2 ? 3 : 2;
-    for (Skip &k : skips)
-        for (int i = kSharedSteps; i < kNumSteps; ++i)
+    for (int ki = 0; ki < 3; ++ki)
+        for (int i = kSharedSteps; i < kNumSteps; ++i) {
+            Skip &k = skips[ki];
             if (kSteps[i].layer >= 0 && kSteps[i].src == k.cat) {
+                const Form form = step_form(kSteps[i], funit, dtype, flags, pl, bl);
                 k.step = i;
-                k.in_place = form_takes_src2(kSteps[i], step_form(kSteps[i], funit, dtype, flags, pl, bl), funit, flags, pl);
-            }
+                k.in_place = form_takes_src2(kSteps[i], form, funit, flags, pl);
+                k.form = form;
+                k.fold = ki < nskips && ((fp.folds >> ki) & 1) && k.in_place;
+            }
+        }
     StepSrc2 src2[3];
     dec.src2 = src2;
     const int per_band = fp.R * cols;
@@ -263,6 +279,10 @@
             bp.split = pl.split;
             ND_TRY(nd_launch_gather_band(img, width, height, cs, ucs, ol, row0, bp.buf[X0], s));
             ND_TRY(run_stack(funit, act, dtype, blob, bp, s, enc));
+            for (int ki = 0; ki < 2; ++ki)
+                if (skips[ki].fold)
+                    ND_TRY(launch_skip_fold(funit, flags, blob, bl, skips[ki].step, skips[ki].form, bp.buf[skips[ki].cat], skips[ki].planes,
+                                            rois[skips[ki].step], skips[ki].tstep, nrows, cols, pl.split, fold_wino, fp.fold_wino_bytes, s));
             Plan re = band_slot(row_edge_plan(fp, funit, dtype, nrows, rows_base), b & 1, fp.slots, P2);
             Plan ce = band_slot(col_edge_plan(fp, funit, dtype, nrows, cs, cols_base), b & 1, fp.slots, P2);
             re.split = ce.split = pl.split;
@@ -274,6 +294,9 @@
                 Plan b2 = l2_scratch(l2_slot(l2_band_plan(fp, funit, dtype, nrows, cs, l2_band_base), b & 1, fp.slots));
                 b2.buf[P2] = bp.buf[P2];
                 ND_TRY(run_stack(funit, act, dtype, blob, b2, s, enc2));
+                if (skips[2].fold)
+                    ND_TRY(launch_skip_fold(funit, flags, blob, bl, skips[2].step, skips[2].form, b2.buf[CAT2], skips[2].planes, rois[skips[2].step],
+                                            skips[2].tstep, nrows, cols, pl.split, fold_wino, fp.fold_wino_bytes, s));
                 const Plan r2 = l2_scratch(l2_slot(l2_row_plan(fp, funit, dtype, nrows, l2_rows_base), b & 1, fp.slots, P3));
                 const Plan c2 = l2_scratch(l2_slot(l2_col_plan(fp, funit, dtype, nrows, cs, l2_cols_base), b & 1, fp.slots, P3));
                 const int h2 = bp.buf[P2].Hb, w2 = bp.buf[P2].Wb;
@@ -305,7 +328,7 @@
         for (int ki = 0; ki < nskips; ++ki) {
             const Skip &k = skips[ki];
             const QpBuf &src = k.cat == CAT2 ? bf2.buf[k.cat] : bf.buf[k.cat];
-            if (!k.in_place) {
+            if (!k.in_place && !k.fold) {
                 SpliceMap m;
                 m.step_y = m.step_x = k.tstep;
                 ND_TRY(nd_launch_splice(src, k.planes, tp.buf[k.cat], k.planes, k.planes, t0, cnt, cols, 0, m, k.win[0], k.win[1], k.win[0],
@@ -316,6 +339,11 @@
             q.step = k.step;
             q.buf = src;
             q.plane0 = q.from = k.planes;
+            q.addend = k.fold;
+            if (k.fold) {
+                q.plane0 = 0;
+                q.buf.pad = 1;
+            }
             q.origin = k.table;
             ND_TRY(nd_launch_skip_origins(src, tp.buf[k.cat].pad, t0, cnt, cols, fp.R, k.tstep, slot_elems(src, fp.slots), k.table,
                                           &q.origin_max, s));
diff --git a/nind_denoise_amd/csrc/utnet_net.h b/nind_denoise_amd/csrc/utnet_net.h
--- a/nind_denoise_amd/csrc/utnet_net.h
+++ b/nind_denoise_amd/csrc/utnet_net.h
@@ -335,6 +335,7 @@
     int plane0 = 0, from = 0;
     const int *origin = nullptr;
     long origin_max = 0;
+    bool addend = false;
 };
 inline bool form_takes_src2(const Step &st, Form form, int f, int flags, const Plan &pl) {
     if (form == FORM_WINO3P) return kWinoTile == 6;
@@ -382,7 +383,8 @@
             d.pre = pre[l.prelu].base;
             d.pre_plane = pre[l.prelu].np();
         }
-        d.cin = lcin(l, f);
+        const int cin = lcin(l, f);
+        d.cin = cin;
         d.cout = lcout(l, f);
         d.wpk = blob + bl.off[st.layer];
         d.bias = d.wpk + nd_bias_offset(l.kind, d.cin, d.cout, dt);
@@ -400,7 +402,14 @@
             d.roi_cols = o.rois[this_step].cols;
         }
         for (int i = 0; i < o.nsrc2; ++i)
-            if (o.src2[i].step == k) {
+            if (o.src2[i].step == k && o.src2[i].addend) {
+                d.add = o.src2[i].buf;
+                d.add_plane0 = o.src2[i].plane0;
+                d.add_origin = o.src2[i].origin;
+                d.add_origin_max = o.src2[i].origin_max;
+                d.w_kb = nd_kblocks(cin, dt);
+                d.cin = o.src2[i].from * cpp;
+            } else if (o.src2[i].step == k) {
                 d.in2 = o.src2[i].buf;
                 d.in2_plane0 = o.src2[i].plane0;
                 d.in2_from = o.src2[i].from;
@@ -418,7 +427,7 @@
         if (form == FORM_W1D4 || form == FORM_W1D2) {
             const int T = form == FORM_W1D4 ? kW1dTile : 2;
             if (!pre) d.wpk = blob + (T == kW1dTile ? bl.w1off[st.layer] : bl.w1off2[st.layer]);
-            d.bias = d.wpk + nd_bias_offset(d.kind, d.cin, d.cout, ND_F32, T);
+            d.bias = d.wpk + nd_bias_offset(d.kind, cin, d.cout, ND_F32, T);
             ND_TRY(form == FORM_W1D4 ? nd_launch_conv_f43(d, flags, s) : nd_launch_conv_w1d(T, d, s));
             continue;
         }
@@ -439,6 +448,7 @@
                     c.pool = &pv;
                 }
                 if (d.in2_origin) c.in2_origin = d.in2_origin + b0;
+                if (d.add_origin) c.add_origin = d.add_origin + b0;
                 ND_TRY(nd_launch_conv_wino(kWinoTile, c, pl.wino, pl.wino_bytes, s, (o.ev_x && nimg <= kWinoChunk) ? o.ev_x + 2 * this_step : nullptr));
             }
             continue;
@@ -515,6 +525,8 @@
     int h2 = 0, w2 = 0;
     int win2[2] = {0, 0};
     size_t l2_band_bytes = 0, l2_row_bytes = 0, l2_col_bytes = 0, l2_corner_bytes = 0, l2_wino_bytes = 0;
+    int folds = 0;
+    size_t fold_wino_bytes = 0;
 };
 inline int band_hx(const FramePlan &fp, int nrows, int cs) { return (nrows - 1) * fp.S + cs + 4; }
 inline Plan row_edge_plan(const FramePlan &fp, int f, int dt, int nrows, char *base) {
@@ -633,6 +645,71 @@
     fp->levels = 3;
 }
 
+constexpr int kFoldRows = 48;
+inline void frame_plan_folds(int f, int dt, int flags, const Plan &tp, const BlobLayout &bl, FramePlan *fp) {
+    fp->folds = 0;
+    fp->fold_wino_bytes = 0;
+    if (!fp->D || (flags & ND_FLAG_TILE_SKIPS)) return;
+    const Buf cats[3] = {CAT4, CAT3, CAT2};
+    for (int k = 0; k < (fp->levels == 3 ? 3 : 2); ++k)
+        for (int i = kSharedSteps; i < kNumSteps; ++i) {
+            const Step &st = kSteps[i];
+            if (st.layer < 0 || st.src != cats[k] || kLayers[st.layer].kind != ND_CONVT3) continue;
+            const Form form = step_form(st, f, dt, flags, tp, bl);
+            if (!form_takes_src2(st, form, f, flags, tp)) continue;
+            fp->folds |= 1 << k;
+            if (form != FORM_WINO3P) continue;
+            QpBuf v = {};
+            v.B = 1;
+            v.Hb = kFoldRows + 2;
+            v.Wb = (k == 2 ? l2_extent(fp->w2, CAT2) : enc_extent(fp->wx, cats[k])) + 4;
+            const size_t need = nd_wino_scratch_bytes(kWinoTile, v, lcin(kLayers[st.layer], f) / 2, lcout(kLayers[st.layer], f));
+            if (need > fp->fold_wino_bytes) fp->fold_wino_bytes = need;
+        }
+    fp->fold_wino_bytes = (fp->fold_wino_bytes + 255) & ~(size_t)255;
+    fp->bytes += fp->fold_wino_bytes;
+}
+inline int launch_skip_fold(int f, int flags, const float *blob, const BlobLayout &bl, int step, Form form, const QpBuf &cat, int planes,
+                            const Roi &roi, int tstep, int nrows, int cols, float *split, char *wino, size_t wino_bytes, hipStream_t s) {
+    const LayerSpec &l = kLayers[kSteps[step].layer];
+    const int cin = lcin(l, f);
+    ConvDesc d;
+    d.kind = l.kind;
+    d.act = ND_ACT_NONE;
+    d.cin = planes * 4;
+    d.cout = lcout(l, f);
+    d.wpk = blob + bl.w1off[kSteps[step].layer];
+    d.bias = d.wpk + nd_bias_offset(l.kind, cin, d.cout, ND_F32, kW1dTile);
+    d.w_kb = nd_kblocks(cin);
+    d.w_kb0 = planes / 2;
+    d.in = cat;
+    d.in_plane0 = planes;
+    d.out = cat;
+    d.out.pad = 1;
+    d.out_plane0 = 0;
+    d.part = split;
+    d.part_bytes = split ? kSplitScratchBytes : 0;
+    d.nosplit = (flags & ND_FLAG_NO_SPLITK) != 0;
+    d.roi_r0 = roi.r0;
+    d.roi_c0 = roi.c0;
+    d.roi_rows = (nrows - 1) * tstep + roi.rows;
+    d.roi_cols = (cols - 1) * tstep + roi.cols;
+    if (form != FORM_WINO3P) return nd_launch_conv_w2d(d, s);
+    d.wpk = blob + bl.woff[kSteps[step].layer];
+    d.bias = nullptr;
+    const int r_end = d.roi_r0 + d.roi_rows;
+    for (int r0 = d.roi_r0; r0 < r_end; r0 += kFoldRows) {
+        ConvDesc c = d;
+        const int rows = r_end - r0 < kFoldRows ? r_end - r0 : kFoldRows;
+        c.in.base = c.out.base = cat.base + (size_t)r0 * cat.Wb * 4;
+        c.in.Hb = c.out.Hb = rows + 2;
+        c.roi_r0 = 0;
+        c.roi_rows = rows;
+        ND_TRY(nd_launch_conv_wino(kWinoTile, c, wino, wino_bytes, s));
+    }
+    return ND_OK;
+}
+
 int frame_plan(int f, int dt, int flags, int W, int H, int cs, int ucs, int ol, int batch, FramePlan *fp) {
     *fp = FramePlan();
     ND_TRY(check_funit(f, dt));
@@ -693,6 +770,7 @@
     fp->bytes = fp->band_bytes + fp->row_edge_bytes + fp->col_edge_bytes + fp->corner_bytes + 2 * fp->origin_bytes;
     fp->D = 2;
     frame_plan_level2(f, dt, flags, cs, batch, bl, rois, fp);
+    frame_plan_folds(f, dt, flags, tp, bl, fp);
     return ND_OK;
 }
 
diff --git a/nind_denoise_amd/csrc/winograd.hip b/nind_denoise_amd/csrc/winograd.hip
--- a/nind_denoise_amd/csrc/winograd.hip
+++ b/nind_denoise_amd/csrc/winograd.hip
@@ -264,20 +264,33 @@
     }
 }
 
-template <int T, int NTL>
+template <int T, int NTL, bool ADD = false>
 __global__ __launch_bounds__(NTL * (T + 2)) void k_wino_out2(const f32x4 *__restrict__ m, long mnp, long mbs, int B, int TY, int TX, int Hv,
                                                              int Wv, const float *__restrict__ bias, int act, float slope_imm,
                                                              const float *__restrict__ slope_dev, f32x4 *__restrict__ out, long onp,
                                                              int out_plane0, long out_img_stride, int Wo, int opad, f32x4 *__restrict__ pool, long pnp,
-                                                             int Hp, int Wp, int ppad) {
+                                                             int Hp, int Wp, int ppad, const f32x4 *__restrict__ add = nullptr, long add_np = 0,
+                                                             const int *__restrict__ origin_add = nullptr, int W_add = 0) {
     constexpr int A = Wino<T>::A, RS = T * A + 1, NTH = NTL * A;
     __shared__ f32x4 sr[NTL * RS];
     __shared__ f32x4 so[T][NTL * T];
     const long tiles = (long)B * TY * TX;
     const long t0 = (long)blockIdx.x * NTL;
     const int q = blockIdx.y;
-    const f32x4 bv = *(const f32x4 *)(bias + 4 * q);
+    const f32x4 bv = ADD ? f32x4{0.f, 0.f, 0.f, 0.f} : *(const f32x4 *)(bias + 4 * q);
     const float slope = act == ND_ACT_NONE ? 1.f : (slope_dev ? *slope_dev : slope_imm);
+    auto activate = [&](f32x4 y) {
+#pragma unroll
+        for (int e = 0; e < 4; ++e) {
+            const float u = y[e];
+            switch (act) {
+                case ND_ACT_ELU: y[e] = u > 0.f ? u : expm1f(u); break;
+                case ND_ACT_HARDSWISH: y[e] = u * fminf(fmaxf(u + 3.f, 0.f), 6.f) / 6.f; break;
+                default: y[e] = u > 0.f ? u : u * slope; break;
+            }
+        }
+        return y;
+    };
     {
         const int j = threadIdx.x / NTL, tl = threadIdx.x % NTL;
         const long t = t0 + tl;
@@ -301,17 +314,7 @@
             Wino<T>::at(r, o);
 #pragma unroll
             for (int j = 0; j < T; ++j) {
-                f32x4 y = o[j] + bv;
-#pragma unroll
-                for (int e = 0; e < 4; ++e) {
-                    const float u = y[e];
-                    switch (act) {
-                        case ND_ACT_ELU: y[e] = u > 0.f ? u : expm1f(u); break;
-                        case ND_ACT_HARDSWISH: y[e] = u * fminf(fmaxf(u + 3.f, 0.f), 6.f) / 6.f; break;
-                        default: y[e] = u > 0.f ? u : u * slope; break;
-                    }
-                }
-                so[i][tl * T + j] = y;
+                so[i][tl * T + j] = ADD ? o[j] : activate(o[j] + bv);
             }
         }
     }
@@ -324,9 +327,13 @@
         int tx, ty, b;
         tile_pos(tt, TX, TY, tx, ty, b);
         const int xx = T * tx + pp % T, yy = T * ty + i;
-        if (xx < Wv && yy < Hv) dst[(long)b * out_img_stride + (long)(yy + opad) * Wo + xx + opad] = so[i][pp];
-    }
-    if (pool) {
+        if (xx < Wv && yy < Hv) {
+            f32x4 y = so[i][pp];
+            if constexpr (ADD) y = activate(y + add[(long)q * add_np + (long)origin_add[b] + (long)yy * W_add + xx]);
+            dst[(long)b * out_img_stride + (long)(yy + opad) * Wo + xx + opad] = y;
+        }
+    }
+    if (!ADD && pool) {
         f32x4 *pd = pool + (long)q * pnp;
         for (int idx = threadIdx.x; idx < (T / 2) * NTL * (T / 2); idx += NTH) {
             const int a = idx / (NTL * (T / 2)), pp = idx - a * (NTL * (T / 2));
@@ -441,6 +448,11 @@
         ND_FAIL(ND_EINVAL, "winograd: fp32 3x3 layers only");
     if (d.cin % 16 || d.cout % 4) ND_FAIL(ND_EINVAL, "winograd: Cin must be a multiple of 16, Cout of 4 (got %d, %d)", d.cin, d.cout);
     if (d.pre) ND_FAIL(ND_EINVAL, "winograd: inference only (no pre-activation copy)");
+    const bool add = d.add.base != nullptr;
+    if ((add || d.w_kb) && T != 6) ND_FAIL(ND_EINVAL, "winograd: only the F(6x6) form takes an addend source or a K-block sub-range");
+    if (add && (d.pool || d.in2.base)) ND_FAIL(ND_EINVAL, "winograd: a layer with an addend source is neither pooled nor has a second input source");
+    if (d.w_kb && (d.w_kb0 < 0 || d.w_kb0 + nd_kblocks(d.cin) > d.w_kb)) ND_FAIL(ND_EINVAL, "winograd: K blocks [%d,+%d) outside the %d of the packed weights", d.w_kb0, nd_kblocks(d.cin), d.w_kb);
+    const int cin_w = d.w_kb ? 8 * d.w_kb : d.cin;
     ND_TRY(nd_check_roi("winograd", d, d.in.Hb - 2, d.in.Wb - 2, T != 6 || d.pool, "a layer other than an unpooled F(6x6) one"));
     const bool roi = d.roi_rows > 0;
     const WinoGeo g = wino_geo(T, d.in, d.cin, d.cout, d.roi_rows, d.roi_cols);
@@ -449,6 +461,7 @@
         if (T != 6) ND_FAIL(ND_EINVAL, "winograd: only the F(6x6) form has a second input source");
         ND_TRY(nd_check_in2("winograd", d, nd_kblocks(d.cin), (long)(d.roi_r0 + g.Hv + 1) * d.in2.Wb + d.roi_c0 + g.Wv + 2));
     }
+    if (add) ND_TRY(nd_check_add("winograd", d, (long)(d.roi_r0 + g.Hv - 1 + d.add.pad) * d.add.Wb + d.roi_c0 + g.Wv - 1 + d.add.pad + 1));
     ND_TRY(nd_check_out("winograd", d, d.in.Hb - 2, d.in.Wb - 2, false));
     const long roi_in = roi ? (long)d.roi_r0 * d.in.Wb + d.roi_c0 : 0, roi_out = roi ? (long)d.roi_r0 * d.out.Wb + d.roi_c0 : 0;
     const int vHb = g.Hv + 2, vWb = g.Wv + 2;
@@ -479,7 +492,9 @@
     e.cin = d.cin;
     e.cout = d.cout;
     e.wpk = d.wpk;
-    e.bias = d.wpk + nd_bias_offset(ND_CONV1, d.cin, d.cout);
+    e.bias = d.wpk + nd_bias_offset(ND_CONV1, cin_w, d.cout);
+    e.w_kb = d.w_kb;
+    e.w_kb0 = d.w_kb0;
     e.in = {(float *)v, in_planes, d.in.B, g.TY, g.TX, 0, g.vnp, ND_F32};
     e.out = {(float *)m, out_planes, d.in.B, g.TY, g.TX, 0, g.mnp, ND_F32};
     e.variant = nd_conv_variant_gemm(d.cin, d.cout);
@@ -489,11 +504,11 @@
     e.nbatch = P;
     e.in_bs = g.vbs;
     e.out_bs = g.mbs;
-    e.w_bs = gemm_floats(d.cin, d.cout);
+    e.w_bs = gemm_floats(cin_w, d.cout);
     ND_TRY(nd_launch_conv(e, s));
     if (ev2) ND_HIP(hipEventRecord(ev2[1], s));
 
-    const float *bias = d.wpk + (size_t)P * gemm_floats(d.cin, d.cout);
+    const float *bias = d.wpk + (size_t)P * gemm_floats(cin_w, d.cout);
     dim3 go((unsigned)((g.tiles + 127) / 128), out_planes);
     f32x4 *out = (f32x4 *)d.out.base + roi_out;
     f32x4 *pool = nullptr;
@@ -509,7 +524,14 @@
         Wp = q.Wb;
         ppad = q.pad;
     }
-    if (T == 6 && kOutNtl == 16) {
+    if (add) {
+        const f32x4 *ap = (const f32x4 *)d.add.base + (long)d.add_plane0 * d.add.np() + (long)((roi ? d.roi_r0 : 0) + d.add.pad) * d.add.Wb +
+                          (roi ? d.roi_c0 : 0) + d.add.pad;
+        dim3 go2((unsigned)((g.tiles + 31) / 32), out_planes);
+        hipLaunchKernelGGL((k_wino_out2<6, 32, true>), go2, dim3(256), 0, s, (const f32x4 *)m, g.mnp, g.mbs, d.in.B, g.TY, g.TX, g.Hv, g.Wv, bias,
+                           d.act, d.slope, d.slope_dev, out, d.out.np(), d.out_plane0, (long)d.out.Hb * d.out.Wb, d.out.Wb, d.out.pad, nullptr, 0L, 0, 0, 0,
+                           ap, d.add.np(), d.add_origin, d.add.Wb);
+    } else if (T == 6 && kOutNtl == 16) {
         dim3 go2((unsigned)((g.tiles + 15) / 16), out_planes);
         hipLaunchKernelGGL((k_wino_out2<6, 16>), go2, dim3(128), 0, s, (const f32x4 *)m, g.mnp, g.mbs, d.in.B, g.TY, g.TX, g.Hv, g.Wv, bias,
                            d.act, d.slope, d.slope_dev, out, d.out.np(), d.out_plane0, (long)d.out.Hb * d.out.Wb, d.out.Wb, d.out.pad, pool, pnp, Hp, Wp, ppad);
diff --git a/nind_denoise_amd/networks/UtNet.py b/nind_denoise_amd/networks/UtNet.py
--- a/nind_denoise_amd/networks/UtNet.py
+++ b/nind_denoise_amd/networks/UtNet.py
@@ -112,6 +112,7 @@
     fused_pool = True
     share_encoder = True
     share_level2 = True
+    fold_skips = True
 
     def __init__(self, funit=64, activation='PReLU', compute_dtype='f32'):
         super().__init__()
@@ -165,7 +166,7 @@
 
     @property
     def frame_flags(self):
-        return self.flags | (0 if self.share_level2 else _lib.FLAG_TILE_LEVEL2)
+        return self.flags | (0 if self.share_level2 else _lib.FLAG_TILE_LEVEL2) | (0 if self.fold_skips else _lib.FLAG_TILE_SKIPS)
 
     def _weights_key(self, device):
         return (str(device), self.weights_generation) + tuple((p.data_ptr(), p._version) for p in self.parameters())
```

After: 87.51 MP/s (median of 6 runs). +4.0%, better.
